# yurimjeon1892/EFGH

Hardware: AMD Instinct MI355X
Metric: frame-pairs/sec EFGHNet fwd+bwd (384x1280 RGB + 64x2048 range), whole job (higher is better)
Workload: dtype f32; 1 GPU; BASELINE.json configs[2]: EFGHNet fwd+bwd with efghloss + gradient all-reduce + fused Adam, synthetic 384x1280 RGB + 131072-point sweep, batch=8 per GPU, random-init weights; global_batch=8, points=131072, parallelism=dp1

## Files before the change

efgh_amd/csrc/backward.hip:

```cpp
#include "common.h"

namespace {
constexpr int TPB = 256;

__device__ __forceinline__ float4 sign4(const unsigned *__restrict__ bits, long long e) {
    const unsigned w = bits[e >> 5] >> ((unsigned)e & 31u);
    return make_float4((w & 1u) ? 1.f : -1.f, (w & 2u) ? 1.f : -1.f, (w & 4u) ? 1.f : -1.f, (w & 8u) ? 1.f : -1.f);
}

__device__ __forceinline__ float dact(float y, int act, float slope) {
    if (act == 1) return y > 0.f ? 1.f : 0.f;
    if (act == 2) return y > 0.f ? 1.f : slope;
    return 1.f;
}

template <bool NT>
__global__ void __launch_bounds__(TPB)
k_act_bn_bwd_reduce(const float *__restrict__ dy, long long lddy, const float *__restrict__ y, long long ldy,
                    const float *__restrict__ raw, long long ldraw, const float *__restrict__ mean,
                    const float *__restrict__ invstd, const float *__restrict__ pscale,
                    const float *__restrict__ pshift, long long M, int C, int act, float slope, int rows_per_block,
                    int CL, double *__restrict__ part, const unsigned *__restrict__ ybits) {
    __shared__ double s1s[TPB][4], s2s[TPB][4];
    const int cl = threadIdx.x % CL, rl = threadIdx.x / CL, RL = TPB / CL;
    const int c = (blockIdx.x * CL + cl) * 4;
    long long r0 = (long long)blockIdx.y * rows_per_block, r1 = r0 + rows_per_block;
    if (r1 > M) r1 = M;
    double s1[4] = {0., 0., 0., 0.}, s2[4] = {0., 0., 0., 0.};
    if (c < C) {
        float4 mu = make_float4(0.f, 0.f, 0.f, 0.f), is = mu, psc = mu, psh = mu;
        if (mean) { mu = *reinterpret_cast<const float4 *>(mean + c); is = *reinterpret_cast<const float4 *>(invstd + c); }
        const bool from_raw = !y && !ybits;
        if (from_raw) { psc = *reinterpret_cast<const float4 *>(pscale + c); psh = *reinterpret_cast<const float4 *>(pshift + c); }
        for (long long r = r0 + rl; r < r1; r += RL) {
            float4 g = ld_stream<NT>(dy + r * lddy + c);
            float4 rw = make_float4(0.f, 0.f, 0.f, 0.f);
            if (mean || from_raw) rw = ld_stream<NT>(raw + r * ldraw + c);
            float4 yy;
            if (ybits) yy = sign4(ybits, r * C + c);
            else if (y) yy = *reinterpret_cast<const float4 *>(y + r * ldy + c);
            else yy = make_float4(rw.x * psc.x + psh.x, rw.y * psc.y + psh.y, rw.z * psc.z + psh.z, rw.w * psc.w + psh.w);
            g.x *= dact(yy.x, act, slope); g.y *= dact(yy.y, act, slope);
            g.z *= dact(yy.z, act, slope); g.w *= dact(yy.w, act, slope);
            s1[0] += (double)g.x; s1[1] += (double)g.y; s1[2] += (double)g.z; s1[3] += (double)g.w;
            if (mean) {
                s2[0] += (double)g.x * (double)((rw.x - mu.x) * is.x); s2[1] += (double)g.y * (double)((rw.y - mu.y) * is.y);
                s2[2] += (double)g.z * (double)((rw.z - mu.z) * is.z); s2[3] += (double)g.w * (double)((rw.w - mu.w) * is.w);
            }
        }
    }
#pragma unroll
    for (int q = 0; q < 4; ++q) { s1s[threadIdx.x][q] = s1[q]; s2s[threadIdx.x][q] = s2[q]; }
    __syncthreads();
    if (rl != 0 || c >= C) return;
    for (int i = 1; i < RL; ++i)
#pragma unroll
        for (int q = 0; q < 4; ++q) { s1[q] += s1s[i * CL + cl][q]; s2[q] += s2s[i * CL + cl][q]; }
#pragma unroll
    for (int q = 0; q < 4; ++q) {
        part[((long long)blockIdx.y * 2) * C + c + q] = s1[q];
        part[((long long)blockIdx.y * 2 + 1) * C + c + q] = s2[q];
    }
}

__global__ void __launch_bounds__(1024)
k_bwd_finalize(const double *__restrict__ part, int G, int C, double count,
               float *__restrict__ sum_dpre, float *__restrict__ sum_dpre_xhat,
               double *__restrict__ mean_dpre, double *__restrict__ mean_dpre_xhat) {
    __shared__ double sa[32][33], sb[32][33];
    const int tx = threadIdx.x, ty = threadIdx.y;
    const int c = blockIdx.x * 32 + tx;
    double a = 0.0, b = 0.0;
    if (c < C) {
        double a1 = 0.0, b1 = 0.0, a2 = 0.0, b2 = 0.0, a3 = 0.0, b3 = 0.0;
        int g = ty;
        for (; g + 96 < G; g += 128) {
            a += part[((long long)g * 2) * C + c]; b += part[((long long)g * 2 + 1) * C + c];
            a1 += part[((long long)(g + 32) * 2) * C + c]; b1 += part[((long long)(g + 32) * 2 + 1) * C + c];
            a2 += part[((long long)(g + 64) * 2) * C + c]; b2 += part[((long long)(g + 64) * 2 + 1) * C + c];
            a3 += part[((long long)(g + 96) * 2) * C + c]; b3 += part[((long long)(g + 96) * 2 + 1) * C + c];
        }
        for (; g < G; g += 32) { a += part[((long long)g * 2) * C + c]; b += part[((long long)g * 2 + 1) * C + c]; }
        a += (a1 + a2) + a3; b += (b1 + b2) + b3;
    }
    sa[ty][tx] = a; sb[ty][tx] = b;
    __syncthreads();
    if (ty != 0 || c >= C) return;
    for (int i = 1; i < 32; ++i) { a += sa[i][tx]; b += sb[i][tx]; }
    sum_dpre[c] = (float)a; sum_dpre_xhat[c] = (float)b;
    if (mean_dpre) { mean_dpre[c] = a / count; mean_dpre_xhat[c] = b / count; }
}

template <bool NT>
__global__ void __launch_bounds__(TPB)
k_act_bn_bwd_apply(const float *__restrict__ dy, long long lddy, const float *__restrict__ y, long long ldy,
                   const float *__restrict__ raw, long long ldraw, const float *__restrict__ mean,
                   const float *__restrict__ invstd, const float *__restrict__ coef,
                   const double *__restrict__ m1, const double *__restrict__ m2, const float *__restrict__ pscale,
                   const float *__restrict__ pshift, long long M, int C, int act,
                   float slope, float *__restrict__ draw, long long lddraw, float *__restrict__ dres,
                   long long lddres, const unsigned *__restrict__ ybits) {
    const int c4n = C >> 2;
    long long total = M * c4n;
    const bool from_raw = !y && !ybits;
    for (long long i = (long long)blockIdx.x * TPB + threadIdx.x; i < total; i += (long long)gridDim.x * TPB) {
        long long r = i / c4n; int c = (int)(i - r * c4n) * 4;
        float4 g = ld_stream<NT>(dy + r * lddy + c);
        float4 rw = make_float4(0.f, 0.f, 0.f, 0.f);
        if (mean || from_raw) rw = ld_stream<NT>(raw + r * ldraw + c);
        float4 yy;
        if (ybits) yy = sign4(ybits, r * C + c);
        else if (y) yy = *reinterpret_cast<const float4 *>(y + r * ldy + c);
        else yy = make_float4(rw.x * pscale[c] + pshift[c], rw.y * pscale[c + 1] + pshift[c + 1],
                              rw.z * pscale[c + 2] + pshift[c + 2], rw.w * pscale[c + 3] + pshift[c + 3]);
        float gv[4] = {g.x * dact(yy.x, act, slope), g.y * dact(yy.y, act, slope), g.z * dact(yy.z, act, slope),
                       g.w * dact(yy.w, act, slope)};
        if (dres) st_stream<NT>(dres + r * lddres + c, make_float4(gv[0], gv[1], gv[2], gv[3]));
        float o[4];
        if (mean) {
            float rv[4] = {rw.x, rw.y, rw.z, rw.w};
#pragma unroll
            for (int q = 0; q < 4; ++q) {
                const double xh = ((double)rv[q] - (double)mean[c + q]) * (double)invstd[c + q];
                o[q] = (float)((double)coef[c + q] * ((double)gv[q] - m1[c + q] - xh * m2[c + q]));
            }
        } else {
#pragma unroll
            for (int q = 0; q < 4; ++q) o[q] = coef ? coef[c + q] * gv[q] : gv[q];
        }
        if (draw) st_stream<NT>(draw + r * lddraw + c, make_float4(o[0], o[1], o[2], o[3]));
    }
}

__device__ __forceinline__ void pool_cell_dpre(const float4 v[4], const bool ok[4], bool pooled, const float4 g, const float sc[4],
                                               const float sf[4], int act, float slope, float dpre[4][4]) {
#pragma unroll
    for (int ch = 0; ch < 4; ++ch) {
        float e[4];
#pragma unroll
        for (int q = 0; q < 4; ++q) {
            const float t = ((const float *)&v[q])[ch] * sc[ch] + sf[ch];
            e[q] = act == 1 ? (t > 0.f ? t : 0.f) : (act == 2 ? (t > 0.f ? t : t * slope) : t);
        }
        int best = 0;
#pragma unroll
        for (int q = 1; q < 4; ++q) if (e[q] > e[best]) best = q;
        const float gg = ((const float *)&g)[ch];
#pragma unroll
        for (int q = 0; q < 4; ++q) {
            const float t = ((const float *)&v[q])[ch] * sc[ch] + sf[ch];
            const float da = act == 1 ? (t > 0.f ? 1.f : 0.f) : (act == 2 ? (t > 0.f ? 1.f : slope) : 1.f);
            dpre[q][ch] = (pooled && q == best && ok[q]) ? gg * da : 0.f;
        }
    }
}

template <bool NT>
__global__ void __launch_bounds__(TPB)
k_pool_bn_bwd_reduce(const float *__restrict__ dyp, const float *__restrict__ raw, const float *__restrict__ mean,
                     const float *__restrict__ invstd, const float *__restrict__ pscale, const float *__restrict__ pshift,
                     int B, int H, int W, int C, int act, float slope, int cells_per_block, int CL, double *__restrict__ part) {
    __shared__ double s1s[TPB][4], s2s[TPB][4];
    const int Hc = (H + 1) / 2, Wc = (W + 1) / 2, Ho = H / 2, Wo = W / 2;
    const long long ncell = (long long)B * Hc * Wc;
    const int cl = threadIdx.x % CL, rl = threadIdx.x / CL, RL = TPB / CL;
    const int c = (blockIdx.x * CL + cl) * 4;
    long long r0 = (long long)blockIdx.y * cells_per_block, r1 = r0 + cells_per_block;
    if (r1 > ncell) r1 = ncell;
    double s1[4] = {0., 0., 0., 0.}, s2[4] = {0., 0., 0., 0.};
    if (c < C) {
        const float4 mu = *reinterpret_cast<const float4 *>(mean + c), is = *reinterpret_cast<const float4 *>(invstd + c);
        const float4 psc = *reinterpret_cast<const float4 *>(pscale + c), psh = *reinterpret_cast<const float4 *>(pshift + c);
        const float sc[4] = {psc.x, psc.y, psc.z, psc.w}, sf[4] = {psh.x, psh.y, psh.z, psh.w};
        const float muv[4] = {mu.x, mu.y, mu.z, mu.w}, isv[4] = {is.x, is.y, is.z, is.w};
        for (long long r = r0 + rl; r < r1; r += RL) {
            const int j = (int)(r % Wc); const long long t = r / Wc;
            const int i = (int)(t % Hc); const long long b = t / Hc;
            if (i >= Ho || j >= Wo) continue;
            const long long base = (((b * H + 2 * i) * W) + 2 * j) * (long long)C + c;
            const long long offs[4] = {0, C, (long long)W * C, (long long)W * C + C};
            float4 v[4];
            const bool ok[4] = {true, true, true, true};
#pragma unroll
            for (int q = 0; q < 4; ++q) v[q] = ld_stream<NT>(raw + base + offs[q]);
            const float4 g = *reinterpret_cast<const float4 *>(dyp + (((b * Ho + i) * Wo) + j) * (long long)C + c);
            float dpre[4][4];
            pool_cell_dpre(v, ok, true, g, sc, sf, act, slope, dpre);
#pragma unroll
            for (int q = 0; q < 4; ++q)
#pragma unroll
                for (int ch = 0; ch < 4; ++ch) {
                    const float d = dpre[q][ch];
                    s1[ch] += (double)d;
                    s2[ch] += (double)d * (double)((((const float *)&v[q])[ch] - muv[ch]) * isv[ch]);
                }
        }
    }
#pragma unroll
    for (int q = 0; q < 4; ++q) { s1s[threadIdx.x][q] = s1[q]; s2s[threadIdx.x][q] = s2[q]; }
    __syncthreads();
    if (rl != 0 || c >= C) return;
    for (int k = 1; k < RL; ++k)
#pragma unroll
        for (int q = 0; q < 4; ++q) { s1[q] += s1s[k * CL + cl][q]; s2[q] += s2s[k * CL + cl][q]; }
#pragma unroll
    for (int q = 0; q < 4; ++q) {
        part[((long long)blockIdx.y * 2) * C + c + q] = s1[q];
        part[((long long)blockIdx.y * 2 + 1) * C + c + q] = s2[q];
    }
}

template <bool NT>
__global__ void __launch_bounds__(TPB)
k_pool_bn_bwd_reduce_y(const float *__restrict__ dyp, const float *__restrict__ y, const float *__restrict__ raw,
                       const float *__restrict__ mean, const float *__restrict__ invstd, const float *__restrict__ pscale,
                       const float *__restrict__ pshift, int H, int W, int C, long long Mp, int rows_per_block, int CL,
                       double *__restrict__ part) {
    __shared__ double s1s[TPB][4], s2s[TPB][4];
    const int cl = threadIdx.x % CL, rl = threadIdx.x / CL, RL = TPB / CL;
    const int c = (blockIdx.x * CL + cl) * 4;
    const int Ho = H >> 1, Wo = W >> 1;
    long long r0 = (long long)blockIdx.y * rows_per_block, r1 = r0 + rows_per_block;
    if (r1 > Mp) r1 = Mp;
    double s1[4] = {0., 0., 0., 0.}, s2[4] = {0., 0., 0., 0.};
    if (c < C) {
        const float4 mu = *reinterpret_cast<const float4 *>(mean + c), is = *reinterpret_cast<const float4 *>(invstd + c);
        const float4 psc = *reinterpret_cast<const float4 *>(pscale + c), psh = *reinterpret_cast<const float4 *>(pshift + c);
        const float muv[4] = {mu.x, mu.y, mu.z, mu.w}, isv[4] = {is.x, is.y, is.z, is.w};
        const float scv[4] = {psc.x, psc.y, psc.z, psc.w}, shv[4] = {psh.x, psh.y, psh.z, psh.w};
        float bet[4], rg[4];
        bool flat = false;
#pragma unroll
        for (int q = 0; q < 4; ++q) {
            bet[q] = fmaf(muv[q], scv[q], shv[q]);
            rg[q] = scv[q] != 0.f ? isv[q] / scv[q] : 0.f;
            flat |= scv[q] == 0.f;
        }
        for (long long r = r0 + rl; r < r1; r += RL) {
            const float4 g4 = ld_stream<NT>(dyp + r * C + c), y4 = ld_stream<NT>(y + r * C + c);
            const float gv[4] = {g4.x, g4.y, g4.z, g4.w}, yv[4] = {y4.x, y4.y, y4.z, y4.w};
            float rw0[4] = {0.f, 0.f, 0.f, 0.f};
            if (flat) {
                const int j = (int)(r % Wo); const long long t = r / Wo;
                const int i = (int)(t % Ho); const long long b = t / Ho;
                const float4 w4 = *reinterpret_cast<const float4 *>(raw + (((b * H + 2 * i) * W) + 2 * j) * (long long)C + c);
                rw0[0] = w4.x; rw0[1] = w4.y; rw0[2] = w4.z; rw0[3] = w4.w;
            }
#pragma unroll
            for (int q = 0; q < 4; ++q) {
                const float d = yv[q] > 0.f ? gv[q] : 0.f;
                const float xh = scv[q] != 0.f ? (yv[q] - bet[q]) * rg[q] : (rw0[q] - muv[q]) * isv[q];
                s1[q] += (double)d;
                s2[q] += (double)d * (double)xh;
            }
        }
    }
#pragma unroll
    for (int q = 0; q < 4; ++q) { s1s[threadIdx.x][q] = s1[q]; s2s[threadIdx.x][q] = s2[q]; }
    __syncthreads();
    if (rl != 0 || c >= C) return;
    for (int k = 1; k < RL; ++k)
#pragma unroll
        for (int q = 0; q < 4; ++q) { s1[q] += s1s[k * CL + cl][q]; s2[q] += s2s[k * CL + cl][q]; }
#pragma unroll
    for (int q = 0; q < 4; ++q) {
        part[((long long)blockIdx.y * 2) * C + c + q] = s1[q];
        part[((long long)blockIdx.y * 2 + 1) * C + c + q] = s2[q];
    }
}

template <bool NT>
__global__ void __launch_bounds__(TPB)
k_pool_bn_bwd_apply(const float *__restrict__ dyp, const float *__restrict__ raw, const float *__restrict__ mean,
                    const float *__restrict__ invstd, const float *__restrict__ coef, const double *__restrict__ m1,
                    const double *__restrict__ m2, const float *__restrict__ pscale, const float *__restrict__ pshift, int B,
                    int H, int W, int C, int act, float slope, float *__restrict__ draw) {
    const int Hc = (H + 1) / 2, Wc = (W + 1) / 2, Ho = H / 2, Wo = W / 2, c4n = C >> 2;
    const long long total = (long long)B * Hc * Wc * c4n;
    for (long long idx = (long long)blockIdx.x * TPB + threadIdx.x; idx < total; idx += (long long)gridDim.x * TPB) {
        const int c = (int)(idx % c4n) * 4; long long r = idx / c4n;
        const int j = (int)(r % Wc); r /= Wc;
        const int i = (int)(r % Hc); const long long b = r / Hc;
        const bool pooled = i < Ho && j < Wo;
        const long long base = (((b * H + 2 * i) * W) + 2 * j) * (long long)C + c;
        const long long offs[4] = {0, C, (long long)W * C, (long long)W * C + C};
        const bool ok[4] = {true, 2 * j + 1 < W, 2 * i + 1 < H, (2 * j + 1 < W) && (2 * i + 1 < H)};
        float4 v[4];
#pragma unroll
        for (int q = 0; q < 4; ++q) v[q] = ok[q] ? ld_stream<NT>(raw + base + offs[q]) : make_float4(0.f, 0.f, 0.f, 0.f);
        float4 g = make_float4(0.f, 0.f, 0.f, 0.f);
        if (pooled) g = *reinterpret_cast<const float4 *>(dyp + (((b * Ho + i) * Wo) + j) * (long long)C + c);
        const float4 psc = *reinterpret_cast<const float4 *>(pscale + c), psh = *reinterpret_cast<const float4 *>(pshift + c);
        const float sc[4] = {psc.x, psc.y, psc.z, psc.w}, sf[4] = {psh.x, psh.y, psh.z, psh.w};
        float dpre[4][4];
        pool_cell_dpre(v, ok, pooled, g, sc, sf, act, slope, dpre);
#pragma unroll
        for (int q = 0; q < 4; ++q) {
            if (!ok[q]) continue;
            float o[4];
#pragma unroll
            for (int ch = 0; ch < 4; ++ch) {
                const double xh = ((double)((const float *)&v[q])[ch] - (double)mean[c + ch]) * (double)invstd[c + ch];
                o[ch] = (float)((double)coef[c + ch] * ((double)dpre[q][ch] - m1[c + ch] - xh * m2[c + ch]));
            }
            st_stream<NT>(draw + base + offs[q], make_float4(o[0], o[1], o[2], o[3]));
        }
    }
}

__global__ void __launch_bounds__(TPB)
k_maxpool2_bwd_affine(const float *__restrict__ x, const float *__restrict__ scale, const float *__restrict__ shift, int act,
                      float slope, const float *__restrict__ dy, float *__restrict__ dx, int B, int H, int W, int C) {
    const int Ho = H / 2, Wo = W / 2, c4 = C >> 2;
    long long total = (long long)B * Ho * Wo * c4;
    for (long long i = (long long)blockIdx.x * TPB + threadIdx.x; i < total; i += (long long)gridDim.x * TPB) {
        int c = (int)(i % c4) * 4; long long r = i / c4;
        int ow = (int)(r % Wo); r /= Wo;
        int oh = (int)(r % Ho); long long b = r / Ho;
        long long base = (((b * H + oh * 2) * W) + ow * 2) * (long long)C + c;
        const long long offs[4] = {0, C, (long long)W * C, (long long)W * C + C};
        const float4 sc = *reinterpret_cast<const float4 *>(scale + c), sf = *reinterpret_cast<const float4 *>(shift + c);
        const float scv[4] = {sc.x, sc.y, sc.z, sc.w}, sfv[4] = {sf.x, sf.y, sf.z, sf.w};
        float4 v[4];
#pragma unroll
        for (int q = 0; q < 4; ++q) v[q] = *reinterpret_cast<const float4 *>(x + base + offs[q]);
        float4 g = *reinterpret_cast<const float4 *>(dy + (((b * Ho + oh) * Wo) + ow) * (long long)C + c);
        float o[4][4];
        const float gg[4] = {g.x, g.y, g.z, g.w};
#pragma unroll
        for (int ch = 0; ch < 4; ++ch) {
            float e[4] = {((float *)&v[0])[ch], ((float *)&v[1])[ch], ((float *)&v[2])[ch], ((float *)&v[3])[ch]};
#pragma unroll
            for (int q = 0; q < 4; ++q) {
                float t = e[q] * scv[ch] + sfv[ch];
                e[q] = act == 1 ? (t > 0.f ? t : 0.f) : (act == 2 ? (t > 0.f ? t : t * slope) : t);
            }
            int best = 0;
#pragma unroll
            for (int q = 1; q < 4; ++q) if (e[q] > e[best]) best = q;
#pragma unroll
            for (int q = 0; q < 4; ++q) o[q][ch] = (q == best) ? gg[ch] : 0.f;
        }
#pragma unroll
        for (int q = 0; q < 4; ++q)
            *reinterpret_cast<float4 *>(dx + base + offs[q]) = make_float4(o[q][0], o[q][1], o[q][2], o[q][3]);
    }
}

__global__ void __launch_bounds__(TPB)
k_maxpool2_bwd(const float *__restrict__ x, const float *__restrict__ dy, float *__restrict__ dx, int B, int H,
               int W, int C) {
    const int Ho = H / 2, Wo = W / 2, c4 = C >> 2;
    long long total = (long long)B * Ho * Wo * c4;
    for (long long i = (long long)blockIdx.x * TPB + threadIdx.x; i < total; i += (long long)gridDim.x * TPB) {
        int c = (int)(i % c4) * 4; long long r = i / c4;
        int ow = (int)(r % Wo); r /= Wo;
        int oh = (int)(r % Ho); long long b = r / Ho;
        long long base = (((b * H + oh * 2) * W) + ow * 2) * (long long)C + c;
        const long long offs[4] = {0, C, (long long)W * C, (long long)W * C + C};
        float4 v[4];
#pragma unroll
        for (int q = 0; q < 4; ++q) v[q] = *reinterpret_cast<const float4 *>(x + base + offs[q]);
        float4 g = *reinterpret_cast<const float4 *>(dy + (((b * Ho + oh) * Wo) + ow) * (long long)C + c);
        float o[4][4];
        const float gg[4] = {g.x, g.y, g.z, g.w};
#pragma unroll
        for (int ch = 0; ch < 4; ++ch) {
            float e[4] = {((float *)&v[0])[ch], ((float *)&v[1])[ch], ((float *)&v[2])[ch], ((float *)&v[3])[ch]};
            int best = 0;
#pragma unroll
            for (int q = 1; q < 4; ++q) if (e[q] > e[best]) best = q;
#pragma unroll
            for (int q = 0; q < 4; ++q) o[q][ch] = (q == best) ? gg[ch] : 0.f;
        }
#pragma unroll
        for (int q = 0; q < 4; ++q)
            *reinterpret_cast<float4 *>(dx + base + offs[q]) = make_float4(o[q][0], o[q][1], o[q][2], o[q][3]);
    }
}

__global__ void k_segment_colmax_bwd(const float *__restrict__ dy, const int *__restrict__ argrow, int nseg, int C,
                                     float *__restrict__ dx, long long ld) {
    int i = blockIdx.x * blockDim.x + threadIdx.x;
    if (i >= nseg * C) return;
    int c = i % C;
    dx[(long long)argrow[i] * ld + c] = dy[i];
}

__global__ void __launch_bounds__(TPB)
k_segment_colmean_bwd(const float *__restrict__ dy, int P, int nseg, int C, float *__restrict__ dx, long long ld) {
    long long total = (long long)nseg * P * C;
    for (long long i = (long long)blockIdx.x * TPB + threadIdx.x; i < total; i += (long long)gridDim.x * TPB) {
        int c = (int)(i % C); long long r = i / C;
        int s = (int)(r / P);
        dx[r * ld + c] = dy[(long long)s * C + c] / (float)P;
    }
}

__global__ void __launch_bounds__(TPB)
k_softmax2_bwd(const float *__restrict__ y, const float *__restrict__ dy, int B, long long HW,
               float *__restrict__ dx, long long ld) {
    long long total = (long long)B * HW;
    for (long long i = (long long)blockIdx.x * TPB + threadIdx.x; i < total; i += (long long)gridDim.x * TPB) {
        long long b = i / HW, p = i - b * HW;
        float y0 = y[(b * 2) * HW + p], y1 = y[(b * 2 + 1) * HW + p];
        float g0 = dy[(b * 2) * HW + p], g1 = dy[(b * 2 + 1) * HW + p];
        float dot = g0 * y0 + g1 * y1;
        for (int c = 0; c < (int)ld; ++c) dx[i * ld + c] = 0.f;
        dx[i * ld] = y0 * (g0 - dot);
        dx[i * ld + 1] = y1 * (g1 - dot);
    }
}

__global__ void __launch_bounds__(TPB)
k_heads_bwd(const float *__restrict__ y, const float *__restrict__ dmask, const float *__restrict__ ddepth, int B, long long HW,
            float4 *__restrict__ dx) {
    long long total = (long long)B * HW;
    for (long long i = (long long)blockIdx.x * TPB + threadIdx.x; i < total; i += (long long)gridDim.x * TPB) {
        long long b = i / HW, p = i - b * HW;
        float4 o = make_float4(ddepth ? ddepth[i] : 0.f, 0.f, 0.f, 0.f);
        if (dmask) {
            float y0 = y[(b * 2) * HW + p], y1 = y[(b * 2 + 1) * HW + p];
            float g0 = dmask[(b * 2) * HW + p], g1 = dmask[(b * 2 + 1) * HW + p];
            float dot = g0 * y0 + g1 * y1;
            o.y = y0 * (g0 - dot);
            o.z = y1 * (g1 - dot);
        }
        dx[i] = o;
    }
}

__global__ void __launch_bounds__(TPB)
k_corr_bwd_cam(const float *__restrict__ rp, const float *__restrict__ dl, int h, int wc, int wp, int nj,
               float *__restrict__ dcam) {
    const int b = blockIdx.z, y = blockIdx.y;
    int i = blockIdx.x * TPB + threadIdx.x;
    if (i >= wc * 4) return;
    const float4 *r = reinterpret_cast<const float4 *>(rp + (((long long)b * h + y) * wp) * 16) + i;
    const float *g = dl + (long long)b * nj;
    float4 a = make_float4(0.f, 0.f, 0.f, 0.f);
    for (int j = 0; j < nj; ++j) {
        float w = g[j]; float4 v = r[(long long)j * 4];
        a.x += w * v.x; a.y += w * v.y; a.z += w * v.z; a.w += w * v.w;
    }
    reinterpret_cast<float4 *>(dcam + (((long long)b * h + y) * wc) * 16)[i] = a;
}

__global__ void __launch_bounds__(TPB)
k_corr_bwd_rng(const float *__restrict__ cam, const float *__restrict__ cam_mm, const float *__restrict__ dl,
               int h, int wc, int wp, int nj, float *__restrict__ drp) {
    extern __shared__ __attribute__((aligned(16))) float sm[];
    float4 *srow = reinterpret_cast<float4 *>(sm);
    float *sdl = sm + (size_t)wc * 16;
    const int b = blockIdx.z, y = blockIdx.y;
    const float d = cam_mm[b * 2 + 1] - cam_mm[b * 2];
    const float4 *cr = reinterpret_cast<const float4 *>(cam + (((long long)b * h + y) * wc) * 16);
    for (int i = threadIdx.x; i < wc * 4; i += TPB) {
        float4 v = cr[i];
        v.x /= d; v.y /= d; v.z /= d; v.w /= d;
        srow[i] = v;
    }
    for (int i = threadIdx.x; i < nj; i += TPB) sdl[i] = dl[(long long)b * nj + i];
    __syncthreads();
    for (int i = blockIdx.x * TPB + threadIdx.x; i < wp * 4; i += gridDim.x * TPB) {
        int xp = i >> 2, cq = i & 3;
        float4 a = make_float4(0.f, 0.f, 0.f, 0.f);
        int x0 = xp - (nj - 1); if (x0 < 0) x0 = 0;
        int x1 = xp < wc - 1 ? xp : wc - 1;
        for (int x = x0; x <= x1; ++x) {
            float w = sdl[xp - x]; float4 v = srow[x * 4 + cq];
            a.x += w * v.x; a.y += w * v.y; a.z += w * v.z; a.w += w * v.w;
        }
        reinterpret_cast<float4 *>(drp + (((long long)b * h + y) * wp) * 16)[i] = a;
    }
}

__global__ void __launch_bounds__(TPB)
k_corr_unpad(const float *__restrict__ drp, int B, int h, int w, int C, int off, float *__restrict__ dx) {
    const int wp = w + 2 * off, c4n = C >> 2;
    long long total = (long long)B * h * w * c4n;
    for (long long i = (long long)blockIdx.x * TPB + threadIdx.x; i < total; i += (long long)gridDim.x * TPB) {
        int cq = (int)(i % c4n); long long r = i / c4n;
        int xs = (int)(r % w); r /= w;
        const float4 *row = reinterpret_cast<const float4 *>(drp + (r * wp) * C) ;
        float4 a = row[(long long)(xs + off) * c4n + cq];
        int xm = w - 1 - xs;
        if (xm < off) { float4 v = row[(long long)xm * c4n + cq]; a.x += v.x; a.y += v.y; a.z += v.z; a.w += v.w; }
        if (xs < off) { float4 v = row[(long long)(xs + off + w) * c4n + cq]; a.x += v.x; a.y += v.y; a.z += v.z; a.w += v.w; }
        reinterpret_cast<float4 *>(dx)[i] = a;
    }
}

int grid_for(long long total) {
    long long g = (total + TPB - 1) / TPB;
    return (int)(g > 16384 ? 16384 : (g < 1 ? 1 : g));
}
}

#ifndef EFGH_BWD_ROW_GRAN
#define EFGH_BWD_ROW_GRAN 16
#endif
static long long bwd_rows_per_block(long long M) {
    const long long groups = 1024;
    long long rows = (M + groups - 1) / groups;
    rows = (rows + EFGH_BWD_ROW_GRAN - 1) / EFGH_BWD_ROW_GRAN * EFGH_BWD_ROW_GRAN;
    return rows < EFGH_BWD_ROW_GRAN ? EFGH_BWD_ROW_GRAN : rows;
}

extern "C" int32_t efgh_bwd_groups(int64_t M) {
    const long long rows = bwd_rows_per_block(M);
    return (int32_t)((M + rows - 1) / rows);
}

extern "C" int efgh_act_bn_bwd_reduce(const float *dy, int64_t lddy, const float *y, int64_t ldy, const float *raw,
                                      int64_t ldraw, const float *mean, const float *invstd, const float *pscale,
                                      const float *pshift, int64_t M, int32_t C,
                                      int32_t act, float slope, double *part, float *sum_dpre, float *sum_dpre_xhat,
                                      double *mean_dpre, double *mean_dpre_xhat, void *stream_) {
    hipStream_t st = (hipStream_t)stream_;
    EFGH_CHECK_ARG(dy && part && sum_dpre && sum_dpre_xhat && M > 0 && C > 0 && C % 4 == 0);
    EFGH_CHECK_ARG(y || (raw && pscale && pshift));
    EFGH_CHECK_ARG(!mean || (raw && invstd));
    EFGH_CHECK_ARG(lddy % 4 == 0 && ldy % 4 == 0 && (!mean || ldraw % 4 == 0));
    const unsigned *ybits = nullptr;
    if (y && ldy == 0) {
        EFGH_CHECK_ARG(C % 32 == 0);
        ybits = (const unsigned *)y; y = nullptr;
    }
    int G = efgh_bwd_groups(M);
    int CL = 1;
    while (CL < 64 && CL * 4 < C) CL <<= 1;
    if (efgh_stream_nt(M * C * 4ll))
        k_act_bn_bwd_reduce<true><<<dim3(cdiv(C / 4, CL), G), TPB, 0, st>>>(dy, lddy, y, ldy, raw, ldraw, mean, invstd, pscale, pshift, M,
                                                                           C, act, slope, (int)bwd_rows_per_block(M), CL, part, ybits);
    else
        k_act_bn_bwd_reduce<false><<<dim3(cdiv(C / 4, CL), G), TPB, 0, st>>>(dy, lddy, y, ldy, raw, ldraw, mean, invstd, pscale, pshift, M,
                                                                            C, act, slope, (int)bwd_rows_per_block(M), CL, part, ybits);
    k_bwd_finalize<<<cdiv(C, 32), dim3(32, 32), 0, st>>>(part, G, C, (double)M, sum_dpre, sum_dpre_xhat, mean_dpre,
                                                         mean_dpre_xhat);
    EFGH_CHECK_LAUNCH();
    return EFGH_OK;
}

__global__ void __launch_bounds__(1024)
k_bwd_finalize_f32(const float *__restrict__ part, int G, int C, double count, float *__restrict__ sum_dpre,
                   float *__restrict__ sum_dpre_xhat, double *__restrict__ mean_dpre, double *__restrict__ mean_dpre_xhat) {
    __shared__ double sa[32][33], sb[32][33];
    const int tx = threadIdx.x, ty = threadIdx.y;
    const int c = blockIdx.x * 32 + tx;
    double a = 0.0, b = 0.0;
    if (c < C) {
        double a1 = 0.0, b1 = 0.0, a2 = 0.0, b2 = 0.0, a3 = 0.0, b3 = 0.0;
        int g = ty;
        for (; g + 96 < G; g += 128) {
            a += (double)part[((long long)g * 2) * C + c]; b += (double)part[((long long)g * 2 + 1) * C + c];
            a1 += (double)part[((long long)(g + 32) * 2) * C + c]; b1 += (double)part[((long long)(g + 32) * 2 + 1) * C + c];
            a2 += (double)part[((long long)(g + 64) * 2) * C + c]; b2 += (double)part[((long long)(g + 64) * 2 + 1) * C + c];
            a3 += (double)part[((long long)(g + 96) * 2) * C + c]; b3 += (double)part[((long long)(g + 96) * 2 + 1) * C + c];
        }
        for (; g < G; g += 32) { a += (double)part[((long long)g * 2) * C + c]; b += (double)part[((long long)g * 2 + 1) * C + c]; }
        a += (a1 + a2) + a3; b += (b1 + b2) + b3;
    }
    sa[ty][tx] = a; sb[ty][tx] = b;
    __syncthreads();
    if (ty != 0 || c >= C) return;
    for (int i = 1; i < 32; ++i) { a += sa[i][tx]; b += sb[i][tx]; }
    sum_dpre[c] = (float)a; sum_dpre_xhat[c] = (float)b;
    mean_dpre[c] = a / count; mean_dpre_xhat[c] = b / count;
}

extern "C" int efgh_bwd_finalize_f32(const float *stats, int32_t rows, int32_t C, double count, float *sum_dpre,
                                     float *sum_dpre_xhat, double *mean_dpre, double *mean_dpre_xhat, void *stream_) {
    EFGH_CHECK_ARG(stats && rows > 0 && C > 0 && count > 0 && sum_dpre && sum_dpre_xhat && mean_dpre && mean_dpre_xhat);
    k_bwd_finalize_f32<<<cdiv(C, 32), dim3(32, 32), 0, (hipStream_t)stream_>>>(stats, rows, C, count, sum_dpre, sum_dpre_xhat,
                                                                               mean_dpre, mean_dpre_xhat);
    EFGH_CHECK_LAUNCH();
    return EFGH_OK;
}

extern "C" int efgh_act_bn_bwd_apply(const float *dy, int64_t lddy, const float *y, int64_t ldy, const float *raw,
                                     int64_t ldraw, const float *mean, const float *invstd, const float *coef,
                                     const double *m1, const double *m2, const float *pscale, const float *pshift,
                                     int64_t M, int32_t C, int32_t act, float slope,
                                     float *draw, int64_t lddraw, float *dres, int64_t lddres, void *stream_) {
    EFGH_CHECK_ARG(dy && (draw || dres) && M > 0 && C > 0 && C % 4 == 0);
    EFGH_CHECK_ARG(y || (raw && pscale && pshift && ldraw % 4 == 0));
    EFGH_CHECK_ARG(lddy % 4 == 0 && ldy % 4 == 0 && (!draw || lddraw % 4 == 0) && (!dres || lddres % 4 == 0));
    EFGH_CHECK_ARG(!mean || (raw && invstd && coef && m1 && m2 && ldraw % 4 == 0));
    const unsigned *ybits = nullptr;
    if (y && ldy == 0) {
        EFGH_CHECK_ARG(C % 32 == 0);
        ybits = (const unsigned *)y; y = nullptr;
    }
    if (efgh_stream_nt(M * C * 4ll))
        k_act_bn_bwd_apply<true><<<grid_for(M * (C / 4)), TPB, 0, (hipStream_t)stream_>>>(
            dy, lddy, y, ldy, raw, ldraw, mean, invstd, coef, m1, m2, pscale, pshift, M, C, act, slope, draw, lddraw, dres, lddres, ybits);
    else
        k_act_bn_bwd_apply<false><<<grid_for(M * (C / 4)), TPB, 0, (hipStream_t)stream_>>>(
            dy, lddy, y, ldy, raw, ldraw, mean, invstd, coef, m1, m2, pscale, pshift, M, C, act, slope, draw, lddraw, dres, lddres, ybits);
    EFGH_CHECK_LAUNCH();
    return EFGH_OK;
}

extern "C" int efgh_maxpool2_bwd(const float *x, const float *dy, float *dx, int32_t B, int32_t H, int32_t W,
                                 int32_t C, void *stream_) {
    EFGH_CHECK_ARG(x && dy && dx && B > 0 && H >= 2 && W >= 2 && C % 4 == 0);
    k_maxpool2_bwd<<<grid_for((long long)B * (H / 2) * (W / 2) * (C / 4)), TPB, 0, (hipStream_t)stream_>>>(x, dy, dx, B, H,
                                                                                                       W, C);
    EFGH_CHECK_LAUNCH();
    return EFGH_OK;
}

extern "C" int efgh_maxpool2_bwd_affine(const float *x, const float *scale, const float *shift, int32_t act, float slope,
                                        const float *dy, float *dx, int32_t B, int32_t H, int32_t W, int32_t C, void *stream_) {
    EFGH_CHECK_ARG(x && scale && shift && dy && dx && B > 0 && H >= 2 && W >= 2 && C % 4 == 0);
    k_maxpool2_bwd_affine<<<grid_for((long long)B * (H / 2) * (W / 2) * (C / 4)), TPB, 0, (hipStream_t)stream_>>>(
        x, scale, shift, act, slope, dy, dx, B, H, W, C);
    EFGH_CHECK_LAUNCH();
    return EFGH_OK;
}

extern "C" int efgh_segment_colmax_bwd(const float *dy, const int32_t *argrow, int32_t nseg, int32_t C, float *dx,
                                       int64_t ld, void *stream_) {
    EFGH_CHECK_ARG(dy && argrow && dx && nseg > 0 && C > 0);
    k_segment_colmax_bwd<<<cdiv((long long)nseg * C, 256), 256, 0, (hipStream_t)stream_>>>(dy, argrow, nseg, C, dx, ld);
    EFGH_CHECK_LAUNCH();
    return EFGH_OK;
}

extern "C" int efgh_segment_colmean_bwd(const float *dy, int32_t P, int32_t nseg, int32_t C, float *dx, int64_t ld,
                                        void *stream_) {
    EFGH_CHECK_ARG(dy && dx && P > 0 && nseg > 0 && C > 0);
    k_segment_colmean_bwd<<<grid_for((long long)nseg * P * C), TPB, 0, (hipStream_t)stream_>>>(dy, P, nseg, C, dx, ld);
    EFGH_CHECK_LAUNCH();
    return EFGH_OK;
}

extern "C" int efgh_heads_bwd(const float *y, const float *dmask, const float *ddepth, int32_t B, int64_t HW, float *dx,
                              void *stream_) {
    EFGH_CHECK_ARG(y && dx && B > 0 && HW > 0 && (((uintptr_t)dx) & 15) == 0);
    k_heads_bwd<<<grid_for((long long)B * HW), TPB, 0, (hipStream_t)stream_>>>(y, dmask, ddepth, B, HW, (float4 *)dx);
    EFGH_CHECK_LAUNCH();
    return EFGH_OK;
}

extern "C" int efgh_softmax2_bwd(const float *y, const float *dy, int32_t B, int64_t HW, float *dx, int64_t ld,
                                 void *stream_) {
    EFGH_CHECK_ARG(y && dy && dx && B > 0 && HW > 0 && ld >= 2);
    k_softmax2_bwd<<<grid_for((long long)B * HW), TPB, 0, (hipStream_t)stream_>>>(y, dy, B, HW, dx, ld);
    EFGH_CHECK_LAUNCH();
    return EFGH_OK;
}

extern "C" int efgh_corr1d_bwd(const float *rp, const float *cam, const float *cam_mm, const float *dlogit, int32_t B,
                               int32_t h, int32_t wc, int32_t wp, float *dcam_n, float *drp, void *stream_) {
    hipStream_t st = (hipStream_t)stream_;
    EFGH_CHECK_ARG(rp && cam && cam_mm && dlogit && dcam_n && drp && B > 0 && h > 0 && wc > 0 && wp >= wc);
    int nj = wp - wc + 1;
    k_corr_bwd_cam<<<dim3(cdiv(wc * 4, TPB), h, B), TPB, 0, st>>>(rp, dlogit, h, wc, wp, nj, dcam_n);
    EFGH_CHECK_ARG((size_t)wc * 64 + (size_t)nj * 4 <= 64 * 1024);
    k_corr_bwd_rng<<<dim3(cdiv(wp * 4, TPB * 4), h, B), TPB, (size_t)wc * 64 + (size_t)nj * 4, st>>>(cam, cam_mm, dlogit, h, wc, wp, nj,
                                                                                              drp);
    EFGH_CHECK_LAUNCH();
    return EFGH_OK;
}

extern "C" int efgh_corr_unpad(const float *drp, int32_t B, int32_t h, int32_t w, int32_t C, int32_t off, float *dx,
                               void *stream_) {
    EFGH_CHECK_ARG(drp && dx && B > 0 && h > 0 && w > 0 && C % 4 == 0 && off >= 0 && off <= w);
    k_corr_unpad<<<grid_for((long long)B * h * w * (C / 4)), TPB, 0, (hipStream_t)stream_>>>(drp, B, h, w, C, off, dx);
    EFGH_CHECK_LAUNCH();
    return EFGH_OK;
}

extern "C" int32_t efgh_pool_bwd_groups(int32_t B, int32_t H, int32_t W) {
    const long long ncell = (long long)B * ((H + 1) / 2) * ((W + 1) / 2);
    const long long rows = bwd_rows_per_block(ncell);
    return (int32_t)((ncell + rows - 1) / rows);
}

extern "C" int efgh_pool_bn_bwd_reduce(const float *dy_pool, const float *raw, const float *mean, const float *invstd,
                                       const float *pscale, const float *pshift, int32_t B, int32_t H, int32_t W, int32_t C,
                                       int32_t act, float slope, double *part, float *sum_dpre, float *sum_dpre_xhat,
                                       double *mean_dpre, double *mean_dpre_xhat, void *stream_) {
    hipStream_t st = (hipStream_t)stream_;
    EFGH_CHECK_ARG(dy_pool && raw && mean && invstd && pscale && pshift && part && sum_dpre && sum_dpre_xhat && mean_dpre &&
                   mean_dpre_xhat);
    EFGH_CHECK_ARG(B > 0 && H >= 2 && W >= 2 && C > 0 && C % 4 == 0);
    const long long ncell = (long long)B * ((H + 1) / 2) * ((W + 1) / 2);
    const int G = efgh_pool_bwd_groups(B, H, W);
    int CL = 1;
    while (CL < 64 && CL * 4 < C) CL <<= 1;
    if (efgh_stream_nt((long long)B * H * W * C * 4)) k_pool_bn_bwd_reduce<true><<<dim3(cdiv(C / 4, CL), G), TPB, 0, st>>>(dy_pool, raw, mean, invstd, pscale, pshift, B, H, W, C, act,
                                                                  slope, (int)bwd_rows_per_block(ncell), CL, part);
    else k_pool_bn_bwd_reduce<false><<<dim3(cdiv(C / 4, CL), G), TPB, 0, st>>>(dy_pool, raw, mean, invstd, pscale, pshift, B, H, W, C, act,
                                                                  slope, (int)bwd_rows_per_block(ncell), CL, part);
    k_bwd_finalize<<<cdiv(C, 32), dim3(32, 32), 0, st>>>(part, G, C, (double)B * H * W, sum_dpre, sum_dpre_xhat, mean_dpre,
                                                         mean_dpre_xhat);
    EFGH_CHECK_LAUNCH();
    return EFGH_OK;
}

extern "C" int efgh_pool_bn_bwd_reduce_pooled(const float *dy_pool, const float *y_pool, const float *raw, const float *mean,
                                              const float *invstd, const float *pscale, const float *pshift, int32_t B, int32_t H,
                                              int32_t W, int32_t C, double *part, float *sum_dpre, float *sum_dpre_xhat,
                                              double *mean_dpre, double *mean_dpre_xhat, void *stream_) {
    hipStream_t st = (hipStream_t)stream_;
    EFGH_CHECK_ARG(dy_pool && y_pool && raw && mean && invstd && pscale && pshift && part && sum_dpre && sum_dpre_xhat && mean_dpre &&
                   mean_dpre_xhat);
    EFGH_CHECK_ARG(B > 0 && H >= 2 && W >= 2 && C > 0 && C % 4 == 0);
    const long long Mp = (long long)B * (H / 2) * (W / 2);
    const int G = efgh_bwd_groups(Mp);
    int CL = 1;
    while (CL < 64 && CL * 4 < C) CL <<= 1;
    if (efgh_stream_nt(Mp * C * 4)) k_pool_bn_bwd_reduce_y<true><<<dim3(cdiv(C / 4, CL), G), TPB, 0, st>>>(dy_pool, y_pool, raw, mean, invstd, pscale, pshift, H, W, C, Mp,
                                                                  (int)bwd_rows_per_block(Mp), CL, part);
    else k_pool_bn_bwd_reduce_y<false><<<dim3(cdiv(C / 4, CL), G), TPB, 0, st>>>(dy_pool, y_pool, raw, mean, invstd, pscale, pshift, H, W, C, Mp,
                                                                  (int)bwd_rows_per_block(Mp), CL, part);
    k_bwd_finalize<<<cdiv(C, 32), dim3(32, 32), 0, st>>>(part, G, C, (double)B * H * W, sum_dpre, sum_dpre_xhat, mean_dpre,
                                                         mean_dpre_xhat);
    EFGH_CHECK_LAUNCH();
    return EFGH_OK;
}

extern "C" int efgh_pool_bn_bwd_apply(const float *dy_pool, const float *raw, const float *mean, const float *invstd,
                                      const float *coef, const double *m1, const double *m2, const float *pscale,
                                      const float *pshift, int32_t B, int32_t H, int32_t W, int32_t C, int32_t act,
                                      float slope, float *draw, void *stream_) {
    EFGH_CHECK_ARG(dy_pool && raw && mean && invstd && coef && m1 && m2 && pscale && pshift && draw);
    EFGH_CHECK_ARG(B > 0 && H >= 2 && W >= 2 && C > 0 && C % 4 == 0);
    const long long total = (long long)B * ((H + 1) / 2) * ((W + 1) / 2) * (C / 4);
    if (efgh_stream_nt((long long)B * H * W * C * 4)) k_pool_bn_bwd_apply<true><<<grid_for(total), TPB, 0, (hipStream_t)stream_>>>(dy_pool, raw, mean, invstd, coef, m1, m2, pscale,
                                                                          pshift, B, H, W, C, act, slope, draw);
    else k_pool_bn_bwd_apply<false><<<grid_for(total), TPB, 0, (hipStream_t)stream_>>>(dy_pool, raw, mean, invstd, coef, m1, m2, pscale,
                                                                          pshift, B, H, W, C, act, slope, draw);
    EFGH_CHECK_LAUNCH();
    return EFGH_OK;
}
```

efgh_amd/csrc/c4conv.hip:

```cpp
#include "common.h"


namespace {

typedef float f32x16 __attribute__((ext_vector_type(16)));
typedef float f32x4 __attribute__((ext_vector_type(4)));

constexpr int TP = 32;
constexpr int LWMAX = (TP - 1) * 2 + 3;
constexpr int WAVES = 4;

struct C4Args {
    const float *A; long long lda;
    int B, Hin, Win, Ho, Wo, s;
    const float *W; int N;
    const float *bias, *scale, *shift, *residual; long long ldr;
    int act; float slope;
    float *out; long long ldo;
    float *stats;
    long long units; int jblocks;
    const float *G; long long ldg; float *dW;
};

__device__ __forceinline__ void unit_coords(const C4Args &p, long long unit, long long &row, int &i, long long &b, int &j0) {
    const int jb = (int)(unit % p.jblocks);
    row = unit / p.jblocks;
    i = (int)(row % p.Ho); b = row / p.Ho;
    j0 = jb * TP;
}

__device__ __forceinline__ float4 load_px(const C4Args &p, int idx, int LW, int i, long long b, int j0) {
    const int kh = idx / LW, x = idx - kh * LW;
    const int yin = p.s * i - 1 + kh, xin = p.s * j0 - 1 + x;
    if (kh < 3 && (unsigned)yin < (unsigned)p.Hin && (unsigned)xin < (unsigned)p.Win)
        return *reinterpret_cast<const float4 *>(p.A + ((b * p.Hin + yin) * p.Win + xin) * p.lda);
    return make_float4(0.f, 0.f, 0.f, 0.f);
}

__device__ __forceinline__ void wave_lds_sync() {
    __builtin_amdgcn_fence(__ATOMIC_RELEASE, "wavefront");
    __builtin_amdgcn_wave_barrier();
    __builtin_amdgcn_fence(__ATOMIC_ACQUIRE, "wavefront");
}

template <int NT, bool RES>
__global__ void __launch_bounds__(64 * WAVES, 2) k_c4_conv(const C4Args p) {
    __shared__ float2 Pw[WAVES][3][2][LWMAX + 1];
    __shared__ float red[2][WAVES][NT * 32];
    constexpr int TPITCH = 40;
    __shared__ __attribute__((aligned(16))) float Tw[WAVES][32 * TPITCH];
    const int tid = threadIdx.x, lane = tid & 63, wave = tid >> 6, r = lane & 31, h = lane >> 5;
    const int LW = (TP - 1) * p.s + 3;
    float2 (*P)[2][LWMAX + 1] = Pw[wave];
    float *T = Tw[wave];

    float2 bw[9][NT];
    float bi[NT], sc[NT], sf[NT], s1[NT], s2[NT];
#pragma unroll
    for (int j = 0; j < NT; ++j) {
        const int n = 32 * j + r;
#pragma unroll
        for (int t = 0; t < 9; ++t) bw[t][j] = *reinterpret_cast<const float2 *>(p.W + ((long long)n * 9 + t) * 4 + 2 * h);
        bi[j] = p.bias ? p.bias[n] : 0.f;
        sc[j] = p.scale ? p.scale[n] : 1.f;
        sf[j] = p.shift ? p.shift[n] : 0.f;
        s1[j] = 0.f; s2[j] = 0.f;
    }
    const float neg = p.act == 1 ? 0.f : (p.act == 2 ? p.slope : 1.f);

#pragma unroll
    for (int j = 0; j < NT; ++j)
#pragma unroll
        for (int t = 0; t < 9; ++t) asm volatile("" ::"v"(bw[t][j].x), "v"(bw[t][j].y));

    const long long nwaves = (long long)gridDim.x * WAVES;
    long long unit = (long long)blockIdx.x * WAVES + wave;
    long long row = 0, b = 0; int i = 0, j0 = 0;
    long long crow = 0; int cj0 = 0;
    float4 pf0, pf1, pf2, pf3;
#define EFGH_FETCH(u)                                                                    \
    {                                                                                   \
        unit_coords(p, u, row, i, b, j0);                                               \
        pf0 = load_px(p, lane, LW, i, b, j0); pf1 = load_px(p, lane + 64, LW, i, b, j0); \
        pf2 = load_px(p, lane + 128, LW, i, b, j0); pf3 = load_px(p, lane + 192, LW, i, b, j0); \
    }
#define EFGH_PUT(q, v)                                                                   \
    {                                                                                   \
        const int idx = lane + 64 * q;                                                  \
        if (idx < 3 * LW) {                                                             \
            const int kh = idx / LW, x = idx - kh * LW;                                 \
            P[kh][0][x] = make_float2(v.x, v.y); P[kh][1][x] = make_float2(v.z, v.w);   \
        }                                                                               \
    }
#define EFGH_STAGE()                                                                     \
    {                                                                                   \
        crow = row; cj0 = j0;                                                           \
        EFGH_PUT(0, pf0) EFGH_PUT(1, pf1) EFGH_PUT(2, pf2) EFGH_PUT(3, pf3)             \
    }
    if (unit < p.units) {
        EFGH_FETCH(unit)
        EFGH_STAGE()
        if (unit + nwaves < p.units) EFGH_FETCH(unit + nwaves)
    }
    for (; unit < p.units; unit += nwaves) {
        const long long orow0 = crow; const int oj0 = cj0;
        wave_lds_sync();
        f32x16 acc[NT];
#pragma unroll
        for (int j = 0; j < NT; ++j)
#pragma unroll
            for (int q = 0; q < 16; ++q) acc[j][q] = 0.f;
        const int px = r * p.s;
        float2 af[9];
#pragma unroll
        for (int t = 0; t < 9; ++t) af[t] = P[t / 3][h][px + t % 3];
#pragma unroll
        for (int t = 0; t < 9; ++t) {
#pragma unroll
            for (int j = 0; j < NT; ++j) {
                acc[j] = __builtin_amdgcn_mfma_f32_32x32x2f32(af[t].x, bw[t][j].x, acc[j], 0, 0, 0);
                acc[j] = __builtin_amdgcn_mfma_f32_32x32x2f32(af[t].y, bw[t][j].y, acc[j], 0, 0, 0);
            }
        }
        wave_lds_sync();
        if (unit + nwaves < p.units) {
            EFGH_STAGE()
            if (unit + 2 * nwaves < p.units) EFGH_FETCH(unit + 2 * nwaves)
        }
        const bool full = oj0 + TP <= p.Wo;
#pragma unroll
        for (int j = 0; j < NT; ++j) {
            float4 rr[4];
            if (RES) {
#pragma unroll
                for (int pass = 0; pass < 4; ++pass) {
                    const int pl = 8 * pass + (lane >> 3), c4 = (lane & 7) * 4;
                    rr[pass] = (full || oj0 + pl < p.Wo)
                                   ? *reinterpret_cast<const float4 *>(p.residual + (orow0 * p.Wo + oj0 + pl) * p.ldr + 32 * j + c4)
                                   : make_float4(0.f, 0.f, 0.f, 0.f);
                }
            }
            wave_lds_sync();
#pragma unroll
            for (int q = 0; q < 16; ++q) {
                const int pl = (q & 3) + 8 * (q >> 2) + 4 * h;
                const bool ok = full || oj0 + pl < p.Wo;
                float v = acc[j][q] + bi[j];
                if (ok) { s1[j] += v; s2[j] = fmaf(v, v, s2[j]); }
                v = fmaf(v, sc[j], sf[j]);
                T[pl * TPITCH + r] = RES ? v : act_neg(v, neg);
            }
            wave_lds_sync();
#pragma unroll
            for (int pass = 0; pass < 4; ++pass) {
                const int pl = 8 * pass + (lane >> 3), c4 = (lane & 7) * 4;
                float4 v = *reinterpret_cast<const float4 *>(&T[pl * TPITCH + c4]);
                if (RES) {
                    v.x += rr[pass].x; v.y += rr[pass].y; v.z += rr[pass].z; v.w += rr[pass].w;
                    v.x = act_neg(v.x, neg); v.y = act_neg(v.y, neg);
                    v.z = act_neg(v.z, neg); v.w = act_neg(v.w, neg);
                }
                if (full || oj0 + pl < p.Wo)
                    *reinterpret_cast<float4 *>(p.out + (orow0 * p.Wo + oj0 + pl) * p.ldo + 32 * j + c4) = v;
            }
        }
    }
#undef EFGH_FETCH
#undef EFGH_PUT
#undef EFGH_STAGE
    if (p.stats) {
#pragma unroll
        for (int j = 0; j < NT; ++j) {
            s1[j] += __shfl_xor(s1[j], 32); s2[j] += __shfl_xor(s2[j], 32);
            if (h == 0) { red[0][wave][32 * j + r] = s1[j]; red[1][wave][32 * j + r] = s2[j]; }
        }
        __syncthreads();
        for (int n = tid; n < NT * 32; n += 64 * WAVES) {
            float a1 = 0.f, a2 = 0.f;
#pragma unroll
            for (int w = 0; w < WAVES; ++w) { a1 += red[0][w][n]; a2 += red[1][w][n]; }
            p.stats[((long long)blockIdx.x * 2 + 0) * p.N + n] = a1;
            p.stats[((long long)blockIdx.x * 2 + 1) * p.N + n] = a2;
        }
    }
}

constexpr int LW1 = TP + 2;
__device__ __forceinline__ float4 load_px4(const C4Args &p, int idx, int ip, long long b, int j0) {
    const int kh = idx / LW1, x = idx - kh * LW1;
    const int yin = 2 * ip - 1 + kh, xin = j0 - 1 + x;
    if (kh < 4 && (unsigned)yin < (unsigned)p.Hin && (unsigned)xin < (unsigned)p.Win)
        return *reinterpret_cast<const float4 *>(p.A + ((b * p.Hin + yin) * p.Win + xin) * p.lda);
    return make_float4(0.f, 0.f, 0.f, 0.f);
}

template <int NT>
__global__ void __launch_bounds__(64 * WAVES, 2) k_c4_conv_pool(const C4Args p) {
    __shared__ float2 Pw[WAVES][4][2][LW1 + 1];
    constexpr int TPITCH = 40;
    __shared__ __attribute__((aligned(16))) float Tw[WAVES][32 * TPITCH];
    const int tid = threadIdx.x, lane = tid & 63, wave = tid >> 6, r = lane & 31, h = lane >> 5;
    float2 (*P)[2][LW1 + 1] = Pw[wave];
    float *T = Tw[wave];
    const int Hp = p.Ho >> 1, Wp = p.Wo >> 1;

    float2 bw[9][NT];
    float bi[NT], sc[NT], sf[NT];
#pragma unroll
    for (int j = 0; j < NT; ++j) {
        const int n = 32 * j + r;
#pragma unroll
        for (int t = 0; t < 9; ++t) bw[t][j] = *reinterpret_cast<const float2 *>(p.W + ((long long)n * 9 + t) * 4 + 2 * h);
        bi[j] = p.bias ? p.bias[n] : 0.f;
        sc[j] = p.scale ? p.scale[n] : 1.f;
        sf[j] = p.shift ? p.shift[n] : 0.f;
    }
    const float neg = p.act == 1 ? 0.f : (p.act == 2 ? p.slope : 1.f);
#pragma unroll
    for (int j = 0; j < NT; ++j)
#pragma unroll
        for (int t = 0; t < 9; ++t) asm volatile("" ::"v"(bw[t][j].x), "v"(bw[t][j].y));

    const long long nwaves = (long long)gridDim.x * WAVES;
    long long unit = (long long)blockIdx.x * WAVES + wave;
    long long rowp = 0, b = 0; int ip = 0, j0 = 0;
    long long crow = 0; int cj0 = 0;
    float4 pf0, pf1, pf2;
#define EFGH_FETCH(u)                                                                    \
    {                                                                                   \
        const int jb = (int)((u) % p.jblocks);                                          \
        rowp = (u) / p.jblocks; ip = (int)(rowp % Hp); b = rowp / Hp; j0 = jb * TP;     \
        pf0 = load_px4(p, lane, ip, b, j0); pf1 = load_px4(p, lane + 64, ip, b, j0);    \
        pf2 = load_px4(p, lane + 128, ip, b, j0);                                       \
    }
#define EFGH_PUT(q, v)                                                                   \
    {                                                                                   \
        const int idx = lane + 64 * q;                                                  \
        if (idx < 4 * LW1) {                                                            \
            const int kh = idx / LW1, x = idx - kh * LW1;                               \
            P[kh][0][x] = make_float2(v.x, v.y); P[kh][1][x] = make_float2(v.z, v.w);   \
        }                                                                               \
    }
#define EFGH_STAGE()                                                                     \
    {                                                                                   \
        crow = rowp; cj0 = j0;                                                          \
        EFGH_PUT(0, pf0) EFGH_PUT(1, pf1) EFGH_PUT(2, pf2)                              \
    }
    if (unit < p.units) {
        EFGH_FETCH(unit)
        EFGH_STAGE()
        if (unit + nwaves < p.units) EFGH_FETCH(unit + nwaves)
    }
    for (; unit < p.units; unit += nwaves) {
        const long long orow0 = crow; const int oj0 = cj0;
        wave_lds_sync();
        f32x16 acc[2][NT];
#pragma unroll
        for (int half = 0; half < 2; ++half) {
#pragma unroll
            for (int j = 0; j < NT; ++j)
#pragma unroll
                for (int q = 0; q < 16; ++q) acc[half][j][q] = 0.f;
            float2 af[9];
#pragma unroll
            for (int t = 0; t < 9; ++t) af[t] = P[t / 3 + half][h][r + t % 3];
#pragma unroll
            for (int t = 0; t < 9; ++t) {
#pragma unroll
                for (int j = 0; j < NT; ++j) {
                    acc[half][j] = __builtin_amdgcn_mfma_f32_32x32x2f32(af[t].x, bw[t][j].x, acc[half][j], 0, 0, 0);
                    acc[half][j] = __builtin_amdgcn_mfma_f32_32x32x2f32(af[t].y, bw[t][j].y, acc[half][j], 0, 0, 0);
                }
            }
        }
        wave_lds_sync();
        if (unit + nwaves < p.units) {
            EFGH_STAGE()
            if (unit + 2 * nwaves < p.units) EFGH_FETCH(unit + 2 * nwaves)
        }
#pragma unroll
        for (int j = 0; j < NT; ++j) {
            wave_lds_sync();
#pragma unroll
            for (int q = 0; q < 16; ++q) {
                const int pl = (q & 3) + 8 * (q >> 2) + 4 * h;
                const float v0 = act_neg(fmaf(acc[0][j][q] + bi[j], sc[j], sf[j]), neg);
                const float v1 = act_neg(fmaf(acc[1][j][q] + bi[j], sc[j], sf[j]), neg);
                T[pl * TPITCH + r] = fmaxf(v0, v1);
            }
            wave_lds_sync();
#pragma unroll
            for (int pass = 0; pass < 2; ++pass) {
                const int item = 64 * pass + lane, pp = item >> 3, c4 = (item & 7) * 4;
                const float4 a = *reinterpret_cast<const float4 *>(&T[(2 * pp) * TPITCH + c4]);
                const float4 c = *reinterpret_cast<const float4 *>(&T[(2 * pp + 1) * TPITCH + c4]);
                float4 v;
                v.x = fmaxf(a.x, c.x); v.y = fmaxf(a.y, c.y); v.z = fmaxf(a.z, c.z); v.w = fmaxf(a.w, c.w);
                if ((oj0 >> 1) + pp < Wp)
                    *reinterpret_cast<float4 *>(p.out + (orow0 * Wp + (oj0 >> 1) + pp) * p.ldo + 32 * j + c4) = v;
            }
        }
    }
#undef EFGH_FETCH
#undef EFGH_PUT
#undef EFGH_STAGE
}

template <int NT16>
__global__ void __launch_bounds__(64 * WAVES) k_c4_wgrad(const C4Args p) {
    __shared__ float4 Xw[WAVES][3][LWMAX + 1];
    const int tid = threadIdx.x, lane = tid & 63, wave = tid >> 6, q16 = lane & 15, k4 = lane >> 4;
    const int LW = (TP - 1) * p.s + 3;
    float4 (*X)[LWMAX + 1] = Xw[wave];
    f32x4 acc[NT16][3];
#pragma unroll
    for (int a = 0; a < NT16; ++a)
#pragma unroll
        for (int c = 0; c < 3; ++c)
#pragma unroll
            for (int e = 0; e < 4; ++e) acc[a][c][e] = 0.f;
    int coff[3]; bool cok[3];
#pragma unroll
    for (int c = 0; c < 3; ++c) {
        const int col = 16 * c + q16, t = col >> 2, ch = col & 3;
        cok[c] = col < 36;
        coff[c] = cok[c] ? ((t / 3) * (LWMAX + 1) + t % 3) * 4 + ch : 0;
    }
    const float *Xf = reinterpret_cast<const float *>(&X[0][0]);

    const long long nwaves = (long long)gridDim.x * WAVES;
    long long unit = (long long)blockIdx.x * WAVES + wave;
    long long row = 0, b = 0; int i = 0, j0 = 0;
    float4 pf0, pf1, pf2, pf3;
    float ga[8][NT16], gn[8][NT16];
#define EFGH_FETCH(u)                                                                    \
    {                                                                                   \
        unit_coords(p, u, row, i, b, j0);                                               \
        pf0 = load_px(p, lane, LW, i, b, j0); pf1 = load_px(p, lane + 64, LW, i, b, j0); \
        pf2 = load_px(p, lane + 128, LW, i, b, j0); pf3 = load_px(p, lane + 192, LW, i, b, j0); \
        const float *grow = p.G + (row * p.Wo + j0) * p.ldg + q16;                       \
        _Pragma("unroll") for (int g = 0; g < 8; ++g) {                                 \
            const int pl = 4 * g + k4;                                                  \
            const bool ok = j0 + pl < p.Wo;                                             \
            _Pragma("unroll") for (int a = 0; a < NT16; ++a) gn[g][a] = ok ? grow[(long long)pl * p.ldg + 16 * a] : 0.f; \
        }                                                                               \
    }
#define EFGH_PUT(q, v)                                                                   \
    {                                                                                   \
        const int idx = lane + 64 * q;                                                  \
        if (idx < 3 * LW) X[idx / LW][idx % LW] = v;                                     \
    }
    if (unit < p.units) EFGH_FETCH(unit)
    for (; unit < p.units; unit += nwaves) {
        wave_lds_sync();
        EFGH_PUT(0, pf0) EFGH_PUT(1, pf1) EFGH_PUT(2, pf2) EFGH_PUT(3, pf3)
#pragma unroll
        for (int g = 0; g < 8; ++g)
#pragma unroll
            for (int a = 0; a < NT16; ++a) ga[g][a] = gn[g][a];
        wave_lds_sync();
        if (unit + nwaves < p.units) EFGH_FETCH(unit + nwaves)
#pragma unroll
        for (int g = 0; g < 8; ++g) {
            const int pl = 4 * g + k4;
            float xb[3];
#pragma unroll
            for (int c = 0; c < 3; ++c) xb[c] = cok[c] ? Xf[coff[c] + pl * p.s * 4] : 0.f;
#pragma unroll
            for (int a = 0; a < NT16; ++a)
#pragma unroll
                for (int c = 0; c < 3; ++c) acc[a][c] = __builtin_amdgcn_mfma_f32_16x16x4f32(ga[g][a], xb[c], acc[a][c], 0, 0, 0);
        }
    }
#undef EFGH_FETCH
#undef EFGH_PUT
    float *plane = p.dW + ((long long)blockIdx.x * WAVES + wave) * (16 * NT16 * 36);
#pragma unroll
    for (int a = 0; a < NT16; ++a)
#pragma unroll
        for (int c = 0; c < 3; ++c) {
            if (!cok[c]) continue;
#pragma unroll
            for (int e = 0; e < 4; ++e)
                plane[(16 * a + 4 * k4 + e) * 36 + 16 * c + q16] = acc[a][c][e];
        }
}

bool c4_geometry_ok(const efgh_gemm_desc *d) {
    if (!d || d->mode != 1 || d->C != 4 || d->T != 9 || d->M_dev || d->nbatch > 1) return false;
    if (d->sh != d->sw || (d->sh != 1 && d->sh != 2) || d->osh != 1 || d->osw != 1 || d->oh0 || d->ow0) return false;
    if (d->Hv != d->Ho || d->Wv != d->Wo || d->B <= 0 || d->M != (int64_t)d->B * d->Ho * d->Wo) return false;
    for (int t = 0; t < 9; ++t) if (d->dh[t] != t / 3 - 1 || d->dw[t] != t % 3 - 1) return false;
    if (d->residual && (d->ldr % 4 != 0 || (((uintptr_t)d->residual) & 15) != 0)) return false;
    return d->lda % 4 == 0 && (((uintptr_t)d->A) & 15) == 0;
}

void fill(C4Args &a, const efgh_gemm_desc *d) {
    a.A = d->A; a.lda = d->lda; a.B = d->B; a.Hin = d->Hin; a.Win = d->Win; a.Ho = d->Ho; a.Wo = d->Wo; a.s = d->sh;
    a.W = d->W; a.N = d->N; a.bias = d->bias; a.scale = d->scale; a.shift = d->shift; a.residual = d->residual; a.ldr = d->ldr; a.act = d->act; a.slope = d->slope;
    a.out = d->out; a.ldo = d->ldo; a.stats = d->stats;
    a.jblocks = (d->Wo + TP - 1) / TP;
    a.units = (long long)d->B * d->Ho * a.jblocks;
    a.G = nullptr; a.ldg = 0; a.dW = nullptr;
}

int grid_of(long long units) {
    const long long g = (units + WAVES - 1) / WAVES;
    return (int)(g < 768 ? g : 768);
}

}

extern "C" int efgh_c4_supported(const efgh_gemm_desc *d) {
    return (c4_geometry_ok(d) && (d->N == 32 || d->N == 64 || d->N == 128)) ? 1 : 0;
}

extern "C" int32_t efgh_c4_stats_rows(int32_t B, int32_t Ho, int32_t Wo) {
    return grid_of((long long)B * Ho * ((Wo + TP - 1) / TP));
}

extern "C" int efgh_c4_conv3x3(const efgh_gemm_desc *d, void *stream_) {
    hipStream_t st = (hipStream_t)stream_;
    EFGH_CHECK_ARG(efgh_c4_supported(d) && d->W && d->out && (((uintptr_t)d->W) & 7) == 0);
    EFGH_CHECK_ARG(d->ldo % 4 == 0 && (((uintptr_t)d->out) & 15) == 0);
    C4Args a;
    fill(a, d);
    const int grid = grid_of(a.units);
    const bool res = d->residual != nullptr;
#define EFGH_GO(NT)                                                                  \
    {                                                                               \
        if (res) k_c4_conv<NT, true><<<grid, 64 * WAVES, 0, st>>>(a);               \
        else k_c4_conv<NT, false><<<grid, 64 * WAVES, 0, st>>>(a);                  \
    }
    if (d->N == 32) EFGH_GO(1) else if (d->N == 64) EFGH_GO(2) else EFGH_GO(4)
#undef EFGH_GO
    EFGH_CHECK_LAUNCH();
    return EFGH_OK;
}

extern "C" int efgh_c4_pooled_supported(const efgh_gemm_desc *d) {
    return (efgh_c4_supported(d) && d->sh == 1 && !d->residual && !d->stats && d->Ho >= 2 && d->Wo >= 2) ? 1 : 0;
}

extern "C" int efgh_c4_conv3x3_pooled(const efgh_gemm_desc *d, void *stream_) {
    hipStream_t st = (hipStream_t)stream_;
    EFGH_CHECK_ARG(efgh_c4_pooled_supported(d) && d->W && d->out && (((uintptr_t)d->W) & 7) == 0);
    EFGH_CHECK_ARG(d->ldo % 4 == 0 && (((uintptr_t)d->out) & 15) == 0);
    C4Args a;
    fill(a, d);
    a.units = (long long)d->B * (d->Ho / 2) * a.jblocks;
    const int grid = grid_of(a.units);
    if (d->N == 32) k_c4_conv_pool<1><<<grid, 64 * WAVES, 0, st>>>(a);
    else if (d->N == 64) k_c4_conv_pool<2><<<grid, 64 * WAVES, 0, st>>>(a);
    else k_c4_conv_pool<4><<<grid, 64 * WAVES, 0, st>>>(a);
    EFGH_CHECK_LAUNCH();
    return EFGH_OK;
}

extern "C" int efgh_c4_wgrad_supported(const efgh_gemm_desc *d) {
    return (c4_geometry_ok(d) && d->N % 16 == 0 && d->N >= 32 && d->N <= 128) ? 1 : 0;
}

extern "C" int64_t efgh_c4_wgrad_workspace(const efgh_gemm_desc *d) {
    if (!efgh_c4_wgrad_supported(d)) return 0;
    C4Args a;
    fill(a, d);
    return (int64_t)grid_of(a.units) * WAVES * d->N * 36;
}

extern "C" int efgh_c4_wgrad(const efgh_gemm_desc *d, const float *G, int64_t ldg, float *dWp, float *workspace,
                             const efgh_wgrad_out_desc *out, void *stream_) {
    hipStream_t st = (hipStream_t)stream_;
    EFGH_CHECK_ARG(efgh_c4_wgrad_supported(d) && G && dWp && ldg >= d->N);
    EFGH_CHECK_ARG(workspace && (((uintptr_t)workspace) & 15) == 0 && (((uintptr_t)dWp) & 15) == 0);
    C4Args a;
    fill(a, d);
    a.G = G; a.ldg = ldg; a.dW = workspace;
    const int grid = grid_of(a.units);
    switch (d->N / 16) {
    case 2: k_c4_wgrad<2><<<grid, 256, 0, st>>>(a); break;
    case 3: k_c4_wgrad<3><<<grid, 256, 0, st>>>(a); break;
    case 4: k_c4_wgrad<4><<<grid, 256, 0, st>>>(a); break;
    case 5: k_c4_wgrad<5><<<grid, 256, 0, st>>>(a); break;
    case 6: k_c4_wgrad<6><<<grid, 256, 0, st>>>(a); break;
    case 7: k_c4_wgrad<7><<<grid, 256, 0, st>>>(a); break;
    default: k_c4_wgrad<8><<<grid, 256, 0, st>>>(a); break;
    }
    const bool wrote = efgh_launch_fold_splits(workspace, grid * WAVES, (long long)d->N * 36, dWp, st, out);
    EFGH_CHECK_LAUNCH();
    return wrote ? EFGH_WROTE_OUT : EFGH_OK;
}
```

efgh_amd/csrc/common.h:

```cpp
#pragma once
#include <hip/hip_runtime.h>
#include <stdint.h>
#include <stdlib.h>
#include <stdio.h>
#include <stdarg.h>
#include <atomic>

#include "../../include/efgh_hip.h"

void efgh_set_error(const char *fmt, ...);

#define EFGH_CHECK_ARG(cond)                                                         \
    do {                                                                             \
        if (!(cond)) {                                                               \
            efgh_set_error("%s:%d: invalid argument: %s", __FILE__, __LINE__, #cond); \
            return EFGH_E_INVALID;                                                   \
        }                                                                            \
    } while (0)

#define EFGH_CHECK_LAUNCH()                                                          \
    do {                                                                             \
        hipError_t e_ = hipGetLastError();                                           \
        if (e_ != hipSuccess) {                                                      \
            efgh_set_error("%s:%d: launch failed: %s", __FILE__, __LINE__,           \
                           hipGetErrorString(e_));                                   \
            return EFGH_E_LAUNCH;                                                    \
        }                                                                            \
    } while (0)

static inline int cdiv(int64_t a, int64_t b) { return (int)((a + b - 1) / b); }

__device__ __forceinline__ float act_neg(float v, float neg) { return v > 0.f ? v : fmaf(neg, v, 0.f); }

template <bool NT>
__device__ __forceinline__ float4 ld_stream(const float *p) {
    if (NT) {
        typedef float v4f __attribute__((ext_vector_type(4)));
        const v4f v = __builtin_nontemporal_load(reinterpret_cast<const v4f *>(p));
        return make_float4(v.x, v.y, v.z, v.w);
    }
    return *reinterpret_cast<const float4 *>(p);
}
template <bool NT>
__device__ __forceinline__ void st_stream(float *p, const float4 &v) {
    if (NT) {
        typedef float v4f __attribute__((ext_vector_type(4)));
        v4f w; w.x = v.x; w.y = v.y; w.z = v.z; w.w = v.w;
        __builtin_nontemporal_store(w, reinterpret_cast<v4f *>(p));
    } else {
        *reinterpret_cast<float4 *>(p) = v;
    }
}
static inline bool efgh_stream_nt(long long bytes) { return bytes >= (384ll << 20); }

static inline bool efgh_raise_lds_once(std::atomic<unsigned long long> &done, const void *fn, int bytes) {
    int dev = 0;
    if (hipGetDevice(&dev) != hipSuccess) return false;
    const unsigned long long bit = 1ull << (dev & 63);
    if (done.load(std::memory_order_acquire) & bit) return true;
    if (hipFuncSetAttribute(fn, hipFuncAttributeMaxDynamicSharedMemorySize, bytes) != hipSuccess) return false;
    done.fetch_or(bit, std::memory_order_release);
    return true;
}

#ifndef EFGH_MFMA_NT_OUT
#define EFGH_MFMA_NT_OUT 0
#endif
__device__ __forceinline__ void st_out(float *p, float v) {
#if EFGH_MFMA_NT_OUT
    __builtin_nontemporal_store(v, p);
#else
    *p = v;
#endif
}

__device__ __forceinline__ void dma16(const float *src, unsigned lds_byte_addr) {
    unsigned keep;
    const unsigned dst = __builtin_amdgcn_readfirstlane(lds_byte_addr);
    asm volatile("s_mov_b32 %0, m0\n\ts_mov_b32 m0, %2\n\ts_nop 0\n\tglobal_load_lds_dwordx4 %1, off\n\ts_mov_b32 m0, %0"
                 : "=&s"(keep) : "v"(src), "s"(dst) : "memory");
}
__device__ __forceinline__ unsigned lds_addr(const float *p) {
    return (unsigned)(uintptr_t)(const __attribute__((address_space(3))) float *)p;
}

template <int N> __device__ __forceinline__ void wait_vm() { asm volatile("s_waitcnt vmcnt(%0)" ::"n"(N) : "memory"); }


static inline long long efgh_round_chunks(long long M, long long blocks, int wg_per_cu, int unit, long long min_chunk,
                                          double plane_elems, long long *chunk_out) {
    const long long slots = 256LL * wg_per_cu;
    const double fold_rows = plane_elems * 1.31e-5 * 2.0 / wg_per_cu;
    long long best_zs = 1, best_chunk = (M + unit - 1) / unit * unit;
    double best = -1.0;
    auto consider = [&](long long zs) {
        if (zs < 1) return;
        long long chunk = (M + zs - 1) / zs;
        chunk = (chunk + unit - 1) / unit * unit;
        if (zs > 1 && chunk < min_chunk) return;
        const long long z = (M + chunk - 1) / chunk;
        const long long wg = z * blocks, full = wg / slots, rem = wg % slots;
        const double rounds = (double)full + (rem ? 0.5 + 0.5 * (double)rem / (double)slots : 0.0);
        const double cost = rounds * ((double)chunk + 128.0) + (z > 1 ? (double)z * fold_rows : 0.0);
        if (best < 0.0 || cost < best * 0.995) { best = cost; best_zs = z; best_chunk = chunk; }
    };
    const long long zmax = M / min_chunk > 1 ? M / min_chunk : 1;
    auto clamp = [&](long long z) { return z < 1 ? 1 : (z > zmax ? zmax : z); };
    consider(1);
    for (int r = 1; r <= 4; ++r) {
        const long long zs = r * slots / blocks;
        consider(clamp(zs)); consider(clamp(zs - 1)); consider(clamp(zs + 1));
    }
    consider(zmax); consider(clamp(zmax - 1)); consider(clamp(zmax / 2));
    if (chunk_out) *chunk_out = best_chunk;
    return best_zs;
}

static inline int efgh_wg_per_cu(const void *kernel, int threads, size_t dyn_lds) {
    int n = 0;
    if (hipOccupancyMaxActiveBlocksPerMultiprocessor(&n, kernel, threads, dyn_lds) != hipSuccess || n < 1) n = 1;
    return n;
}

bool efgh_launch_fold_splits(const float *part, int zs, long long total, float *dst, hipStream_t st, const efgh_wgrad_out_desc *out = nullptr);
static inline bool efgh_wgrad_out_fits(const efgh_wgrad_out_desc *out, int rows, int T, int Cp) {
    if (!out || !out->W || out->T != T || out->Cp != Cp || rows < out->N || rows >= out->N + 4) return false;
    for (int t = 0; t < T; ++t) if (out->taps[t] != t) return false;
    return true;
}

__device__ __forceinline__ void wino_pack_item(const float *__restrict__ Wp, float *__restrict__ U, int N, int C, long long i) {
    const double G[6][3] = {{0.25, 0., 0.}, {-1. / 6, -1. / 6, -1. / 6}, {-1. / 6, 1. / 6, -1. / 6},
                            {1. / 24, 1. / 12, 1. / 6}, {1. / 24, -1. / 12, 1. / 6}, {0., 0., 1.}};
    const int ci = (int)(i % 16); long long r = i / 16;
    const int n = (int)(r % N); const int ch = (int)(r / N);
    const int cc = ch / 3, kh = ch - cc * 3, c = cc * 16 + ci;
    const float *w = Wp + ((long long)n * 9 + kh * 3) * C + c;
    const double w0 = w[0], w1 = w[C], w2 = w[2 * (long long)C];
#pragma unroll
    for (int a = 0; a < 6; ++a)
        U[(((long long)ch * 6 + a) * N + n) * 16 + ci] = (float)fma(G[a][2], w2, fma(G[a][1], w1, G[a][0] * w0));
}

__device__ __forceinline__ void w2_pack_item(const float *__restrict__ Wp, float *__restrict__ U, int N, int C, long long i) {
    const double a = 0.75, b = 1.5, f0 = a * a * b * b, fa = 2 * a * a * (a * a - b * b), fb = 2 * b * b * (b * b - a * a);
    const double G[6][3] = {{1 / f0, 0., 0.}, {1 / fa, a / fa, a * a / fa}, {1 / fa, -a / fa, a * a / fa},
                            {1 / fb, b / fb, b * b / fb}, {1 / fb, -b / fb, b * b / fb}, {0., 0., 1.}};
    const int c = (int)(i % C); const long long n = i / C;
    double w[3][3];
#pragma unroll
    for (int t = 0; t < 9; ++t) w[t / 3][t % 3] = Wp[(n * 9 + t) * C + c];
    double gw[6][3];
#pragma unroll
    for (int p = 0; p < 6; ++p)
#pragma unroll
        for (int kw = 0; kw < 3; ++kw) gw[p][kw] = fma(G[p][2], w[2][kw], fma(G[p][1], w[1][kw], G[p][0] * w[0][kw]));
#pragma unroll
    for (int p = 0; p < 6; ++p)
#pragma unroll
        for (int q = 0; q < 6; ++q)
            U[((long long)(6 * p + q) * N + n) * C + c] = (float)fma(gw[p][2], G[q][2], fma(gw[p][1], G[q][1], gw[p][0] * G[q][0]));
}
```

efgh_amd/nets/fn.py:

```python
import torch

from .. import ops
from ..ops import ACT_NONE, ceil4


def rows_ok(t):
    if t.stride(-1) != 1:
        return False
    ld = t.stride(-2) if t.dim() >= 2 else t.shape[-1]
    exp = ld
    for d in range(t.dim() - 2, -1, -1):
        if t.shape[d] != 1 and t.stride(d) != exp:
            return False
        exp *= t.shape[d]
    return ld % 4 == 0 and t.data_ptr() % 16 == 0


def as_rows(t):
    return t if rows_ok(t) else t.contiguous()


def ld_of(t):
    return t.stride(-2) if t.dim() >= 2 else t.shape[-1]


class LayerSpec:
    dgrad = custom_forward = custom_wgrad = None
    takes_bnsrc = passthrough = pool = defer_act = bwd_fusable = False

    def __init__(self, N, C, T, mode, launches, layouts, M, out_shape, bn=None, train=False, act=ACT_NONE, slope=0.0, table=None,
                 c_real=None):
        self.N, self.C, self.T, self.mode, self.M = N, C, T, mode, M
        self.launches, self.layouts, self.out_shape = launches, layouts, out_shape
        self.bn, self.train, self.act, self.slope, self.table = bn, train, act, slope, table
        self.c_real = c_real if c_real is not None else C

    def for_tape(self, dgrad, takes_bnsrc=False, custom_forward=None, custom_wgrad=None, passthrough=False, pool=False,
                 defer_act=False, bwd_fusable=False):
        self.dgrad, self.takes_bnsrc = dgrad, takes_bnsrc
        self.custom_forward, self.custom_wgrad = custom_forward, custom_wgrad
        self.passthrough = passthrough
        self.pool = pool
        self.defer_act = defer_act
        self.bwd_fusable = bwd_fusable
        return self


def run_launches(spec, x, lda, weight, out, ldo, bias, want_stats, a_off=0, out_off=0, lazy=None, pool=False, w2v=None, **epilogue):
    Np = ceil4(spec.N)
    wps = [lay.pack(weight) for lay in spec.layouts]
    custom = spec.custom_forward
    stats, thin = None, False
    if want_stats:
        thin = custom is not None or ops.no_stats_epilogue(spec.mode, spec.C, Np, spec.T, spec.launches)
        if not thin:
            gs = [ops.stats_rows(spec.mode, spec.C, Np, g, m) for g, m in spec.launches]
            stats = torch.empty((sum(gs), 2, Np), dtype=torch.float32, device=x.device)
    if custom is not None:
        custom(x, weight, out)
    if w2v is not None:
        ops.TLS.w2v_wanted = w2v
    g0 = 0
    for li, (geom, m) in enumerate(spec.launches if custom is None else ()):
        T = ops.taps_of(spec.T, geom)
        st = None
        if stats is not None:
            st = stats[g0:g0 + gs[li]]
            g0 += gs[li]
        ops.gather_gemm(x, lda, spec.C, T, wps[li], Np, m, out, ldo, mode=spec.mode, geom=geom, table=spec.table, bias=bias, stats=st,
                        a_off=a_off, out_off=out_off, flops=2.0 * m * spec.N * T * spec.c_real, lazy=lazy, pool=pool, **epilogue)
    if w2v is not None:
        ops.TLS.w2v_wanted = False
    if thin:
        stats, _ = ops.col_stats(out, spec.M, Np, ldo, x_off=out_off)
    return stats


def bn_batch_stats(bn, stats, Np, count, save=False):
    N = bn.num_features
    ops.bn_tick(bn)
    momentum = bn.momentum if bn.momentum is not None else 0.1
    rm, rv = ops.pad_vec(bn.running_mean, Np), ops.pad_vec(bn.running_var, Np, 1.0)
    res = ops.bn_finalize(stats, stats.shape[0], Np, count, ops.pad_vec(bn.weight, Np), ops.pad_vec(bn.bias, Np), rm, rv, momentum,
                          bn.eps, save=save)
    if Np != N:
        bn.running_mean.copy_(rm[:N])
        bn.running_var.copy_(rv[:N])
    return res


def materialize(x, lazy):
    M = x.numel() // x.shape[-1]
    y = torch.empty(x.shape, dtype=torch.float32, device=x.device)
    ops.scale_shift_act(x, ld_of(x), lazy.scale, lazy.shift, y, x.shape[-1], M, x.shape[-1], lazy.act, lazy.slope)
    return y


def claim_grad(p):
    slot = getattr(p, '_efgh_flat', None) if p is not None else None
    if slot is None:
        return None, None
    flat, i = slot
    g = flat.claim(p, i)
    if g is None:
        return None, None
    return g, (lambda stream=None: flat.deliver(i, stream))


def note_use(*params):
    for p in params:
        slot = getattr(p, '_efgh_flat', None) if p is not None else None
        if slot is not None:
            slot[0].uses[slot[1]] += 1


def _bias_grad_behind_bn(ctx, p_bias, draw, M, Np, N, train_bn, delivered):
    if not ctx.needs_input_grad[2]:
        return None
    if not train_bn:
        return ops.col_sum(draw, M, Np)[:N]
    g, done = claim_grad(p_bias)
    if g is not None:
        delivered.append(done)
        return None
    return torch.zeros(N, dtype=torch.float32, device=ctx.saved_tensors[0].device)


class BnSrc:
    __slots__ = ('raw', 'y', 'psc', 'psh', 'mean', 'invstd', 'act', 'slope', 'M', 'N')

    def __init__(self, raw, y, psc, psh, mean, invstd, act, slope, M, N):
        self.raw, self.y, self.psc, self.psh, self.mean, self.invstd = raw, y, psc, psh, mean, invstd
        self.act, self.slope, self.M, self.N = act, slope, M, N

    def fits(self, M, N):
        return self.M == M and self.N == N


TRACE = None


class GemmLayerFn(torch.autograd.Function):

    @staticmethod
    def forward(ctx, x, weight, bias, gamma, beta, residual, spec, out_target=None):
        ctx.planes_split = ops.planes_split_active()
        old, ops.TLS.planes_split = ops.TLS.planes_split, ctx.planes_split
        try:
            return GemmLayerFn._forward(ctx, x, weight, bias, gamma, beta, residual, spec, out_target)
        finally:
            ops.TLS.planes_split = old

    @staticmethod
    def _forward(ctx, x, weight, bias, gamma, beta, residual, spec, out_target=None):
        ctx.set_materialize_grads(False)
        ctx.xsrc = getattr(x, '_efgh_bnsrc', None)
        lazy = getattr(x, '_efgh_lazy', None)
        x = as_rows(x)
        if lazy is not None and not (spec.custom_forward is None and len(spec.launches) == 1 and not spec.passthrough
                                     and x.shape[-1] == spec.C
                                     and ops.lazy_capable(spec.mode, spec.C, ceil4(spec.N), spec.launches[0][0])):
            x, lazy = materialize(x, lazy), None
        ctx.lazy = lazy
        dev = x.device
        N, Np = spec.N, ceil4(spec.N)
        M = spec.M
        bn = spec.bn
        b = None if bias is None else ops.pad_vec(bias.detach(), Np)
        out = torch.empty(tuple(spec.out_shape) + (Np,), dtype=torch.float32, device=dev)
        res = None if residual is None else as_rows(residual)
        mean = invstd = raw = None
        need_stats = bn is not None and spec.train
        assert spec.custom_forward is None or (bn is not None and bias is None)
        w2v = bool(ctx.needs_input_grad[1])
        if bn is None:
            run_launches(spec, x, ld_of(x), weight, out, Np, b, False, lazy=lazy, w2v=w2v, residual=res,
                         ldr=0 if res is None else ld_of(res), act=spec.act, slope=spec.slope)
        else:
            stats = run_launches(spec, x, ld_of(x), weight, out, Np, b, need_stats, lazy=lazy, w2v=w2v)
        y = out
        if bn is not None:
            raw = out
            if need_stats:
                scale, shift, mean, invstd = bn_batch_stats(bn, stats, Np, float(M), save=True)
            else:
                with torch.no_grad():
                    invstd = ops.pad_vec(torch.rsqrt(bn.running_var + bn.eps), Np)
                    mean = ops.pad_vec(bn.running_mean.clone(), Np)
                    scale = ops.pad_vec(gamma.detach(), Np) * invstd
                    shift = ops.pad_vec(beta.detach(), Np) - mean * scale
            if spec.pool:
                assert res is None
                y = ops.maxpool2_affine(raw, scale, shift, spec.act, spec.slope)
            elif (spec.defer_act and ops.LAZY_ACT and need_stats and res is None and Np == N and out_target is None
                  and spec.custom_forward is None):
                y = raw.detach()
                y._efgh_lazy = ops.LazyAct(scale, shift, spec.act, spec.slope)
            else:
                y = None
                if out_target is not None and Np == N:
                    tb, toff = out_target
                    if tuple(tb.shape[:-1]) == tuple(raw.shape[:-1]) and toff % 4 == 0 and toff + N <= tb.shape[-1]:
                        y = tb[..., toff:toff + N]
                if y is None:
                    y = torch.empty_like(raw)
                ybits = None
                if (res is not None and need_stats and ops.BN_MASK_BITS and Np % 32 == 0 and spec.act != ACT_NONE
                        and any(ctx.needs_input_grad)):
                    ybits = torch.empty(M * Np // 32, dtype=torch.int32, device=dev)
                ops.scale_shift_act(raw, Np, scale, shift, y, ld_of(y), M, Np, spec.act, spec.slope, res=res,
                                    ldr=0 if res is None else ld_of(res), bits=ybits)
                ctx.ybits = ybits
        if TRACE is not None:
            y._efgh_src = ('bn' if bn is not None else 'plain', spec.N, spec.pool, residual is not None)
        ctx.bnsrc = None
        if need_stats and not spec.pool and Np == N and any(ctx.needs_input_grad):
            ctx.bnsrc = y._efgh_bnsrc = BnSrc(raw, y.detach() if residual is not None else None, scale, shift, mean, invstd,
                                              spec.act, spec.slope, M, Np)
        ctx.spec = spec
        if not hasattr(ctx, 'ybits'):
            ctx.ybits = None
        ctx.train_step = ops.TLS.train_step
        ctx.has = (bias is not None, gamma is not None, residual is not None)
        ctx.params = (weight, bias, gamma, beta)
        if any(ctx.needs_input_grad[1:5]):
            note_use(weight, bias, gamma, beta)
        psc, psh = (scale, shift) if (bn is not None and residual is None) else (None, None)
        ctx.save_for_backward(x, weight, y, raw, mean, invstd, scale if bn is not None else None, psc, psh)
        if spec.passthrough:
            return y, x.view_as(x)
        return y

    @staticmethod
    def backward(ctx, dy, dskip=None):
        old, ops.TLS.train_step = ops.TLS.train_step, ctx.train_step
        old_split, ops.TLS.planes_split = ops.TLS.planes_split, ctx.planes_split
        try:
            return GemmLayerFn._backward(ctx, dy, dskip)
        finally:
            ops.TLS.train_step = old
            ops.TLS.planes_split = old_split

    @staticmethod
    def _backward(ctx, dy, dskip=None):
        spec = ctx.spec
        sums = getattr(dy, '_efgh_bnsums', None) if dy is not None else None
        if sums is not None and (sums[1] is not ctx.bnsrc or sums[2] != dy._version):
            sums = None
        if dy is None:
            dy = torch.zeros(tuple(spec.out_shape) + (ceil4(spec.N),), dtype=torch.float32, device=ctx.saved_tensors[0].device)
        x, weight, y, raw, mean, invstd, coef, psc, psh = ctx.saved_tensors
        ymask = None if psc is not None else y
        ybits = ctx.ybits
        has_bias, has_bn, has_res = ctx.has
        N, Np, M = spec.N, ceil4(spec.N), spec.M
        dev = x.device
        fused_pool = spec.pool and has_bn and spec.train and not has_res and Np == N
        if TRACE is not None:
            g0, m0 = spec.launches[0] if spec.launches else (None, M)
            TRACE.append(dict(M=M, N=N, C=spec.C, T=spec.T, mode=spec.mode, bn=has_bn, res=has_res, pool=spec.pool, act=spec.act,
                              nl=len(spec.launches), route=ops.gemm_route(spec.mode, spec.C, Np, ops.taps_of(spec.T, g0), g0, m0),
                              x_from=getattr(x, '_efgh_src', None), dx=bool(ctx.needs_input_grad[0]),
                              in_elems=int(x.numel()), custom=spec.custom_forward is not None))
        if spec.pool and not fused_pool:
            dy = ops.maxpool2_bwd_affine(raw, psc, psh, spec.act, spec.slope, dy.contiguous())
        dy = as_rows(dy)
        dbias = dgamma = dbeta = dres = None
        need_pre = spec.act != ACT_NONE or has_bn or has_res or has_bias
        p_w, p_bias, p_gamma, p_beta = ctx.params
        delivered = []
        gs1 = gs2 = None
        if Np == N and has_bn and ctx.needs_input_grad[3] and ctx.needs_input_grad[4]:
            gs1, d1 = claim_grad(p_beta)
            gs2, d2 = claim_grad(p_gamma) if gs1 is not None else (None, None)
            if gs2 is None:
                gs1 = None
            else:
                delivered += [d1, d2]
        elif Np == N and has_bias and not has_bn and ctx.needs_input_grad[2]:
            gs1, d1 = claim_grad(p_bias)
            if gs1 is not None:
                delivered.append(d1)
        own_wgrad = ctx.needs_input_grad[1] and spec.custom_wgrad is None
        pre_v = pre_gy = None
        fuse_bwd = (ops.W2_BWD_FUSED and spec.bwd_fusable and has_bn and spec.train and Np == N
                    and ctx.needs_input_grad[0] and own_wgrad and (ybits is not None or (psc is not None and not has_res))
                    and len(spec.out_shape) == 3 and ((fused_pool and ops.W2_BWD_FUSED_POOL) or not spec.pool))
        if fused_pool:
            draw, s1, s2 = ops.pool_bn_bwd(dy.contiguous(), raw, mean, invstd, coef, psc, psh, spec.act, spec.slope,
                                           s1=gs1, s2=gs2, transforms=fuse_bwd, y_pool=y)
            if fuse_bwd:
                (pre_v, pre_gy), draw = draw, None
            if gs1 is None:
                dbeta, dgamma = s1, s2
            if has_bias:
                dbias = _bias_grad_behind_bn(ctx, p_bias, draw, M, Np, N, True, delivered)
        elif not need_pre:
            draw = dy
        else:
            G = ops.bwd_groups(M)
            part = torch.empty((G, 2, Np), dtype=torch.float64, device=dev)
            s1 = gs1 if gs1 is not None else torch.empty(Np, dtype=torch.float32, device=dev)
            s2 = gs2 if gs2 is not None else torch.empty(Np, dtype=torch.float32, device=dev)
            train_bn = has_bn and spec.train
            m1 = torch.empty(Np, dtype=torch.float64, device=dev) if train_bn else None
            m2 = torch.empty(Np, dtype=torch.float64, device=dev) if train_bn else None
            ldy = Np if ymask is None else ld_of(ymask)
            if ybits is not None:
                ymask, ldy = ybits, 0
            if sums is not None and train_bn:
                f1, f2, m1, m2 = ops.bwd_finalize_f32(sums[0], Np, float(M))
                if gs1 is not None:
                    gs1.copy_(f1)
                    gs2.copy_(f2)
                s1, s2 = (gs1, gs2) if gs1 is not None else (f1, f2)
            else:
                ops.act_bn_bwd_reduce(dy, ld_of(dy), ymask, ldy, raw, Np, mean if has_bn else None,
                                      invstd if has_bn else None, M, Np, spec.act, spec.slope, part, s1, s2, m1, m2,
                                      pscale=psc, pshift=psh)
            if has_bn and gs1 is None:
                dbeta, dgamma = (s1, s2) if Np == N else (s1[:N].clone(), s2[:N].clone())
            if has_bias and not has_bn and gs1 is None:
                dbias = s1 if Np == N else s1[:N].clone()
            if fuse_bwd:
                Bo, Ho, Wo = spec.out_shape
                pre_v, pre_gy, dres = ops.wino2d_bwd_transforms(dy, ld_of(dy), raw, Np, ybits, None if ybits is not None else psc,
                                                                None if ybits is not None else psh, mean, invstd, coef, m1, m2, Np,
                                                                Bo, Ho, Wo, spec.act, spec.slope, has_res)
                draw = None
            else:
                draw = torch.empty(tuple(spec.out_shape) + (Np,), dtype=torch.float32, device=dev)
                if has_res:
                    dres = torch.empty(tuple(spec.out_shape) + (Np,), dtype=torch.float32, device=dev)
                ops.act_bn_bwd_apply(dy, ld_of(dy), ymask, ldy, raw, Np, mean if train_bn else None,
                                     invstd if train_bn else None, coef, m1, m2, M, Np, spec.act, spec.slope, draw, Np,
                                     dres, Np, pscale=psc, pshift=psh)
            if has_bias and has_bn:
                dbias = _bias_grad_behind_bn(ctx, p_bias, draw, M, Np, N, train_bn, delivered)
        gW = dw_done = side = None
        if own_wgrad:
            gW, dw_done = claim_grad(p_w)
            side = ops.wgrad_stream(dev) if (gW is not None and ops.WGRAD_SIDE) else None
        dx = None
        if ctx.needs_input_grad[0]:
            kw = {}
            if dskip is not None:
                kw['add'] = as_rows(dskip)
            if ctx.xsrc is not None and spec.takes_bnsrc:
                kw['bnsrc'] = ctx.xsrc
            if pre_v is not None:
                kw['pre_v'] = pre_v
            dx = spec.dgrad(spec, weight, draw, x, **kw)
        dW = None
        if ctx.needs_input_grad[1] and spec.custom_wgrad is not None:
            dW = spec.custom_wgrad(x, weight, draw)
        elif own_wgrad:
            dW = gW if gW is not None else torch.empty_like(weight)

            xw, lazy_w = x, ctx.lazy
            if lazy_w is not None and not ops.wgrad_lazy_capable(spec.mode, spec.C, Np, spec.launches[0][0]):
                xw, lazy_w = materialize(x, lazy_w), None

            def run_wgrad():
                x = xw
                for (geom, m), lay in zip(spec.launches, spec.layouts):
                    T = ops.taps_of(spec.T, geom)
                    dWp = torch.empty((Np, T, spec.C), dtype=torch.float32, device=dev)
                    ua = lay.fold_args()
                    done = ops.gather_wgrad(x, ld_of(x), spec.C, T, Np, m, draw, Np, dWp, mode=spec.mode, geom=geom,
                                            table=spec.table, unpack=None if ua is None else (dW,) + ua,
                                            lazy=lazy_w, pre_gy=pre_gy)
                    if not done:
                        lay.unpack(dWp, dW)
            if side is None:
                run_wgrad()
            else:
                side.wait_stream(torch.cuda.current_stream())
                x.record_stream(side)
                (draw if draw is not None else pre_gy).record_stream(side)
                with torch.cuda.stream(side):
                    run_wgrad()
            if gW is not None:
                dW = None
                delivered.append(dw_done if side is None else (lambda: dw_done(side)))
        if dres is not None and Np != N:
            dres = dres[..., :N]
        for done in delivered:
            done()
        return dx, dW, dbias, dgamma, dbeta, dres, None, None


class ConcatFn(torch.autograd.Function):

    @staticmethod
    def forward(ctx, buf, *parts):
        ctx.widths = [p.shape[-1] for p in parts]
        return buf.view_as(buf)

    @staticmethod
    def backward(ctx, g):
        outs, off = [], 0
        for w in ctx.widths:
            outs.append(g[..., off:off + w])
            off += w
        return (None,) + tuple(outs)


def concat(buf, parts):
    off, ok = 0, buf is not None
    for p in parts:
        ok = ok and p.shape[:-1] == buf.shape[:-1] and p.stride() == buf.stride() and \
            p.data_ptr() == buf.data_ptr() + 4 * off
        off += p.shape[-1]
    if ok and off == buf.shape[-1]:
        return ConcatFn.apply(buf, *parts)
    return torch.cat(parts, -1)


class MaxPool2Fn(torch.autograd.Function):
    @staticmethod
    def forward(ctx, x):
        x = x.contiguous()
        ctx.save_for_backward(x)
        return ops.maxpool2(x)

    @staticmethod
    def backward(ctx, dy):
        (x,) = ctx.saved_tensors
        B, H, W, C = x.shape
        dx = torch.zeros_like(x) if (H % 2 or W % 2) else torch.empty_like(x)
        ops.maxpool2_bwd(x, dy.contiguous(), dx)
        return dx


class SegmentColMaxFn(torch.autograd.Function):
    @staticmethod
    def forward(ctx, x, seg, nseg, C):
        x = as_rows(x)
        y, arg = ops.segment_colmax(x, ld_of(x), C, seg, nseg, want_arg=True)
        ctx.save_for_backward(arg)
        ctx.shape = (tuple(x.shape), C, nseg)
        return y

    @staticmethod
    def backward(ctx, dy):
        (arg,) = ctx.saved_tensors
        shape, C, nseg = ctx.shape
        dx = torch.zeros(shape, dtype=torch.float32, device=dy.device)
        ops.segment_colmax_bwd(dy.contiguous(), arg, nseg, C, dx, shape[-1])
        return dx, None, None, None


class SegmentColMeanFn(torch.autograd.Function):
    @staticmethod
    def forward(ctx, x, P, nseg, C):
        x = as_rows(x)
        ctx.meta = (tuple(x.shape), P, nseg, C)
        return ops.segment_colmean(x, ld_of(x), C, P, nseg)

    @staticmethod
    def backward(ctx, dy):
        shape, P, nseg, C = ctx.meta
        dx = torch.zeros(shape, dtype=torch.float32, device=dy.device)
        ops.segment_colmean_bwd(dy.contiguous(), P, nseg, C, dx, shape[-1])
        return dx, None, None, None


class SplatFn(torch.autograd.Function):

    @staticmethod
    def forward(ctx, feat, lv, Cf, use_emg=True, normalize=True):
        feat = as_rows(feat)
        splat, wsum = ops.splat_fwd(lv, feat, Cf, use_emg, normalize)
        ctx.save_for_backward(wsum)
        ctx.meta = (lv, Cf, feat.shape[-1], use_emg, normalize)
        return splat

    @staticmethod
    def backward(ctx, g):
        (wsum,) = ctx.saved_tensors
        lv, Cf, ldf, use_emg, normalize = ctx.meta
        gfeat = torch.zeros((lv.n_in, ldf), dtype=torch.float32, device=g.device) if ldf != Cf else \
            torch.empty((lv.n_in, Cf), dtype=torch.float32, device=g.device)
        ops.splat_bwd(lv, g.contiguous(), wsum, Cf, gfeat, use_emg, normalize)
        return gfeat, None, None, None, None


class Softmax2ToNchwFn(torch.autograd.Function):
    @staticmethod
    def forward(ctx, x):
        x = x.contiguous()
        y = ops.softmax2_to_nchw(x)
        ctx.save_for_backward(y)
        ctx.ld = x.shape[-1]
        return y

    @staticmethod
    def backward(ctx, dy):
        (y,) = ctx.saved_tensors
        B, _, H, W = y.shape
        dx = torch.empty((B, H, W, ctx.ld), dtype=torch.float32, device=dy.device)
        ops.softmax2_bwd(y, dy.contiguous(), dx)
        return dx


class HeadsToNchwFn(torch.autograd.Function):
    @staticmethod
    def forward(ctx, x):
        depth, mask = ops.heads_to_nchw(x.contiguous())
        ctx.save_for_backward(mask)
        ctx.set_materialize_grads(False)
        return depth, mask

    @staticmethod
    def backward(ctx, gd, gm):
        (mask,) = ctx.saved_tensors
        return ops.heads_bwd(mask, None if gm is None else gm.contiguous(), None if gd is None else gd.contiguous())


class NhwcToNchwFn(torch.autograd.Function):
    @staticmethod
    def forward(ctx, x, Cs):
        ctx.meta = (tuple(x.shape), Cs)
        return ops.nhwc_to_nchw(x.contiguous(), Cs)

    @staticmethod
    def backward(ctx, dy):
        shape, Cs = ctx.meta
        return ops.nchw_to_nhwc(dy.contiguous(), shape[-1]), None


class RangeImageFn(torch.autograd.Function):

    @staticmethod
    def forward(ctx, pc, e_l, H, W, fov_up, fov_down):
        img, pix = ops.range_image(pc, e_l, H, W, fov_up, fov_down)
        ctx.save_for_backward(pc, e_l, pix)
        ctx.hw = (H, W)
        return img

    @staticmethod
    def backward(ctx, g):
        pc, e_l, pix = ctx.saved_tensors
        H, W = ctx.hw
        B, _, N = pc.shape
        ge = ops.raster_pose_bwd(pix, g.contiguous(), pc, e_l.detach(), B, N, H * W, 0).view(B, 4, 4)
        return None, ge, None, None, None, None


class DepthImageFn(torch.autograd.Function):

    @staticmethod
    def forward(ctx, pc, P, H, W):
        img, pix = ops.depth_image(pc, P, H, W)
        ctx.save_for_backward(pc, pix)
        ctx.hw = (H, W)
        return img

    @staticmethod
    def backward(ctx, g):
        pc, pix = ctx.saved_tensors
        H, W = ctx.hw
        B, _, N = pc.shape
        gP = ops.raster_pose_bwd(pix, g.contiguous(), pc, None, B, N, H * W, 1).view(B, 3, 4)
        return None, gP, None, None


class CorrHeadFn(torch.autograd.Function):

    @staticmethod
    def forward(ctx, cam, rng):
        cam, rng = cam.contiguous(), rng.contiguous()
        score, logit, rp, cam_mm, rng_mm = ops.corr_head(cam, rng, want_logit=True, want_aux=True)
        ctx.save_for_backward(cam, rng, rp, cam_mm, rng_mm, score)
        return score

    @staticmethod
    def backward(ctx, ds):
        cam, rng, rp, cam_mm, rng_mm, score = ctx.saved_tensors
        B, h, wc, C = cam.shape
        wr = rng.shape[2]
        off = int(wr / 8)
        dl = (ds * score * (1 - score) / 16.0).contiguous()
        dcam_n, drp = ops.corr1d_bwd(rp, cam, cam_mm, dl, B, h, wc, wr + 2 * off)
        drng_n = ops.corr_unpad(drp, B, h, wr, C, off)

        return ops.norm_bwd(cam, dcam_n.contiguous(), cam_mm), ops.norm_bwd(rng, drng_n.contiguous(), rng_mm)


class GImageLossFn(torch.autograd.Function):

# ... 16 lines not shown
```

efgh_amd/ops.py:

```python
import ctypes
import os as _os
import threading
import weakref

import torch

from . import _C
from ._C import c_float, c_int32, c_int64, ptr

ACT_NONE, ACT_RELU, ACT_LEAKY = 0, 1, 2


def _L():
    return _C.lib()


def _st():
    return _C.stream_ptr()


def ceil4(n):
    return (n + 3) // 4 * 4


# ... 214 lines not shown
    for i in ent[1]:
        ref, key = jobs[i]
        w = ref()
        if w is None or not w.is_cuda or w.device != device or epoch_of(w) is not holder:
            continue
        c = w.__dict__.get('_efgh_cache', {}).get(key)
        if c is not None and c[0] != _ver(w):
            return True
    return False


def pack_weight(w, N, T, C, sn, sc, st, taps=None, Np=None, Cp=None, key=None):
    Np = Np or N
    Cp = Cp or C
    prm = (N, T, C, Np, Cp, sn, sc, st, None if taps is None else tuple(int(t) for t in taps))
    wd = w.detach()
    _C.require_cuda(wd)
    if key is None or not wd.is_contiguous():
        out = torch.empty((Np, T, Cp), dtype=torch.float32, device=wd.device)
        _pack_one(wd.contiguous(), out, prm)
        return out
    key = tuple(key)
    store = w.__dict__.setdefault('_efgh_cache', {})
    ent = store.get(key)
    cur = _ver(w)
    if ent is not None and ent[0] == cur:
        return ent[1]
    if ent is None or getattr(ent[1], '_efgh_pack', None) != prm:
        buf = torch.empty((Np, T, Cp), dtype=torch.float32, device=wd.device)
        buf._efgh_pack = prm
        _pack_one(wd, buf, prm)
        store[key] = (cur, buf)
        buf._efgh_holder = epoch_of(w)
        with _LOCK:
            jl = buf._efgh_holder.jobs
            if len(jl) >= 1024 and len(jl) % 256 == 0:
                jl[:] = [j for j in jl if j[0]() is not None]
            jl.append((weakref.ref(w), key))
        return buf
    if BATCH_PACK and _same_storage(ent[0], cur):
        _repack_all(wd.device, epoch_of(w))
        ent = store[key]
        if ent[0] == cur:
            return ent[1]
    _pack_one(wd, ent[1], prm)
    store[key] = (cur, ent[1])
    if getattr(ent[1], '_efgh_holder', None) is not epoch_of(w):
        ent[1]._efgh_holder = epoch_of(w)
        with _LOCK:
            ent[1]._efgh_holder.jobs.append((weakref.ref(w), key))
    return ent[1]


class WeightLayout:
    __slots__ = ('N', 'T', 'C', 'sn', 'sc', 'st', 'taps', 'Np', 'Cp', 'key')

    def __init__(self, N, T, C, sn, sc, st, taps, Np=None, Cp=None, key=None):
        self.N, self.T, self.C, self.sn, self.sc, self.st, self.taps = N, T, C, sn, sc, st, taps
        self.Np, self.Cp, self.key = Np or N, Cp or C, key

    def pack(self, w):
        return pack_weight(w, self.N, self.T, self.C, self.sn, self.sc, self.st, self.taps, Np=self.Np, Cp=self.Cp, key=self.key)

    def unpack(self, dWp, dW):
        unpack_weight(dWp, dW, self.N, self.T, self.C, self.Cp, self.sn, self.sc, self.st, self.taps)

    def fold_args(self):
        return (self.N, self.T, self.C, self.Cp, self.sn, self.sc, self.st, self.taps, False)


def pad_vec(v, Np, fill=0.0):
    if v is None or v.numel() == Np:
        return v
    v = v.detach()
    if not v.is_cuda or v.dtype != torch.float32 or not v.is_contiguous():
        out = torch.full((Np,), fill, dtype=torch.float32, device=v.device)
        out[:v.numel()] = v
        return out
    out = torch.empty((Np,), dtype=torch.float32, device=v.device)
    _C.check(_L().efgh_pad_vec(ptr(v), c_int32(v.numel()), ptr(out), c_int32(Np), c_float(fill), _st()))
    return out


def gemm_grid_m(M, N):
    return _L().efgh_gather_gemm_grid_m(c_int64(M), c_int32(N))


USE_WINO = True


def wino_eligible(mode, C, N, geom):
    if not USE_WINO or mode != 1 or geom is None or C % 16 or N % 64:
        return False
    (B, Hin, Win, Hv, Wv, sh, sw, dh, dw, Ho, Wo, osh, osw, oh0, ow0) = geom
    return (len(dh) == 9 and (sh, sw, osh, osw, oh0, ow0) == (1, 1, 1, 1, 0, 0) and Hv == Hin == Ho and Wv == Win == Wo
            and list(dh) == [t // 3 - 1 for t in range(9)] and list(dw) == [t % 3 - 1 for t in range(9)])


USE_WINO2D = True
WINO2D_MIN_C = 128
WINO2D_MIN_C_WGRAD = 128
WINO2D_MIN_C_TRAIN = 128


def _pow2(v):
    return v > 0 and (v & (v - 1)) == 0


def wino2d_eligible(mode, C, N, geom, wgrad=False):
    if not USE_WINO2D or not wino_eligible(mode, C, N, geom):
        return False
    lim = WINO2D_MIN_C_WGRAD if wgrad else (min(WINO2D_MIN_C, WINO2D_MIN_C_TRAIN) if TLS.train_step else WINO2D_MIN_C)
    if geom[1] < 8 or geom[2] < 8:
        return False
    return min(C, N) >= lim and _pow2(C // 4) and _pow2(N // 4) and C <= 512 and N <= 512


def wino2d_weight(Wp, N, C):
    def make():
        U = torch.empty((36, N, C), dtype=torch.float32, device=Wp.device)
        _C.check(_L().efgh_wino2d_pack(ptr(Wp), ptr(U), c_int32(N), c_int32(C), _st()))
        return U
    return _cached(Wp, ('wino2d',), _ver(Wp), make)


USE_C4 = True


def c4_eligible(mode, C, N, geom, wgrad=False):
    if not USE_C4 or mode != 1 or geom is None or C != 4:
        return False
    if (N % 16 or not 32 <= N <= 128) if wgrad else N not in (32, 64, 128):
        return False
    (B, Hin, Win, Hv, Wv, sh, sw, dh, dw, Ho, Wo, osh, osw, oh0, ow0) = geom
    return (len(dh) == 9 and sh == sw and sh in (1, 2) and (osh, osw, oh0, ow0) == (1, 1, 0, 0) and Hv == Ho and Wv == Wo
            and list(dh) == [t // 3 - 1 for t in range(9)] and list(dw) == [t % 3 - 1 for t in range(9)])


USE_SMALLC = True


SC_MIN_PIXELS_32 = 60000


def sc_eligible(mode, C, N, geom, wgrad=False):
    if not USE_SMALLC or mode != 1 or geom is None:
        return False
    (B, Hin, Win, Hv, Wv, sh, sw, dh, dw, Ho, Wo, osh, osw, oh0, ow0) = geom
    if not ((sh, sw, osh, osw, oh0, ow0) == (1, 1, 1, 1, 0, 0) and Hv == Hin == Ho and Wv == Win == Wo):
        return False
    if len(dh) == 1:
        return (C, N) in ((64, 32), (32, 64)) and dh[0] == 0 and dw[0] == 0
    if C == 32 and N == 32 and not wgrad and Hin * Win < SC_MIN_PIXELS_32:
        return False
    return (C in (16, 32) and N in (16, 32) and len(dh) == 9
            and list(dh) == [t // 3 - 1 for t in range(9)] and list(dw) == [t % 3 - 1 for t in range(9)])


def _sc_aligned(d, lda, ldo, residual, ldr, stats):
    ok = (lda % 4 == 0 and ldo % 4 == 0 and d.A % 16 == 0 and d.out % 16 == 0
          and (residual is None or (ldr % 4 == 0 and d.residual % 16 == 0)))
    if not ok and stats is not None:
        raise _C.EfghError('16- / 32-channel layer with BatchNorm statistics on a channel slice that is not 16-byte aligned')
    return ok


def wino_weight(Wp, N, C):
    def make():
        U = torch.empty((3 * C // 16, 6, N, 16), dtype=torch.float32, device=Wp.device)
        _C.check(_L().efgh_wino_pack(ptr(Wp), ptr(U), c_int32(N), c_int32(C), _st()))
        return U
    return _cached(Wp, ('wino',), _ver(Wp), make)


USE_THIN = True

def thin_eligible(mode, C, N, T):
    if not USE_THIN or mode != 1 or N % 4 or C % 4:
        return False
    if C == 4 and N <= 16 and T in (1, 2, 4, 9) and T * N * 16 + 4 * 64 * 36 * 4 <= 64 * 1024:
        return True
    return N == 4 and T * C * 16 <= 60 * 1024


def conv_bytes(M, N, T, C):
    return 4.0 * (float(M) * (C + N) + float(N) * T * C)


RIDGE_FLOP_PER_BYTE = 30.0


def hbm_bound(M, N, T, C):
    return 2.0 * M * N * T * C / conv_bytes(M, N, T, C) < RIDGE_FLOP_PER_BYTE


PROFILE_DED = None
TRACE_THIN = None
PROFILE_WINO = None
PROFILE = None


KSPLIT_MAX_ROWS = 16384


def gemm_route(mode, C, N, T, geom, M, stats=False, M_dev=False, batch=False, pool=False, plain=True, aligned=True):
    if mode == MODE_BLUR_R:
        return 'blur_r'
    if (KSPLIT_MAX_ROWS and mode == 2 and M <= KSPLIT_MAX_ROWS and T == 15 and N % 4 == 0 and T * C >= 1024 and plain
            and not (stats or M_dev or batch)):
        return 'ksplit'
    if not (stats or M_dev) and thin_eligible(mode, C, N, T):
        return 'thin'
    if M_dev or batch:
        return 'gemm'
    if c4_eligible(mode, C, N, geom):
        return 'c4'
    if aligned and sc_eligible(mode, C, N, geom):
        return 'sc'
    if wino2d_eligible(mode, C, N, geom):
        return 'wino2d'
    if wino_eligible(mode, C, N, geom):
        return 'wino_hpool' if pool == 'h' else 'wino'
    return 'gemm'


def wgrad_route(mode, C, N, T, geom, aligned=True):
    if mode == MODE_BLUR_R:
        return 'blur_r'
    if aligned and C == 4 and N == 4 and T == 9 and mode == 1:
        return 'c4n4'
    if thin_eligible(mode, C, N, T) and (N == 4 or (T in (1, 2, 4, 9) and _pow2(N // 4))):
        return 'thin'
    if (aligned and USE_SMALLC and C == 4 and N in (32, 64) and geom is not None and geom[5] == 1
            and sc_eligible(mode, 16, 16, geom, wgrad=True)):
        return 'sc_c4'
    if c4_eligible(mode, C, N, geom, wgrad=True):
        return 'c4'
    if aligned and sc_eligible(mode, C, N, geom, wgrad=True):
        return 'sc'
    if USE_WINO_WGRAD and wino2d_eligible(mode, C, N, geom, wgrad=True):
        return 'wino2d'
    if USE_WINO_WGRAD and C % 64 == 0 and wino_eligible(mode, C, N, geom):
        return 'wino'
    return 'gemm'


def stats_rows(mode, C, N, geom, M):
    route = gemm_route(mode, C, N, 1 if geom is None else len(geom[7]), geom, M, stats=True)
    if route == 'sc':
        return _L().efgh_sc_stats_rows(c_int32(geom[0]), c_int32(geom[1]), c_int32(geom[2]))
    if route == 'c4':
        return _L().efgh_c4_stats_rows(c_int32(geom[0]), c_int32(geom[9]), c_int32(geom[10]))
    if route == 'wino2d':
        return _L().efgh_wino2d_stats_rows(c_int32(geom[0]), c_int32(geom[1]), c_int32(geom[2]), c_int32(N))
    if route == 'wino':
        return _L().efgh_wino_grid_m(c_int32(geom[0]), c_int32(geom[1]), c_int32(geom[2]))
    return gemm_grid_m(M, N)


def taps_of(T, geom):
    return T if geom is None else len(geom[7])


def no_stats_epilogue(mode, C, N, T, launches):
    return all(gemm_route(mode, C, N, taps_of(T, g), g, m) == 'thin' for g, m in launches)


def _desc(A, lda, C, T, mode, N, M, geom=None, table=None, a_off=0, Wp=None, out=None, ldo=0, out_off=0, bias=None, scale=None,
          shift=None, residual=None, ldr=0, res_off=0, act=ACT_NONE, slope=0.0, stats=None, M_dev=None, batch=None):
    d = _C.GemmDesc()
    if A is not None:
        d.A = A.data_ptr() + 4 * a_off
    d.lda, d.C, d.T, d.mode, d.N, d.M = lda, C, T, mode, N, M
    if geom is not None:
        (d.B, d.Hin, d.Win, d.Hv, d.Wv, d.sh, d.sw, dh, dw, d.Ho, d.Wo, d.osh, d.osw, d.oh0, d.ow0) = geom
        for i, (a, b) in enumerate(zip(dh, dw)):
            d.dh[i], d.dw[i] = a, b
    for field, t in (('table', table), ('W', Wp), ('bias', bias), ('scale', scale), ('shift', shift), ('stats', stats), ('M_dev', M_dev)):
        if t is not None:
            setattr(d, field, t.data_ptr())
    if out is not None:
        d.out, d.ldo = out.data_ptr() + 4 * out_off, ldo
    if residual is not None:
        d.residual = residual.data_ptr() + 4 * res_off
    d.ldr, d.act, d.slope = ldr, act, slope
    if batch is not None:
        d.nbatch, d.batch_stride_a, d.batch_stride_w, d.batch_stride_out = batch[:4]
        if len(batch) > 4:
            d.batch_stride_table = batch[4]
    return d


_DEDICATED = ('thin', 'c4', 'c4n4', 'sc_c4')


def _prof_start(on):
    if on is None:
        return None
    ev = (torch.cuda.Event(enable_timing=True), torch.cuda.Event(enable_timing=True))
    ev[0].record()
    return ev


def _prof_end(ev, route, shape, flops, plain, wino_list=None, batched=False):
    if ev is None:
        return
    ev[1].record()
    if route in ('blur_r', 'planes'):
        plain.append(ev + (flops, shape))
        return
    nbytes = conv_bytes(*shape[1:])
    if PROFILE_DED is not None and (route in _DEDICATED or route == 'sc'):
        PROFILE_DED.append(ev + (nbytes, shape))
    wino = route in ('wino2d', 'wino', 'wino_hpool')
    if route in _DEDICATED or (not wino and not batched and hbm_bound(*shape[1:])):
        if PROFILE_THIN is not None:
            PROFILE_THIN.append(ev + (nbytes, shape))
    elif route == 'wino2d' and PROFILE_WINO2D is not None:
        PROFILE_WINO2D.append(ev + (flops, shape))
    else:
        (wino_list if (wino and wino_list is not None) else plain).append(ev + (flops, shape))


def _blur_gemm_ksplit(A, lda, C, Wp, N, M, out, ldo, table, bias, act, slope, a_off, out_off, flops, alias_mask=False):
    S, Ts = 5, 3
    dev = out.device

    def regroup():
        return Wp.view(N, S, Ts * C).permute(1, 0, 2).contiguous()
    Wg = _cached(Wp, ('ksplit', S), _ver(Wp), regroup)
    part = _scratch(S * M * N, dev)
    gather_gemm(A, lda, C, Ts, Wg, N, M, part, N, mode=2, table=table, a_off=a_off, batch=(S, 0, N * Ts * C, M * N, Ts),
                flops=flops if flops is not None else 2.0 * M * N * 15 * C, alias_mask=alias_mask)
    b = None
    if bias is not None:
        b = bias if bias.numel() == N else None
        assert b is not None
    _C.check(_L().efgh_fold_planes(ptr(part), c_int32(S), c_int64(M), c_int32(N), ptr(b), c_int32(act), c_float(slope),
                                   _C.c_void_p(out.data_ptr() + 4 * out_off), c_int64(ldo), _st()))


def gather_gemm(A, lda, C, T, Wp, N, M, out, ldo, mode=0, geom=None, table=None, bias=None, scale=None,
                shift=None, residual=None, ldr=0, act=ACT_NONE, slope=0.0, stats=None, a_off=0, out_off=0,
                res_off=0, M_dev=None, flops=None, batch=None, alias_mask=False, bn_bwd=None, pool=False, lazy=None, pre_v=None):
    key = (mode, C, N, T, geom, M, stats is not None, M_dev is not None, batch is not None, pool,
           scale is None and shift is None and residual is None and (bias is None or bias.numel() == N))
    route = gemm_route(*key)
    if (lazy is not None or pre_v is not None) and not (route == 'wino2d' and min(C, N) >= 64):
        raise _C.EfghError('gather_gemm(lazy= / pre_v=) on a launch the 2-D Winograd path does not serve (ask lazy_capable() first)')
    if route == 'blur_r':
        if (geom is not None or batch is not None or M_dev is not None or scale is not None or shift is not None or residual is not None
                or stats is not None or alias_mask or pool or bn_bwd is not None):
            raise _C.EfghError('gather_gemm(mode=MODE_BLUR_R) takes a plain blur launch: bias and activation only')
        blur_r_gemm(A, lda, C, T, Wp, N, M, out, ldo, table, bias=bias, act=act, slope=slope, a_off=a_off, out_off=out_off, flops=flops)
        return None
    if route == 'ksplit':
        return _blur_gemm_ksplit(A, lda, C, Wp, N, M, out, ldo, table, bias, act, slope, a_off, out_off, flops, alias_mask)
    d = _desc(A, lda, C, T, mode, N, M, geom, table, a_off, Wp, out, ldo, out_off, bias, scale, shift, residual, ldr, res_off, act, slope,
              stats, M_dev, batch)
    d.table_alias_mask = 1 if (alias_mask and mode == 2) else 0
    if route == 'sc' and not _sc_aligned(d, lda, ldo, residual, ldr, stats):
        route = gemm_route(*key, aligned=False)
    if pool and route not in ('c4', 'wino2d', 'wino_hpool'):
        raise _C.EfghError('gather_gemm(pool=True) on a launch no pooling epilogue serves (ask pool_fusable() first)')
    ev = _prof_start(PROFILE)
    bn_stats = None
    if route == 'thin':
        if TRACE_THIN is not None:
            TRACE_THIN.append(int(_L().efgh_thin_supported(ctypes.byref(d))))
        _C.check(_L().efgh_thin_gemm(ctypes.byref(d), _st()))
    elif route == 'c4':
        assert lda % 4 == 0
        _C.check((_L().efgh_c4_conv3x3_pooled if pool else _L().efgh_c4_conv3x3)(ctypes.byref(d), _st()))
    elif route == 'sc':
        _C.check(_L().efgh_sc_conv3x3(ctypes.byref(d), _st()))
    elif route == 'wino2d':
        if (bn_bwd is not None and stats is None and BN_BWD_FUSED_2D and out_off == 0 and not pool and bn_bwd.fits(M, N)
                and bn_bwd.y is None and bn_bwd.raw.stride(-2) % 4 == 0):
            rows = _L().efgh_wino2d_stats_rows(c_int32(geom[0]), c_int32(geom[1]), c_int32(geom[2]), c_int32(N))
            bn_stats = _bn_bwd_sums(d, bn_bwd, rows, N, out.device)
        _wino2d_forward(d, A, a_off, lda, C, N, geom, Wp, pool=pool, lazy=lazy, pre_v=pre_v)
    elif route == 'wino_hpool':
        _C.check(_L().efgh_wino_conv3x3_hpool(ctypes.byref(d), ptr(wino_weight(Wp, N, C)), _st()))
    elif route == 'wino':
        if bn_bwd is not None and stats is None and BN_BWD_FUSED and out_off == 0 and bn_bwd.fits(M, N):
            rows = _L().efgh_wino_grid_m(c_int32(geom[0]), c_int32(geom[1]), c_int32(geom[2]))
            bn_stats = _bn_bwd_sums(d, bn_bwd, rows, N, out.device)
        _C.check(_L().efgh_wino_conv3x3(ctypes.byref(d), ptr(wino_weight(Wp, N, C)), _st()))
    else:
        _C.check(_L().efgh_gather_gemm(ctypes.byref(d), _st()))
    if ev is not None:
        _prof_end(ev, route, (mode, M, N, T, C), float(flops) if flops is not None else 2.0 * M * N * T * C, PROFILE, PROFILE_WINO,
                  batched=batch is not None)
    return bn_stats


def _bn_bwd_sums(d, src, rows, N, device):
    part = torch.empty((rows, 2, N), dtype=torch.float32, device=device)
    d.stats, d.stats_mode = part.data_ptr(), 1
    d.bn_raw, d.bn_ldraw = src.raw.data_ptr(), src.raw.stride(-2)
    if src.y is not None:
        d.bn_y, d.bn_ldy = src.y.data_ptr(), src.y.stride(-2)
    else:
        d.bn_pscale, d.bn_pshift = src.psc.data_ptr(), src.psh.data_ptr()
    d.bn_mean, d.bn_invstd = src.mean.data_ptr(), src.invstd.data_ptr()
    d.bn_act, d.bn_slope = src.act, src.slope
    return part


GEMM_DMA = True


def apply_switches():
    _L().efgh_gather_gemm_set_dma(c_int32(1 if GEMM_DMA else 0))


PLANE_DMA = True
PLANE_DMA_NBUF = 0
PROFILE_WINO2D = None
PROFILE_WINO2D_GEMM = None
PLANES_SPLIT = None
PLANE_SPLIT_HITS = [0, 0]


def planes_split_active():
    if PLANES_SPLIT is not None:
        return bool(PLANES_SPLIT)
    return torch.backends.cuda.matmul.fp32_precision == 'tf32'


def _planes_split_now():
    m = TLS.planes_split
    return planes_split_active() if m is None else m


def _batched_plain_gemm(A3, W3, out3, rows, C, N):
    g = _desc(A3, 36 * C, C, 1, 0, N, rows, Wp=W3, out=out3, ldo=36 * N, batch=(36, C, N * C, N))
    ev = _prof_start(PROFILE_WINO2D_GEMM)
    if PLANE_DMA and _L().efgh_plane_gemm_supported(ctypes.byref(g)):
        if _planes_split_now():
            PLANE_SPLIT_HITS[0] += 1
            _C.check(_L().efgh_plane_gemm_x6(ctypes.byref(g), c_int32(PLANE_DMA_NBUF), _st()))
        else:
            _C.check(_L().efgh_plane_gemm(ctypes.byref(g), c_int32(PLANE_DMA_NBUF), _st()))
    else:
        _C.check(_L().efgh_gather_gemm(ctypes.byref(g), _st()))
    _prof_end(ev, 'planes', (0, rows, N, 36, C), 2.0 * 36 * rows * C * N, PROFILE_WINO2D_GEMM)


W2V_CACHE = {}
W2V_KEEP = True


def w2v_clear():
    me = threading.get_ident()
    with _LOCK:
        for k in [k for k, v in W2V_CACHE.items() if v[2] == me]:
            del W2V_CACHE[k]


POOL_FUSED = True
POOL_HALF = True


def pool_fusable(mode, C, N, geom, residual=None, stats=None):
    if not (POOL_FUSED and residual is None and stats is None and geom is not None and geom[1] >= 2 and geom[2] >= 2):
        return False
    route = gemm_route(mode, C, N, len(geom[7]), geom, geom[0] * geom[3] * geom[4], pool='h')
    if route == 'c4':
        return geom[5] == 1 and geom[6] == 1
    if route == 'wino2d':
        return True
    return 'h' if (route == 'wino_hpool' and POOL_HALF) else False


class LazyAct:
    __slots__ = ('scale', 'shift', 'act', 'slope')

    def __init__(self, scale, shift, act, slope):
        self.scale, self.shift, self.act, self.slope = scale, shift, act, slope


LAZY_ACT = True
W2_BWD_FUSED = True
W2_BWD_FUSED_POOL = True
LAZY_HITS = [0, 0]


def lazy_capable(mode, C, N, geom):
    return geom is not None and min(C, N) >= 64 and gemm_route(mode, C, N, len(geom[7]), geom, 0) == 'wino2d'


def wino2d_input(A, a_off, lda, C, B, H, W, V, lazy=None):
    if lazy is None:
        _C.check(_L().efgh_wino2d_input(_C.c_void_p(A.data_ptr() + 4 * a_off), c_int64(lda), c_int32(C), c_int32(B), c_int32(H),
                                        c_int32(W), ptr(V), _st()))
    else:
        LAZY_HITS[0] += 1
        _C.check(_L().efgh_wino2d_input_act(_C.c_void_p(A.data_ptr() + 4 * a_off), c_int64(lda), c_int32(C), c_int32(B), c_int32(H),
                                            c_int32(W), ptr(lazy.scale), ptr(lazy.shift), c_int32(lazy.act), c_float(lazy.slope),
                                            ptr(V), _st()))


def wino2d_bwd_transforms(dy, lddy, raw, ldraw, ybits, psc, psh, mean, invstd, coef, m1, m2, N, B, H, W, act, slope, want_dres):
    T2 = _L().efgh_wino2d_tiles(c_int32(B), c_int32(H), c_int32(W))
    dev = raw.device
    Vd = torch.empty((T2, 36, N), dtype=torch.float32, device=dev)
    Gy = torch.empty((T2, 36, N), dtype=torch.float32, device=dev)
    dres = torch.empty((B, H, W, N), dtype=torch.float32, device=dev) if want_dres else None
    LAZY_HITS[1] += 1
    _C.check(_L().efgh_wino2d_bwd_transforms(ptr(dy), c_int64(lddy), ptr(raw), c_int64(ldraw), ptr(ybits), ptr(psc), ptr(psh), ptr(mean),
                                             ptr(invstd), ptr(coef), ptr(m1), ptr(m2), c_int32(N), c_int32(B), c_int32(H), c_int32(W),
                                             c_int32(act), c_float(slope), ptr(Vd), ptr(Gy), ptr(dres), c_int64(N), _st()))
    return Vd, Gy, dres


def _wino2d_forward(d, A, a_off, lda, C, N, geom, Wp, pool=False, lazy=None, pre_v=None):
    B, H, W = geom[0], geom[1], geom[2]
    T = _L().efgh_wino2d_tiles(c_int32(B), c_int32(H), c_int32(W))
    dev = A.device if A is not None else pre_v.device
    Mb = torch.empty((T, 36, N), dtype=torch.float32, device=dev)
    if pre_v is not None:
        assert tuple(pre_v.shape) == (T, 36, C)
        V = pre_v
    else:
        V = torch.empty((T, 36, C), dtype=torch.float32, device=dev)
        wino2d_input(A, a_off, lda, C, B, H, W, V, lazy)
    if pre_v is None and W2V_KEEP and TLS.w2v_wanted and a_off == 0:
        with _LOCK:
            if len(W2V_CACHE) > 512:
                W2V_CACHE.clear()
            W2V_CACHE[(A.data_ptr(), lda, C, B, H, W)] = (V, A._version, threading.get_ident())
    _batched_plain_gemm(V, wino2d_weight(Wp, N, C), Mb, T, C, N)
    if pool:
        _C.check(_L().efgh_wino2d_output_pooled(ptr(Mb), ctypes.byref(d), _st()))
    else:
        _C.check(_L().efgh_wino2d_output(ptr(Mb), ctypes.byref(d), _st()))


def bn_finalize(stats, G, C, count, gamma, beta, rmean, rvar, momentum, eps, save=False):
    dev = stats.device
    scale = torch.empty(C, dtype=torch.float32, device=dev)
    shift = torch.empty(C, dtype=torch.float32, device=dev)
    sm = torch.empty(C, dtype=torch.float32, device=dev) if save else None
    si = torch.empty(C, dtype=torch.float32, device=dev) if save else None
    _C.check(_L().efgh_bn_finalize(ptr(stats), c_int32(G), c_int32(C), ctypes.c_double(count), ptr(gamma), ptr(beta),
                                   ptr(rmean), ptr(rvar), c_float(momentum), c_float(eps), ptr(scale), ptr(shift),
                                   ptr(sm), ptr(si), _st()))
    return scale, shift, sm, si


def col_stats(x, M, C, ld, x_off=0):
    G = _L().efgh_col_stats_groups(c_int64(M))
    stats = torch.empty((G, 2, C), dtype=torch.float32, device=x.device)
    _C.check(_L().efgh_col_stats(_C.c_void_p(x.data_ptr() + 4 * x_off), c_int64(M), c_int32(C), c_int64(ld),
                                 ptr(stats), _st()))
    return stats, G


def scale_shift_act(x, ldx, scale, shift, y, ldy, M, C, act=ACT_NONE, slope=0.0, res=None, ldr=0, x_off=0,
                    y_off=0, res_off=0, bits=None):
    if bits is not None:
        _C.check(_L().efgh_scale_shift_act_bits(
            _C.c_void_p(x.data_ptr() + 4 * x_off), c_int64(ldx), ptr(scale), ptr(shift),
            _C.c_void_p(0 if res is None else res.data_ptr() + 4 * res_off), c_int64(ldr),
            _C.c_void_p(y.data_ptr() + 4 * y_off), c_int64(ldy), ptr(bits), c_int64(M), c_int32(C), c_int32(act), c_float(slope),
            _st()))
        return
    _C.check(_L().efgh_scale_shift_act(
        _C.c_void_p(x.data_ptr() + 4 * x_off), c_int64(ldx), ptr(scale), ptr(shift),
        _C.c_void_p(0 if res is None else res.data_ptr() + 4 * res_off), c_int64(ldr),
        _C.c_void_p(y.data_ptr() + 4 * y_off), c_int64(ldy), c_int64(M), c_int32(C), c_int32(act), c_float(slope),
        _st()))


def maxpool2(x):
    B, H, W, C = x.shape
    y = torch.empty((B, H // 2, W // 2, C), dtype=torch.float32, device=x.device)
    _C.check(_L().efgh_maxpool2(ptr(x), ptr(y), c_int32(B), c_int32(H), c_int32(W), c_int32(C), _st()))
    return y


def maxpool_v2(x):
    B, H, W, C = x.shape
    y = torch.empty((B, H // 2, W, C), dtype=torch.float32, device=x.device)
    _C.check(_L().efgh_maxpool_v2(ptr(x), ptr(y), c_int32(B), c_int32(H), c_int32(W), c_int32(C), _st()))
    return y


def maxpool2_affine(raw, scale, shift, act, slope=0.0):
    B, H, W, C = raw.shape
    y = torch.empty((B, H // 2, W // 2, C), dtype=torch.float32, device=raw.device)
    _C.check(_L().efgh_maxpool2_affine(ptr(raw), ptr(scale), ptr(shift), c_int32(act), c_float(slope), ptr(y), c_int32(B),
                                       c_int32(H), c_int32(W), c_int32(C), _st()))
    return y


def maxpool2_bwd_affine(raw, scale, shift, act, slope, dy):
    B, H, W, C = raw.shape
    dx = torch.zeros_like(raw) if (H % 2 or W % 2) else torch.empty_like(raw)
    _C.check(_L().efgh_maxpool2_bwd_affine(ptr(raw), ptr(scale), ptr(shift), c_int32(act), c_float(slope), ptr(dy), ptr(dx),
                                           c_int32(B), c_int32(H), c_int32(W), c_int32(C), _st()))
    return dx


def nchw_to_nhwc(x, Cd=None):
    _C.require_cuda(x)
    x = x.contiguous()
    B, Cs = x.shape[0], x.shape[1]
    sp = tuple(x.shape[2:])
    HW = 1
    for s in sp:
        HW *= s
    Cd = Cd or Cs
# ... 199 lines not shown
    def fold_args(self):
        return None


def blur_r_dgrad(lv, draw, C0, w, C):
    from .lattice import filter_offsets
    H = lv.H
    Wd = blur_r_pack(w, filter_offsets(lv.radius)[1])
    dx = torch.empty((H, C), dtype=torch.float32, device=draw.device)
    blur_r_gemm(draw, draw.stride(0), C0, lv.F, Wd, C, H, dx, C, lv.nbr, flops=2.0 * H * lv.F * C * C0, hit=1)
    return dx


def range_image(pc, e_l, H, W, fov_up, fov_down):
    _C.require_cuda(pc, e_l)
    pc, e_l = pc.contiguous(), e_l.detach().contiguous()
    B, _, N = pc.shape
    dev = pc.device
    pix = torch.empty((B, N), dtype=torch.int32, device=dev)
    vals = torch.empty((B, N, 4), dtype=torch.float32, device=dev)
    win = torch.empty((B, H * W), dtype=torch.int32, device=dev)
    img = torch.empty((B, H, W, 4), dtype=torch.float32, device=dev)
    _C.check(_L().efgh_range_image(ptr(pc), ptr(e_l), c_int32(B), c_int32(N), c_int32(H), c_int32(W),
                                   ctypes.c_double(fov_up), ctypes.c_double(fov_down), ptr(pix), ptr(vals),
                                   ptr(win), ptr(img), _st()))
    return img, pix


def depth_image(pc, cam_T_velo, H, W):
    _C.require_cuda(pc, cam_T_velo)
    pc, P = pc.contiguous(), cam_T_velo.detach().contiguous()
    B, _, N = pc.shape
    dev = pc.device
    pix = torch.empty((B, N), dtype=torch.int32, device=dev)
    vals = torch.empty((B, N, 4), dtype=torch.float32, device=dev)
    win = torch.empty((B, H * W), dtype=torch.int32, device=dev)
    img = torch.empty((B, H, W, 4), dtype=torch.float32, device=dev)
    _C.check(_L().efgh_depth_image(ptr(pc), ptr(P), c_int32(B), c_int32(N), c_int32(H), c_int32(W), ptr(pix),
                                   ptr(vals), ptr(win), ptr(img), _st()))
    return img, pix


def rotate_nearest_u8(img, rot_deg, want_nchw=True, want_nhwc4=True):
    _C.require_cuda(img, rot_deg)
    img = img.detach().contiguous()
    B, _, H, W = img.shape
    o1 = torch.empty((B, 3, H, W), dtype=torch.float32, device=img.device) if want_nchw else None
    o2 = torch.empty((B, H, W, 4), dtype=torch.float32, device=img.device) if want_nhwc4 else None
    _C.check(_L().efgh_rotate_nearest_u8(ptr(img), ptr(rot_deg.detach().contiguous().float()), c_int32(B), c_int32(H),
                                         c_int32(W), ptr(o1), ptr(o2), _st()))
    return o1, o2


def minmax(x):
    B = x.shape[0]
    n = x.numel() // B
    G = _L().efgh_minmax_groups(c_int64(n))
    part = torch.empty((B, G, 2), dtype=torch.float32, device=x.device)
    mm = torch.empty((B, 2), dtype=torch.float32, device=x.device)
    _C.check(_L().efgh_minmax(ptr(x), c_int32(B), c_int64(n), ptr(part), ptr(mm), _st()))
    return mm


USE_MFMA_CORR = True


def corr_head(cam, rng, want_logit=False, want_aux=False):
    B, h, wc, C = cam.shape
    wr = rng.shape[2]
    assert C == 16 and rng.shape[1] == h
    off = int(wr / 8)
    wp = wr + 2 * off
    nj = wp - wc + 1
    dev = cam.device
    cam_mm, rng_mm = minmax(cam), minmax(rng)
    score = torch.empty((B, nj), dtype=torch.float32, device=dev)
    logit = torch.empty((B, nj), dtype=torch.float32, device=dev) if want_logit else None
    segw = (wc + 31) // 32
    nseg = ceil4((wc + segw - 1) // segw)
    mfma = USE_MFMA_CORR and (not want_aux or h * 16 >= 128) and h * segw * 16 < 65536 and nseg <= 32
    wpitch = wp + segw if mfma else wp
    rp = torch.empty((B, h, wpitch, C), dtype=torch.float32, device=dev)
    _C.check(_L().efgh_corr_pad(ptr(rng), ptr(rng_mm), c_int32(B), c_int32(h), c_int32(wr), c_int32(C),
                                c_int32(off), c_int32(wpitch), ptr(rp), _st()))
    if mfma:
        nsplit = max(d for d in range(1, 17) if h % d == 0)
        T = h // nsplit
        nseg_real = (wc + segw - 1) // segw
        Wc = torch.empty((B, nsplit, nseg, T, segw * 16), dtype=torch.float32, device=dev)
        _C.check(_L().efgh_corr_pack_cam(ptr(cam), ptr(cam_mm), c_int32(B), c_int32(h), c_int32(wc), c_int32(segw),
                                         c_int32(nseg), c_int32(nsplit), ptr(Wc), _st()))
        P = torch.empty((B, nsplit, wp, nseg), dtype=torch.float32, device=dev)
        geom = (1, T, wpitch, 1, wp, 1, 1, [], [], 1, wp, 1, 1, 0, 0)
        gather_gemm(rp, 16, segw * 16, T, Wc, nseg, wp, P, nseg, mode=3, geom=geom, flops=2.0 * B * nj * h * wc * 16,
                    batch=(B * nsplit, T * wpitch * 16, nseg * T * segw * 16, wp * nseg))
        _C.check(_L().efgh_corr_fold(ptr(P), c_int32(B), c_int32(nsplit), c_int64(wp), c_int32(nseg),
                                     c_int32(nseg_real), c_int32(segw), c_int32(nj), ptr(logit), ptr(score), _st()))
        if want_aux:
            return score, logit, rp, cam_mm, rng_mm
        return score, logit
    part = torch.empty((B, h, nj), dtype=torch.float32, device=dev)
    _C.check(_L().efgh_corr1d(ptr(rp), ptr(cam), ptr(cam_mm), c_int32(B), c_int32(h), c_int32(wc), c_int32(wp),
                              ptr(part), ptr(logit), ptr(score), _st()))
    if want_aux:
        return score, logit, rp, cam_mm, rng_mm
    return score, logit


PROFILE_WGRAD = None
PROFILE_WINO_WGRAD = None
PROFILE_THIN = None
USE_WINO_WGRAD = True


_SCRATCH = {}
WGRAD_SIDE = _os.environ.get('EFGH_WGRAD_STREAM', '1') != '0'


def wgrad_stream(device):
    from .nets import efghbackbone as bb
    return bb._side_stream(device, 2)


def reserve_comm_queue():
    global WGRAD_SIDE
    if _os.environ.get('EFGH_WGRAD_STREAM') is None:
        WGRAD_SIDE = False


def side_streams():
    from .nets import efghbackbone as bb
    return list(bb._SIDE.values())
DETERMINISTIC = False


def _scratch(nfloats, device):
    nfloats = int(nfloats)
    if nfloats <= 0:
        return None
    key = (device.index, _C.stream_ptr().value, threading.get_ident())
    t = _SCRATCH.get(key)
    if t is None or t.numel() < nfloats:
        t = _SCRATCH[key] = torch.empty(max(nfloats, 1 << 22), dtype=torch.float32, device=device)
    return t


FOLD_UNPACK = True
FOLD_UNPACK_HITS = [0]


def wgrad_lazy_capable(mode, C, N, geom):
    return geom is not None and min(C, N) >= 64 and wgrad_route(mode, C, N, len(geom[7]), geom) == 'wino2d'


_WGRAD_ENTRY = {'c4n4': ('efgh_c4n4_wgrad', 'efgh_c4n4_wgrad_workspace'), 'thin': ('efgh_thin_wgrad', 'efgh_thin_wgrad_workspace'),
                'sc_c4': ('efgh_sc_wgrad', 'efgh_sc_wgrad_workspace'), 'c4': ('efgh_c4_wgrad', 'efgh_c4_wgrad_workspace'),
                'sc': ('efgh_sc_wgrad', 'efgh_sc_wgrad_workspace'), 'gemm': ('efgh_gather_wgrad', 'efgh_gather_wgrad_workspace')}


def _wgrad_aligned(route, d, lda, ldg, G, dWp):
    if route == 'c4n4':
        return lda % 4 == 0 and ldg % 4 == 0 and dWp.data_ptr() % 16 == 0 and _L().efgh_c4n4_supported(ctypes.byref(d))
    return lda % 4 == 0 and ldg % 4 == 0 and d.A % 16 == 0 and G.data_ptr() % 16 == 0


def gather_wgrad(A, lda, C, T, N, M, G, ldg, dWp, mode=0, geom=None, table=None, unpack=None, lazy=None, pre_gy=None):
    route = wgrad_route(mode, C, N, T, geom)
    if (lazy is not None or pre_gy is not None) and not (route == 'wino2d' and min(C, N) >= 64):
        raise _C.EfghError('gather_wgrad(lazy= / pre_gy=) on a launch the 2-D Winograd weight gradient does not serve')
    if route == 'blur_r':
        blur_r_wgrad(A, lda, C, T, N, M, G, ldg, dWp, table)
        return False
    od = None
    if unpack is not None and FOLD_UNPACK and unpack[4] % 4 == 0 and unpack[2] <= 16:
        dW_, n_, t_, c_, cp_, sn_, sc_, st_, taps_, acc_ = unpack
        od = _C.WgradOutDesc()
        od.W, od.N, od.T, od.C, od.Cp, od.sn, od.sc, od.st = dW_.data_ptr(), n_, t_, c_, cp_, sn_, sc_, st_
        for i_, t__ in enumerate(taps_):
            od.taps[i_] = int(t__)
        od.accumulate = 1 if acc_ else 0
    odp = None if od is None else ctypes.byref(od)
    ev = _prof_start(PROFILE_WGRAD)
    d = _desc(A, lda, C, T, mode, N, M, geom, table)
    if route in ('c4n4', 'sc_c4', 'sc') and not _wgrad_aligned(route, d, lda, ldg, G, dWp):
        route = wgrad_route(mode, C, N, T, geom, aligned=False)
    if route == 'wino2d':
        B, H, W = geom[0], geom[1], geom[2]
        T2 = _L().efgh_wino2d_tiles(c_int32(B), c_int32(H), c_int32(W))
        dev = dWp.device
        with _LOCK:
            kept = W2V_CACHE.pop((A.data_ptr(), lda, C, B, H, W), None)
        if kept is not None:
            kept[0].record_stream(torch.cuda.current_stream())
        S = torch.empty((36, N, C), dtype=torch.float32, device=dev)
        if kept is not None and kept[1] == A._version and kept[0].shape == (T2, 36, C):
            V = kept[0]
        else:
            V = torch.empty((T2, 36, C), dtype=torch.float32, device=dev)
            wino2d_input(A, 0, lda, C, B, H, W, V, lazy)
        if pre_gy is not None:
            assert tuple(pre_gy.shape) == (T2, 36, N)
            Gy = pre_gy
        else:
            Gy = torch.empty((T2, 36, N), dtype=torch.float32, device=dev)
            _C.check(_L().efgh_wino2d_dy(ptr(G), c_int64(ldg), c_int32(N), c_int32(B), c_int32(H), c_int32(W), ptr(Gy), _st()))
        g = _desc(V, 36 * C, C, 1, 0, N, T2, batch=(36, C, 0, 0))
        pv = _prof_start(PROFILE_WINO2D_GEMM)
        if PLANE_DMA and _L().efgh_plane_wgrad_supported(ctypes.byref(g), c_int64(36 * N)):
            split = _planes_split_now()
            if split:
                PLANE_SPLIT_HITS[1] += 1
            fn = _L().efgh_plane_wgrad_x6_batched if split else _L().efgh_plane_wgrad_batched
            _C.check(fn(ctypes.byref(g), ptr(Gy), c_int64(36 * N), c_int64(N), ptr(S), c_int64(N * C),
                        ptr(_scratch(_L().efgh_plane_wgrad_workspace(ctypes.byref(g)), dev)), c_int32(PLANE_DMA_NBUF), _st()))
        else:
            _C.check(_L().efgh_gather_wgrad_batched(ctypes.byref(g), ptr(Gy), c_int64(36 * N), c_int64(N), ptr(S), c_int64(N * C),
                                                    ptr(_scratch(_L().efgh_gather_wgrad_workspace(ctypes.byref(g)), dev)), _st()))
        _prof_end(pv, 'planes', (0, T2, N, 36, C), 2.0 * 36 * T2 * C * N, PROFILE_WINO2D_GEMM)
        done = _C.check_wrote(_L().efgh_wino2d_wfinish(ptr(S), ptr(dWp), c_int32(N), c_int32(C), odp, _st()))
    elif route == 'wino':
        S = _scratch(_L().efgh_wino_wgrad_workspace(ctypes.byref(d)), dWp.device)
        done = _C.check_wrote(_L().efgh_wino_wgrad(ctypes.byref(d), ptr(G), c_int64(ldg), ptr(S), ptr(dWp), odp, _st()))
    else:
        entry, workspace = _WGRAD_ENTRY[route]
        S = _scratch(getattr(_L(), workspace)(ctypes.byref(d)), dWp.device)
        done = _C.check_wrote(getattr(_L(), entry)(ctypes.byref(d), ptr(G), c_int64(ldg), ptr(dWp), ptr(S), odp, _st()))
    if done:
        FOLD_UNPACK_HITS[0] += 1
    if ev is not None:
        _prof_end(ev, route, (mode, M, N, T, C), 2.0 * M * N * T * C, PROFILE_WGRAD, PROFILE_WINO_WGRAD)
    return done


def unpack_weight(Wp, W, N, T, C, Cp, sn, sc, st, taps, accumulate=False):
    tp = (ctypes.c_int32 * 16)(*([int(t) for t in taps] + [0] * (16 - len(taps))))
    _C.check(_L().efgh_unpack_weight(ptr(Wp), ptr(W), c_int32(N), c_int32(T), c_int32(C), c_int32(Cp), c_int64(sn),
                                     c_int64(sc), c_int64(st), tp, c_int32(1 if accumulate else 0), _st()))


def table_scatter_add(src, table, M, T, C, dst):
    _C.check(_L().efgh_table_scatter_add(ptr(src), ptr(table), c_int64(M), c_int32(T), c_int32(C), ptr(dst), _st()))


def bwd_groups(M):
    return _L().efgh_bwd_groups(c_int64(M))


def act_bn_bwd_reduce(dy, lddy, y, ldy, raw, ldraw, mean, invstd, M, C, act, slope, part, s1, s2, m1, m2,
                      pscale=None, pshift=None):
    _C.check(_L().efgh_act_bn_bwd_reduce(ptr(dy), c_int64(lddy), ptr(y), c_int64(ldy), ptr(raw), c_int64(ldraw),
                                         ptr(mean), ptr(invstd), ptr(pscale), ptr(pshift), c_int64(M), c_int32(C),
                                         c_int32(act),
                                         c_float(slope), ptr(part), ptr(s1), ptr(s2), ptr(m1), ptr(m2), _st()))


POOL_REDUCE_FROM_Y = True


def pool_bn_bwd(dy_pool, raw, mean, invstd, coef, pscale, pshift, act, slope, s1=None, s2=None, transforms=False, y_pool=None):
    B, H, W, C = raw.shape
    dev = raw.device
    s1 = s1 if s1 is not None else torch.empty(C, dtype=torch.float32, device=dev)
    s2 = s2 if s2 is not None else torch.empty(C, dtype=torch.float32, device=dev)
    m1 = torch.empty(C, dtype=torch.float64, device=dev)
    m2 = torch.empty(C, dtype=torch.float64, device=dev)
    if (POOL_REDUCE_FROM_Y and y_pool is not None and act == ACT_RELU and y_pool.is_contiguous()
            and tuple(y_pool.shape) == (B, H // 2, W // 2, C)):
        G = _L().efgh_bwd_groups(c_int64(B * (H // 2) * (W // 2)))
        part = torch.empty((G, 2, C), dtype=torch.float64, device=dev)
        _C.check(_L().efgh_pool_bn_bwd_reduce_pooled(ptr(dy_pool), ptr(y_pool), ptr(raw), ptr(mean), ptr(invstd), ptr(pscale), ptr(pshift),
                                                     c_int32(B), c_int32(H), c_int32(W), c_int32(C), ptr(part), ptr(s1), ptr(s2), ptr(m1),
                                                     ptr(m2), _st()))
    else:
        G = _L().efgh_pool_bwd_groups(c_int32(B), c_int32(H), c_int32(W))
        part = torch.empty((G, 2, C), dtype=torch.float64, device=dev)
        _C.check(_L().efgh_pool_bn_bwd_reduce(ptr(dy_pool), ptr(raw), ptr(mean), ptr(invstd), ptr(pscale), ptr(pshift), c_int32(B),
                                              c_int32(H), c_int32(W), c_int32(C), c_int32(act), c_float(slope), ptr(part), ptr(s1),
                                              ptr(s2), ptr(m1), ptr(m2), _st()))
    if transforms:
        T2 = _L().efgh_wino2d_tiles(c_int32(B), c_int32(H), c_int32(W))
        Vd = torch.empty((T2, 36, C), dtype=torch.float32, device=dev)
        Gy = torch.empty((T2, 36, C), dtype=torch.float32, device=dev)
        LAZY_HITS[1] += 1
        _C.check(_L().efgh_wino2d_bwd_transforms_pooled(ptr(dy_pool), c_int64(C), ptr(raw), c_int64(C), ptr(pscale), ptr(pshift), ptr(mean),
                                                        ptr(invstd), ptr(coef), ptr(m1), ptr(m2), c_int32(C), c_int32(B), c_int32(H),
                                                        c_int32(W), c_int32(act), c_float(slope), ptr(Vd), ptr(Gy), _st()))
        return (Vd, Gy), s1, s2
    draw = torch.empty_like(raw)
    _C.check(_L().efgh_pool_bn_bwd_apply(ptr(dy_pool), ptr(raw), ptr(mean), ptr(invstd), ptr(coef), ptr(m1), ptr(m2), ptr(pscale),
                                         ptr(pshift), c_int32(B), c_int32(H), c_int32(W), c_int32(C), c_int32(act),
                                         c_float(slope), ptr(draw), _st()))
    return draw, s1, s2


def act_bn_bwd_apply(dy, lddy, y, ldy, raw, ldraw, mean, invstd, coef, m1, m2, M, C, act, slope, draw, lddraw,
                     dres, lddres, pscale=None, pshift=None):
    _C.check(_L().efgh_act_bn_bwd_apply(ptr(dy), c_int64(lddy), ptr(y), c_int64(ldy), ptr(raw), c_int64(ldraw),
                                        ptr(mean), ptr(invstd), ptr(coef), ptr(m1), ptr(m2), ptr(pscale), ptr(pshift),
                                        c_int64(M), c_int32(C),
                                        c_int32(act), c_float(slope), ptr(draw), c_int64(lddraw), ptr(dres),
                                        c_int64(lddres), _st()))


def col_sum(x, M, C):
    stats, G = col_stats(x, M, C, x.shape[-1])
    return stats[:, 0, :].sum(0)


def maxpool2_bwd(x, dy, dx):
    B, H, W, C = x.shape
    _C.check(_L().efgh_maxpool2_bwd(ptr(x), ptr(dy), ptr(dx), c_int32(B), c_int32(H), c_int32(W), c_int32(C), _st()))


def segment_colmax_bwd(dy, arg, nseg, C, dx, ld):
    _C.check(_L().efgh_segment_colmax_bwd(ptr(dy), ptr(arg), c_int32(nseg), c_int32(C), ptr(dx), c_int64(ld), _st()))


def segment_colmean_bwd(dy, P, nseg, C, dx, ld):
    _C.check(_L().efgh_segment_colmean_bwd(ptr(dy), c_int32(P), c_int32(nseg), c_int32(C), ptr(dx), c_int64(ld),
                                           _st()))


def softmax2_bwd(y, dy, dx):
    B, _, H, W = y.shape
    _C.check(_L().efgh_softmax2_bwd(ptr(y), ptr(dy), c_int32(B), c_int64(H * W), ptr(dx), c_int64(dx.shape[-1]),
                                    _st()))


def raster_bwd(pix, gimg, B, N, HW):
    gv = torch.empty((B, N, 4), dtype=torch.float32, device=gimg.device)
    _C.check(_L().efgh_raster_bwd(ptr(pix), ptr(gimg), c_int32(B), c_int32(N), c_int64(HW), ptr(gv), _st()))
    return gv


def raster_pose_bwd(pix, gimg, pc, e_l, B, N, HW, mode):
    _C.require_cuda(pix, gimg, pc)
    pc = pc.contiguous()
    part = torch.empty((B, 64, 16), dtype=torch.float64, device=gimg.device)
    out = torch.empty((B, 16 if mode == 0 else 12), dtype=torch.float32, device=gimg.device)
    _C.check(_L().efgh_raster_pose_bwd(ptr(pix), ptr(gimg), ptr(pc), ptr(None if e_l is None else e_l.contiguous()), c_int32(B),
                                       c_int32(N), c_int64(HW), c_int32(mode), ptr(part), ptr(out), _st()))
    return out


def corr1d_bwd_mfma(rp, cam, cam_mm, dl, B, h, wc, wp, rp_pitch=None):
    dev = cam.device
    nj = wp - wc + 1
    rp_pitch = rp_pitch or wp
    wpP, wcP = ceil4(wp), ceil4(wc)
    f = lambda *shape: torch.empty(shape, dtype=torch.float32, device=dev)
    rpT, camT = f(B, h * 16, wpP), f(B, h * 16, wcP)
    _C.check(_L().efgh_corr_planes(ptr(rp), None, c_int32(B), c_int32(h), c_int32(wp), c_int32(rp_pitch), c_int32(wpP),
                                   ptr(rpT), _st()))
    _C.check(_L().efgh_corr_planes(ptr(cam), ptr(cam_mm), c_int32(B), c_int32(h), c_int32(wc), c_int32(wc), c_int32(wcP),
                                   ptr(camT), _st()))
    T, TT = f(B, wc, wpP), f(B, wp, wcP)
    _C.check(_L().efgh_corr_toeplitz(ptr(dl), c_int32(B), c_int32(nj), c_int32(wc), c_int32(wp), c_int32(wpP), c_int32(0),
                                     ptr(T), _st()))
    _C.check(_L().efgh_corr_toeplitz(ptr(dl), c_int32(B), c_int32(nj), c_int32(wp), c_int32(wc), c_int32(wcP), c_int32(1),
                                     ptr(TT), _st()))
    dcamT, drpT = f(B, h * 16, wc), f(B, h * 16, wp)
    M = h * 16
    gather_gemm(rpT, wpP, wpP, 1, T, wc, M, dcamT, wc, mode=0, flops=2.0 * B * h * wc * 16 * nj,
                batch=(B, M * wpP, wc * wpP, M * wc))
    gather_gemm(camT, wcP, wcP, 1, TT, wp, M, drpT, wp, mode=0, flops=2.0 * B * h * wc * 16 * nj,
                batch=(B, M * wcP, wp * wcP, M * wp))
    dcam, drp = f(B, h, wc, 16), f(B, h, wp, 16)
    _C.check(_L().efgh_corr_unplanes(ptr(dcamT), c_int32(B), c_int32(h), c_int32(wc), c_int32(wc), ptr(dcam), _st()))
    _C.check(_L().efgh_corr_unplanes(ptr(drpT), c_int32(B), c_int32(h), c_int32(wp), c_int32(wp), ptr(drp), _st()))
    return dcam, drp


def corr1d_bwd(rp, cam, cam_mm, dl, B, h, wc, wp):
    pitch = rp.shape[2]
    if (USE_MFMA_CORR and h * 16 >= 128) or pitch != wp:
        return corr1d_bwd_mfma(rp, cam, cam_mm, dl, B, h, wc, wp, rp_pitch=pitch)
    dcam = torch.empty_like(cam)
    drp = torch.empty_like(rp)
    _C.check(_L().efgh_corr1d_bwd(ptr(rp), ptr(cam), ptr(cam_mm), ptr(dl), c_int32(B), c_int32(h), c_int32(wc),
                                  c_int32(wp), ptr(dcam), ptr(drp), _st()))
    return dcam, drp


def norm_bwd(x, dxn, mm):
    B = x.shape[0]
    n = x.numel() // B
    G = _L().efgh_minmax_groups(c_int64(n))
    part = torch.empty((B, G, 3), dtype=torch.float32, device=x.device)
    dx = torch.empty_like(x)
    _C.check(_L().efgh_norm_bwd(ptr(x), ptr(dxn), ptr(mm), c_int32(B), c_int64(n), ptr(part), ptr(dx), _st()))
    return dx


def corr_unpad(drp, B, h, w, C, off):
    dx = torch.empty((B, h, w, C), dtype=torch.float32, device=drp.device)
    _C.check(_L().efgh_corr_unpad(ptr(drp), c_int32(B), c_int32(h), c_int32(w), c_int32(C), c_int32(off), ptr(dx),
                                  _st()))
    return dx


def convt_col2im(Y, B, Hin, Win, Ho, Wo, O, pad, scale, shift, act, slope, out):
    _C.check(_L().efgh_convt_col2im(ptr(Y), c_int64(Y.shape[-1]), c_int32(B), c_int32(Hin), c_int32(Win), c_int32(Ho),
                                    c_int32(Wo), c_int32(O), c_int32(pad), ptr(scale), ptr(shift), c_int32(act),
                                    c_float(slope), ptr(out), c_int64(out.shape[-1]), _st()))


def convt_im2col(G, B, Hin, Win, Ho, Wo, O, pad, Ycol):
    _C.check(_L().efgh_convt_im2col(ptr(G), c_int64(G.shape[-1]), c_int32(B), c_int32(Hin), c_int32(Win), c_int32(Ho),
                                    c_int32(Wo), c_int32(O), c_int32(pad), ptr(Ycol), c_int64(Ycol.shape[-1]), _st()))


def gimg_loss_fwd(pred_depth, pred_mask, gdep4, img_mask):
    B, _, H, W = pred_depth.shape
    dev = pred_depth.device
    gt_depth = torch.empty((B, 1, H, W), dtype=torch.float32, device=dev)
    gt_mask = torch.empty((B, 1, H, W), dtype=torch.float32, device=dev)
    G = _L().efgh_gimg_loss_groups(c_int64(B * H * W))
    part = torch.empty((G, 3), dtype=torch.float64, device=dev)
    out3 = torch.empty(3, dtype=torch.float32, device=dev)
    _C.check(_L().efgh_gimg_loss_fwd(ptr(pred_depth), ptr(pred_mask), c_int64(pred_mask.stride(0)), ptr(gdep4), ptr(img_mask),
                                     c_int32(B), c_int64(H * W), ptr(gt_depth), ptr(gt_mask), ptr(part), ptr(out3), _st()))
    return out3, gt_depth, gt_mask


def gimg_loss_bwd(pred_depth, pred_mask, gt_depth, img_mask, out3, g_depth, g_mask):
    B, _, H, W = pred_depth.shape
    d_depth = torch.empty_like(pred_depth)
    d_mask = torch.zeros_like(pred_mask)
    _C.check(_L().efgh_gimg_loss_bwd(ptr(pred_depth), ptr(pred_mask), c_int64(pred_mask.stride(0)), ptr(gt_depth), ptr(img_mask),
                                     c_int32(B), c_int64(H * W), ptr(out3), ptr(g_depth), ptr(g_mask), ptr(d_depth), ptr(d_mask),
                                     c_int64(d_mask.stride(0)), _st()))
    return d_depth, d_mask
```

include/efgh_hip.h:

```cpp
#ifndef EFGH_HIP_H
#define EFGH_HIP_H
#include <stdint.h>

#ifdef __cplusplus
extern "C" {
#endif

#define EFGH_OK 0
#define EFGH_E_INVALID (-1)
#define EFGH_E_LAUNCH (-2)
#define EFGH_WROTE_OUT 1

const char *efgh_last_error(void);

#define EFGH_ABI_VERSION 4
int efgh_version(void);

#define EFGH_LATTICE_INFO_H 0
#define EFGH_LATTICE_INFO_ERR 1
#define EFGH_LATTICE_INFO_ALIAS 2
#define EFGH_LATTICE_INFO_CURSOR 3
#define EFGH_LATTICE_INFO_SEG 4
#define EFGH_LATTICE_MAX_SAMPLES 1024

int64_t efgh_lattice_hash_capacity(int32_t n_cap);
int64_t efgh_lattice_workspace_bytes(int32_t n_cap, int32_t h_cap, int32_t nsamples);

int efgh_lattice_level_build(const float *pts, int64_t pts_cstride, const int32_t *n_dev, int32_t n_cap,
                             const int32_t *sid, int32_t pts_per_sample, int32_t nsamples, float scale32,
                             float div32, float *bary, float *emg, int32_t *off, int32_t *list, int32_t h_cap,
                             int32_t *vseg, float *pts_next, int32_t *vsid, int32_t *info, void *workspace,
                             int64_t hash_slots, void *stream);

int efgh_lattice_level_neighbors(const void *workspace, int32_t n_cap, int32_t h_cap_build, int32_t nsamples,
                                 int32_t *info, const int32_t *vsid, int32_t h_cap, int32_t *nbr, int32_t *alist,
                                 int32_t alias_cap, int64_t hash_slots, void *stream);

int32_t efgh_lattice_part_max_entries(int32_t n_cap);
int64_t efgh_lattice_part_list_len(int32_t n_cap, int32_t nbuckets);
int32_t efgh_lattice_part_buckets(int32_t n_cap);
int64_t efgh_lattice_part_workspace_bytes(int32_t n_cap, int32_t h_cap, int32_t nsamples, int32_t nbuckets, int32_t slots);
int64_t efgh_lattice_part_zeroed_bytes(int32_t n_cap);
int efgh_lattice_part_build(const float *pts, int64_t pts_cstride, const int32_t *n_dev, int32_t n_cap,
                            const int32_t *sid, int32_t pts_per_sample, int32_t nsamples, float scale32,
                            float *bary, float *emg, int32_t *list, int32_t h_cap, int32_t *info, void *workspace,
                            void *zeroed, int32_t nbuckets, int32_t slots, int32_t want_off, int32_t big_buckets, void *stream);
int efgh_lattice_part_neighbors(const void *workspace, const float *pts, int64_t pts_cstride, const int32_t *n_dev,
                                int32_t n_cap, const int32_t *sid, int32_t pts_per_sample, int32_t nsamples,
                                float scale32, float div32, int32_t h_cap_build, int32_t *info, int32_t h_cap,
                                int32_t *nbr, int32_t *alist, int32_t alias_cap, int32_t *off, int32_t *vseg,
                                float *pts_next, int32_t *vsid, int32_t nbuckets, int32_t slots, void *stream);

int efgh_splat_gather(const float *emg, const float *feat, int64_t ldf, int32_t Cf, const float *bary,
                      const int32_t *list, const int32_t *vseg, int32_t H, int32_t avg_len, int32_t lanes_per_vertex,
                      int32_t normalize, float *splat, float *wsum, void *stream);
int efgh_splat_bwd(const float *gsplat, int32_t C, int32_t coff, const float *wsum, int32_t Cf, const float *bary,
                   const int32_t *off, int32_t n, float *gfeat, int64_t ldg, int32_t normalize, void *stream);
int efgh_table_gather_transposed(const float *src, const int32_t *nbr, int32_t H, int32_t C, const int32_t *alist,
                                 const int32_t *n_alias, int32_t alias_cap, float *dst, void *stream);
int efgh_blur_dgrad_alias(const float *dy, int64_t ldy, int32_t N, const float *w, int32_t C, const int32_t *alist,
                          const int32_t *n_alias, int32_t alias_cap, float *dx, int64_t ldx, void *stream);

typedef struct {
    const float *A;
    int64_t lda;
    int32_t C;
    int32_t T;
    int32_t mode;
    int32_t B, Hin, Win, Hv, Wv, sh, sw;
    int8_t dh[16], dw[16];
    int32_t Ho, Wo, osh, osw, oh0, ow0;
    const int32_t *table;
    const float *W;
    int32_t N;
    int64_t M;
    const int32_t *M_dev;
    const float *bias, *scale, *shift;
    const float *residual; int64_t ldr;
    int32_t act;
    float slope;
    float *out; int64_t ldo;
    float *stats;
    int32_t nbatch;
    int64_t batch_stride_a, batch_stride_w, batch_stride_out;
    int32_t batch_stride_table;
    int32_t table_alias_mask;
    int32_t stats_mode;
    const float *bn_raw; int64_t bn_ldraw;
    const float *bn_y; int64_t bn_ldy;
    const float *bn_pscale, *bn_pshift, *bn_mean, *bn_invstd;
    int32_t bn_act; float bn_slope;
} efgh_gemm_desc;

int efgh_gather_gemm(const efgh_gemm_desc *d, void *stream);
int efgh_bwd_finalize_f32(const float *stats, int32_t rows, int32_t C, double count, float *sum_dpre, float *sum_dpre_xhat,
                          double *mean_dpre, double *mean_dpre_xhat, void *stream);
int32_t efgh_gather_gemm_grid_m(int64_t M, int32_t N);

int efgh_pack_weight(const float *W, float *Wp, int32_t N, int32_t T, int32_t C, int64_t sn,
                     int64_t sc, int64_t st, const int32_t *tapidx_host, void *stream);
int efgh_pack_weight_padded(const float *W, float *Wp, int32_t N, int32_t T, int32_t C, int32_t Np, int32_t Cp, int64_t sn,
                            int64_t sc, int64_t st, const int32_t *tapidx_host, void *stream);
typedef struct {
    const float *W; float *Wp;
    int32_t N, T, C, Np, Cp, pad_;
    int64_t sn, sc, st;
    int32_t taps[16];
} efgh_pack_job;
int efgh_pack_weight_batched(const efgh_pack_job *jobs_dev, const int64_t *prefix_dev, int32_t njobs, int64_t total, void *stream);
int efgh_pack_weight_batched_tiled(const efgh_pack_job *jobs_dev, const int64_t *tile_prefix_dev, int32_t njobs, int64_t ntiles,
                                   void *stream);
int efgh_fold_planes(const float *part, int32_t S, int64_t M, int32_t N, const float *bias, int32_t act, float slope, float *out,
                     int64_t ldo, void *stream);
int efgh_pad_vec(const float *v, int32_t n, float *out, int32_t np, float fill, void *stream);


int efgh_bn_finalize(const float *stats, int32_t G, int32_t C, double count, const float *gamma,
                     const float *beta, float *rmean, float *rvar, float momentum, float eps,
                     float *scale, float *shift, float *save_mean, float *save_invstd, void *stream);
int32_t efgh_col_stats_groups(int64_t M);
int efgh_col_stats(const float *x, int64_t M, int32_t C, int64_t ld, float *stats, void *stream);
int efgh_scale_shift_act(const float *x, int64_t ldx, const float *scale, const float *shift,
                         const float *res, int64_t ldr, float *y, int64_t ldy, int64_t M, int32_t C,
                         int32_t act, float slope, void *stream);
int efgh_scale_shift_act_bits(const float *x, int64_t ldx, const float *scale, const float *shift,
                              const float *res, int64_t ldr, float *y, int64_t ldy, uint32_t *bits, int64_t M, int32_t C,
                              int32_t act, float slope, void *stream);
int efgh_maxpool2(const float *x, float *y, int32_t B, int32_t H, int32_t W, int32_t C, void *stream);
int efgh_maxpool_v2(const float *x, float *y, int32_t B, int32_t H, int32_t W, int32_t C, void *stream);
int efgh_nchw_to_nhwc(const float *x, float *y, int32_t B, int32_t Cs, int64_t HW, int32_t Cd, void *stream);
int efgh_nhwc_to_nchw(const float *x, int64_t ld, float *y, int32_t B, int32_t Cs, int64_t HW, void *stream);
int efgh_segment_colmax(const float *x, int64_t ld, int32_t C, const int32_t *seg, int32_t nseg,
                        float *y, int32_t *argrow, void *stream);
int efgh_segment_colmean(const float *x, int64_t ld, int32_t C, int32_t rows_per_seg, int32_t nseg,
                         float *y, void *stream);
int64_t efgh_segment_workspace(int32_t C, int32_t nseg);
int efgh_segment_colmax_ws(const float *x, int64_t ld, int32_t C, const int32_t *seg, int32_t nseg, int64_t rows_hint, float *y,
                           int32_t *argrow, void *workspace, void *stream);
int efgh_segment_colmean_ws(const float *x, int64_t ld, int32_t C, int32_t rows_per_seg, int32_t nseg, float *y, void *workspace,
                            void *stream);
int efgh_softmax2_to_nchw(const float *x, int64_t ld, float *y, int32_t B, int64_t HW, void *stream);
int efgh_heads_to_nchw(const float *x, float *depth, float *mask, int32_t B, int64_t HW, void *stream);

int efgh_range_image(const float *pc, const float *e_l, int32_t B, int32_t N, int32_t H, int32_t W,
                     double fov_up, double fov_down, int32_t *pix, float *vals, int32_t *winner,
                     float *img, void *stream);
int efgh_depth_image(const float *pc, const float *cam_T_velo, int32_t B, int32_t N, int32_t H,
                     int32_t W, int32_t *pix, float *vals, int32_t *winner, float *img, void *stream);
int efgh_raster_bwd(const int32_t *pix, const float *gimg, int32_t B, int32_t N, int64_t HW,
                    float *gvals, void *stream);
int efgh_raster_pose_bwd(const int32_t *pix, const float *gimg, const float *pc, const float *e_l, int32_t B, int32_t N,
                         int64_t HW, int32_t mode, double *partials, float *g_pose, void *stream);
int efgh_rotate_nearest_u8(const float *img, const float *rot_deg, int32_t B, int32_t H, int32_t W,
                           float *out_nchw, float *out_nhwc4, void *stream);

int32_t efgh_minmax_groups(int64_t n);
int efgh_minmax(const float *x, int32_t B, int64_t n, float *part, float *mm, void *stream);
int efgh_corr_pad(const float *rng, const float *rng_mm, int32_t B, int32_t h, int32_t w, int32_t C,
                  int32_t off, int32_t wpitch, float *rp, void *stream);
int efgh_corr1d(const float *rp, const float *cam, const float *cam_mm, int32_t B, int32_t h,
                int32_t wc, int32_t wp, float *part, float *logit, float *score, void *stream);


typedef struct efgh_wgrad_out_desc {
    float *W;
    int32_t N, T, C, Cp;
    int64_t sn, sc, st;
    int32_t taps[16];
    int32_t accumulate;
} efgh_wgrad_out_desc;
int64_t efgh_gather_wgrad_workspace(const efgh_gemm_desc *d);
int efgh_gather_wgrad(const efgh_gemm_desc *d, const float *G, int64_t ldg, float *dWp, float *workspace,
                      const efgh_wgrad_out_desc *out, void *stream);
int efgh_gather_wgrad_batched(const efgh_gemm_desc *d, const float *G, int64_t ldg, int64_t batch_stride_g, float *dWp,
                              int64_t batch_stride_dw, float *workspace, void *stream);

int64_t efgh_lattice_neighbors_r_workspace(int32_t h_cap, int32_t nsamples);
int efgh_lattice_neighbors_r(const float *pts, int64_t pts_cstride, const int32_t *sid, int32_t pts_per_sample, int32_t nsamples,
                             float scale32, const int32_t *list, const int32_t *vseg, const int32_t *vsid, const int32_t *info,
                             int32_t h_cap, const int32_t *offsets, int32_t F, int32_t ld, int32_t *nbr, void *workspace,
                             void *stream);
int efgh_blur_r_gemm(const efgh_gemm_desc *d, int32_t ld, void *stream);
int efgh_blur_r_wgrad(const efgh_gemm_desc *d, int32_t ld, const float *G, int64_t ldg, float *dWp, float *workspace,
                      void *stream);

int efgh_wino2d_supported(const efgh_gemm_desc *d);
int64_t efgh_wino2d_tiles(int32_t B, int32_t H, int32_t W);
int32_t efgh_wino2d_stats_rows(int32_t B, int32_t H, int32_t W, int32_t N);
int efgh_wino2d_pack(const float *Wp, float *U, int32_t N, int32_t C, void *stream);
typedef struct efgh_wino_pack_job {
    const float *Wp;
    float *U;
    int32_t N, C, kind, pad_;
    int64_t first_block;
} efgh_wino_pack_job;
int efgh_wino_pack_batched(const efgh_wino_pack_job *jobs_dev, int32_t njobs, int64_t nblocks, void *stream);
int efgh_wino2d_input(const float *A, int64_t lda, int32_t C, int32_t B, int32_t H, int32_t W, float *V, void *stream);
int efgh_wino2d_input_act(const float *A, int64_t lda, int32_t C, int32_t B, int32_t H, int32_t W, const float *scale,
                          const float *shift, int32_t act, float slope, float *V, void *stream);
int efgh_wino2d_bwd_transforms(const float *dy, int64_t lddy, const float *raw, int64_t ldraw, const uint32_t *ybits,
                               const float *pscale, const float *pshift, const float *mean, const float *invstd, const float *coef,
                               const double *m1, const double *m2, int32_t N, int32_t B, int32_t H, int32_t W, int32_t act,
                               float slope, float *Vd, float *Gy, float *dres, int64_t lddres, void *stream);
int efgh_wino2d_bwd_transforms_pooled(const float *dy_pool, int64_t lddy, const float *raw, int64_t ldraw, const float *pscale,
                                      const float *pshift, const float *mean, const float *invstd, const float *coef,
                                      const double *m1, const double *m2, int32_t N, int32_t B, int32_t H, int32_t W, int32_t act,
                                      float slope, float *Vd, float *Gy, void *stream);
int efgh_wino2d_output(const float *M, const efgh_gemm_desc *d, void *stream);
int efgh_wino2d_output_pooled(const float *M, const efgh_gemm_desc *d, void *stream);
int efgh_wino2d_dy(const float *G, int64_t ldg, int32_t N, int32_t B, int32_t H, int32_t W, float *Gy, void *stream);
int efgh_wino2d_wfinish(const float *S, float *dWp, int32_t N, int32_t C, const efgh_wgrad_out_desc *out, void *stream);

int efgh_unpack_weight(const float *Wp, float *W, int32_t N, int32_t T, int32_t C, int32_t Cp, int64_t sn,
                       int64_t sc, int64_t st, const int32_t *tapidx_host, int32_t accumulate, void *stream);
int efgh_table_scatter_add(const float *src, const int32_t *table, int64_t M, int32_t T, int32_t C,
                           float *dst, void *stream);
int32_t efgh_bwd_groups(int64_t M);
int efgh_act_bn_bwd_reduce(const float *dy, int64_t lddy, const float *y, int64_t ldy, const float *raw,
                           int64_t ldraw, const float *mean, const float *invstd, const float *pscale,
                           const float *pshift, int64_t M, int32_t C,
                           int32_t act, float slope, double *part, float *sum_dpre, float *sum_dpre_xhat,
                           double *mean_dpre, double *mean_dpre_xhat, void *stream);
int efgh_act_bn_bwd_apply(const float *dy, int64_t lddy, const float *y, int64_t ldy, const float *raw,
                          int64_t ldraw, const float *mean, const float *invstd, const float *coef,
                          const double *m1, const double *m2, const float *pscale, const float *pshift,
                          int64_t M, int32_t C, int32_t act, float slope,
                          float *draw, int64_t lddraw, float *dres, int64_t lddres, void *stream);
int efgh_maxpool2_bwd(const float *x, const float *dy, float *dx, int32_t B, int32_t H, int32_t W, int32_t C,
                      void *stream);
int efgh_maxpool2_affine(const float *x, const float *scale, const float *shift, int32_t act, float slope, float *y,
                         int32_t B, int32_t H, int32_t W, int32_t C, void *stream);
int efgh_maxpool2_bwd_affine(const float *x, const float *scale, const float *shift, int32_t act, float slope,
                             const float *dy, float *dx, int32_t B, int32_t H, int32_t W, int32_t C, void *stream);
int32_t efgh_pool_bwd_groups(int32_t B, int32_t H, int32_t W);
int efgh_pool_bn_bwd_reduce(const float *dy_pool, const float *raw, const float *mean, const float *invstd, const float *pscale,
                            const float *pshift, int32_t B, int32_t H, int32_t W, int32_t C, int32_t act, float slope,
                            double *part, float *sum_dpre, float *sum_dpre_xhat, double *mean_dpre, double *mean_dpre_xhat,
                            void *stream);
int efgh_pool_bn_bwd_reduce_pooled(const float *dy_pool, const float *y_pool, const float *raw, const float *mean,
                                   const float *invstd, const float *pscale, const float *pshift, int32_t B, int32_t H, int32_t W,
                                   int32_t C, double *part, float *sum_dpre, float *sum_dpre_xhat, double *mean_dpre,
                                   double *mean_dpre_xhat, void *stream);
int efgh_pool_bn_bwd_apply(const float *dy_pool, const float *raw, const float *mean, const float *invstd, const float *coef,
                           const double *m1, const double *m2, const float *pscale, const float *pshift, int32_t B, int32_t H,
                           int32_t W, int32_t C, int32_t act, float slope, float *draw, void *stream);
int efgh_segment_colmax_bwd(const float *dy, const int32_t *argrow, int32_t nseg, int32_t C, float *dx,
                            int64_t ld, void *stream);
int efgh_segment_colmean_bwd(const float *dy, int32_t P, int32_t nseg, int32_t C, float *dx, int64_t ld,
                             void *stream);
int efgh_softmax2_bwd(const float *y, const float *dy, int32_t B, int64_t HW, float *dx, int64_t ld, void *stream);
int efgh_heads_bwd(const float *y, const float *dmask, const float *ddepth, int32_t B, int64_t HW, float *dx, void *stream);
int efgh_corr1d_bwd(const float *rp, const float *cam, const float *cam_mm, const float *dlogit, int32_t B,
                    int32_t h, int32_t wc, int32_t wp, float *dcam_n, float *drp, void *stream);
int efgh_corr_unpad(const float *drp, int32_t B, int32_t h, int32_t w, int32_t C, int32_t off, float *dx,
                    void *stream);

int efgh_adam_step(float *w, const float *g, float *m, float *v, int64_t n, float lr, float beta1,
                   float beta2, float eps, float weight_decay, int32_t step, float grad_scale, void *stream);

int efgh_thin_supported(const efgh_gemm_desc *d);
int efgh_thin_gemm(const efgh_gemm_desc *d, void *stream);
int64_t efgh_thin_wgrad_workspace(const efgh_gemm_desc *d);
int efgh_thin_wgrad(const efgh_gemm_desc *d, const float *G, int64_t ldg, float *dWp, float *workspace,
                    const efgh_wgrad_out_desc *out, void *stream);
int efgh_c4n4_supported(const efgh_gemm_desc *d);
int64_t efgh_c4n4_wgrad_workspace(const efgh_gemm_desc *d);
int efgh_c4n4_wgrad(const efgh_gemm_desc *d, const float *G, int64_t ldg, float *dWp, float *workspace,
                    const efgh_wgrad_out_desc *out, void *stream);

int efgh_sc_supported(const efgh_gemm_desc *d);
int32_t efgh_sc_stats_rows(int32_t B, int32_t H, int32_t W);
int efgh_sc_conv3x3(const efgh_gemm_desc *d, void *stream);
int efgh_sc_wgrad_supported(const efgh_gemm_desc *d);
int64_t efgh_sc_wgrad_workspace(const efgh_gemm_desc *d);
int efgh_sc_wgrad(const efgh_gemm_desc *d, const float *G, int64_t ldg, float *dWp, float *workspace,
                  const efgh_wgrad_out_desc *out, void *stream);
int efgh_c4_supported(const efgh_gemm_desc *d);
int32_t efgh_c4_stats_rows(int32_t B, int32_t Ho, int32_t Wo);
int efgh_c4_conv3x3(const efgh_gemm_desc *d, void *stream);
int efgh_c4_pooled_supported(const efgh_gemm_desc *d);
int efgh_c4_conv3x3_pooled(const efgh_gemm_desc *d, void *stream);
int efgh_c4_wgrad_supported(const efgh_gemm_desc *d);
int64_t efgh_c4_wgrad_workspace(const efgh_gemm_desc *d);
int efgh_c4_wgrad(const efgh_gemm_desc *d, const float *G, int64_t ldg, float *dWp, float *workspace,
                  const efgh_wgrad_out_desc *out, void *stream);

int efgh_debug_occupancy(char *out, int32_t cap);

int efgh_gather_gemm_set_dma(int32_t on);

int efgh_plane_gemm_supported(const efgh_gemm_desc *d);
int efgh_plane_gemm(const efgh_gemm_desc *d, int32_t nbuf, void *stream);
int efgh_plane_wgrad_supported(const efgh_gemm_desc *d, int64_t ldg);
int64_t efgh_plane_wgrad_workspace(const efgh_gemm_desc *d);
int efgh_plane_wgrad_batched(const efgh_gemm_desc *d, const float *G, int64_t ldg, int64_t batch_stride_g, float *dWp,
                             int64_t batch_stride_dw, float *workspace, int32_t nbuf, void *stream);

int efgh_plane_gemm_x6(const efgh_gemm_desc *d, int32_t nbuf, void *stream);
int efgh_plane_wgrad_x6_batched(const efgh_gemm_desc *d, const float *G, int64_t ldg, int64_t batch_stride_g, float *dWp,
                                int64_t batch_stride_dw, float *workspace, int32_t nbuf, void *stream);

int efgh_convt_col2im(const float *Y, int64_t ldy, int32_t B, int32_t Hin, int32_t Win, int32_t Ho, int32_t Wo,
                      int32_t O, int32_t pad, const float *scale, const float *shift, int32_t act, float slope,
                      float *out, int64_t ldo, void *stream);
int efgh_convt_im2col(const float *G, int64_t ldg, int32_t B, int32_t Hin, int32_t Win, int32_t Ho, int32_t Wo,
                      int32_t O, int32_t pad, float *Ycol, int64_t ldy, void *stream);

int efgh_corr_pack_cam(const float *cam, const float *cam_mm, int32_t B, int32_t h, int32_t wc, int32_t segw,
                       int32_t nseg, int32_t nsplit, float *Wc, void *stream);
int efgh_corr_fold(const float *P, int32_t B, int32_t nsplit, int64_t Mv, int32_t ldp, int32_t nseg, int32_t segw,
                   int32_t nj, float *logit, float *score, void *stream);
int efgh_norm_bwd(const float *x, const float *dxn, const float *mm, int32_t B, int64_t n, float *part, float *dx, void *stream);
int efgh_corr_planes(const float *x, const float *mm, int32_t B, int32_t h, int32_t w, int32_t w_in_pitch, int32_t wP,
                     float *out, void *stream);
int efgh_corr_unplanes(const float *in, int32_t B, int32_t h, int32_t w, int32_t wP, float *out, void *stream);
int efgh_corr_toeplitz(const float *dl, int32_t B, int32_t nj, int32_t rows, int32_t cols, int32_t colsP, int32_t transpose,
                       float *T, void *stream);

int efgh_wino_supported(const efgh_gemm_desc *d);
int32_t efgh_wino_grid_m(int32_t B, int32_t H, int32_t W);
int efgh_wino_pack(const float *Wp, float *U, int32_t N, int32_t C, void *stream);
int efgh_wino_conv3x3_hpool(const efgh_gemm_desc *d, const float *U, void *stream);
int efgh_wino_conv3x3(const efgh_gemm_desc *d, const float *U, void *stream);
int efgh_wino_wgrad_supported(const efgh_gemm_desc *d);
int64_t efgh_wino_wgrad_workspace(const efgh_gemm_desc *d);
int efgh_wino_wgrad(const efgh_gemm_desc *d, const float *G, int64_t ldg, float *S, float *dWp, const efgh_wgrad_out_desc *out,
                    void *stream);

int efgh_prep_affine_nearest_u8(const uint8_t *in, int32_t h, int32_t w, const int64_t *coef6_host, uint8_t *out,
                                int32_t nh, int32_t nw, void *stream);
int efgh_prep_crop_pad_u8(const uint8_t *in, int32_t h, int32_t w, int32_t oy, int32_t ox, uint8_t *out, int32_t th,
                          int32_t tw, void *stream);
int efgh_prep_resample_u8(const uint8_t *in, int32_t h, int32_t w, int32_t axis, int32_t out_size, const int32_t *bounds,
                          const int32_t *coeffs, int32_t ksize, uint8_t *out, void *stream);
int efgh_prep_hwc_to_chw_u8(const uint8_t *in, int32_t h, int32_t w, uint8_t *chw, uint8_t *mask, void *stream);
int efgh_prep_u8_to_f32_chw_pad(const uint8_t *in, int32_t h, int32_t w, int32_t oy, int32_t ox, float *out, int32_t th,
                                int32_t tw, void *stream);
int32_t efgh_prep_filter_blocks(int32_t n);
int efgh_prep_radius_filter(const float *pcd, const int32_t *pre_idx, int32_t n, int32_t flip_xy, float radius,
                            int32_t *block_scratch, int32_t *keep_idx, int32_t *count, void *stream);
int efgh_prep_gather_transform(const float *pcd, const int32_t *keep_idx, const int32_t *sel, int32_t n_sel,
                               int32_t flip_xy, const double *T34, int32_t num_points, float *out32, double *out64,
                               void *stream);

int efgh_pose_errors(const float *gt, const float *pred, int32_t B, int32_t mode, float *rot_err, float *trs_err,
                     void *stream);

int32_t efgh_gimg_loss_groups(int64_t n);
int efgh_gimg_loss_fwd(const float *pred_depth, const float *pred_mask, int64_t mask_bstride, const float *gdep4,
                       const uint8_t *img_mask, int32_t B, int64_t HW, float *gt_depth, float *gt_mask, double *part,
                       float *out3, void *stream);
int efgh_gimg_loss_bwd(const float *pred_depth, const float *pred_mask, int64_t mask_bstride, const float *gt_depth,
                       const uint8_t *img_mask, int32_t B, int64_t HW, const float *sums3, const float *g_depth,
                       const float *g_mask, float *d_pred_depth, float *d_pred_mask, int64_t dmask_bstride, void *stream);

int efgh_sum_depth_last(const float *pc, int64_t pc_cstride, int32_t N, const double *T34, int32_t H, int32_t W, int32_t *idx_ws,
                        uint8_t *out, void *stream);
int efgh_sum_range_last(const float *pc, int64_t pc_cstride, int32_t N, const double *T34, int32_t H, int32_t W, double fov_up,
                        double fov_down, int32_t *idx_ws, double *out, void *stream);
int efgh_sum_paint(const void *jobs_dev, int32_t njobs, void *stream);
int efgh_sum_colorize(const double *minmax, int64_t n, const uint8_t *lut, uint8_t *rgb, uint8_t *mask, void *stream);

int efgh_pose_head_normal(const float *abs_logits, int64_t lda, const float *sgn_logits, int64_t lds, int32_t B, int32_t nd,
                          float dx, float dy, float dz, float *abs_out, float *normal, float *R44, void *stream);
int efgh_pose_head_yaw(const float *score, int64_t lds, int32_t B, int32_t n, float *R44, void *stream);
int efgh_pose_cam_T_velo(const float *c_T, int64_t ldc, const float *l_T, const float *calib, const float *A, int32_t B,
                         float *out34, void *stream);

int efgh_pose_head_normal_bwd(const float *abs_logits, int64_t lda, const float *sgn_logits, int64_t lds, int32_t B, int32_t nd,
                              float dx, float dy, float dz, const float *g_abs, const float *g_normal, const float *g_R44,
                              float *g_abs_logits, void *stream);
int efgh_pose_mat44_mul(const float *a, const float *b, int32_t B, int32_t transpose_a, int32_t transpose_b, float *out, void *stream);
int efgh_pose_rotation_between(const float *src3, int32_t B, float dx, float dy, float dz, float *R44, void *stream);
int efgh_pose_cam_T_velo_bwd(const float *c_T, int64_t ldc, const float *l_T, const float *calib, const float *A,
                             const float *g_out34, int32_t B, float *g_cT33, float *g_lT44, void *stream);

typedef struct {
    const float *e_gn_abs, *e_gn_sgn, *h_hrzn_abs, *h_hrzn_sgn, *f_score, *g_trs, *e_l, *f_l;
    int64_t ld_e_gn_sgn, ld_h_hrzn_sgn, ld_f_score;
    const float *rand_init_l, *rand_init_c, *sensor2_T_sensor1;
    int32_t rand_init_l_dim, rand_init_c_dim;
    int32_t B, W, fov_pos_num;
    float fov_neg_ratio;
    float lambda_e_gn, lambda_h_hrzn, lambda_fov, lambda_g_trs, lambda_g_depth, lambda_g_mask;
} efgh_pose_loss_desc;
int efgh_pose_loss_fwd(const efgh_pose_loss_desc *d, const float *l_depth, const float *l_mask, float *gt72, int64_t *gt_cls2,
                       float *gt_f_score, float *selected, float *partials, float *L11, float *n_selected, void *stream);
int efgh_pose_loss_bwd(const efgh_pose_loss_desc *d, const float *g_L11, const float *selected, const float *n_selected,
                       float *g_e_gn_abs, float *g_e_gn_sgn, float *g_h_hrzn_abs, float *g_h_hrzn_sgn, float *g_f_score,
                       float *g_g_trs, float *g_e_l, float *g_ldepth_lmask, void *stream);

#ifdef __cplusplus
}
#endif
#endif
```

Baseline: 31.26 frame-pairs/s.

## Recompute first 4-channel conv instead of storing full-resolution pre-pool activations

For large first-layer 3x3 convs with 4 input channels followed by BN+ReLU+pool, the forward now runs a stats-only conv pass and then a fused conv+BN+pool pass, so the full-resolution raw output is never written. In backward, the conv is recomputed inside a new fused kernel that applies the pool/activation/BN backward and writes the input gradient directly. The goal is to cut the large full-resolution memory traffic and footprint in exchange for running the cheap conv two extra times. Flat-scale channels fall back to recomputing the dot product in the reduce kernel.

New measurement: 31.46 frame-pairs/s, median of 6. About the same (+0.6%).

```diff
diff --git a/efgh_amd/csrc/backward.hip b/efgh_amd/csrc/backward.hip
--- a/efgh_amd/csrc/backward.hip
+++ b/efgh_amd/csrc/backward.hip
@@ -132,29 +132,6 @@
     }
 }
 
-__device__ __forceinline__ void pool_cell_dpre(const float4 v[4], const bool ok[4], bool pooled, const float4 g, const float sc[4],
-                                               const float sf[4], int act, float slope, float dpre[4][4]) {
-#pragma unroll
-    for (int ch = 0; ch < 4; ++ch) {
-        float e[4];
-#pragma unroll
-        for (int q = 0; q < 4; ++q) {
-            const float t = ((const float *)&v[q])[ch] * sc[ch] + sf[ch];
-            e[q] = act == 1 ? (t > 0.f ? t : 0.f) : (act == 2 ? (t > 0.f ? t : t * slope) : t);
-        }
-        int best = 0;
-#pragma unroll
-        for (int q = 1; q < 4; ++q) if (e[q] > e[best]) best = q;
-        const float gg = ((const float *)&g)[ch];
-#pragma unroll
-        for (int q = 0; q < 4; ++q) {
-            const float t = ((const float *)&v[q])[ch] * sc[ch] + sf[ch];
-            const float da = act == 1 ? (t > 0.f ? 1.f : 0.f) : (act == 2 ? (t > 0.f ? 1.f : slope) : 1.f);
-            dpre[q][ch] = (pooled && q == best && ok[q]) ? gg * da : 0.f;
-        }
-    }
-}
-
 template <bool NT>
 __global__ void __launch_bounds__(TPB)
 k_pool_bn_bwd_reduce(const float *__restrict__ dyp, const float *__restrict__ raw, const float *__restrict__ mean,
@@ -215,7 +192,8 @@
 k_pool_bn_bwd_reduce_y(const float *__restrict__ dyp, const float *__restrict__ y, const float *__restrict__ raw,
                        const float *__restrict__ mean, const float *__restrict__ invstd, const float *__restrict__ pscale,
                        const float *__restrict__ pshift, int H, int W, int C, long long Mp, int rows_per_block, int CL,
-                       double *__restrict__ part) {
+                       double *__restrict__ part, const float *__restrict__ x4 = nullptr, long long ldx = 0,
+                       const float *__restrict__ Wt = nullptr, const float *__restrict__ bias = nullptr) {
     __shared__ double s1s[TPB][4], s2s[TPB][4];
     const int cl = threadIdx.x % CL, rl = threadIdx.x / CL, RL = TPB / CL;
     const int c = (blockIdx.x * CL + cl) * 4;
@@ -243,8 +221,24 @@
             if (flat) {
                 const int j = (int)(r % Wo); const long long t = r / Wo;
                 const int i = (int)(t % Ho); const long long b = t / Ho;
-                const float4 w4 = *reinterpret_cast<const float4 *>(raw + (((b * H + 2 * i) * W) + 2 * j) * (long long)C + c);
-                rw0[0] = w4.x; rw0[1] = w4.y; rw0[2] = w4.z; rw0[3] = w4.w;
+                if (raw) {
+                    const float4 w4 = *reinterpret_cast<const float4 *>(raw + (((b * H + 2 * i) * W) + 2 * j) * (long long)C + c);
+                    rw0[0] = w4.x; rw0[1] = w4.y; rw0[2] = w4.z; rw0[3] = w4.w;
+                } else {
+#pragma unroll
+                    for (int q = 0; q < 4; ++q) {
+                        if (scv[q] != 0.f) continue;
+                        float a = 0.f;
+                        for (int t = 0; t < 9; ++t) {
+                            const int yin = 2 * i - 1 + t / 3, xin = 2 * j - 1 + t % 3;
+                            if ((unsigned)yin >= (unsigned)H || (unsigned)xin >= (unsigned)W) continue;
+                            const float4 px = *reinterpret_cast<const float4 *>(x4 + ((b * H + yin) * W + xin) * ldx);
+                            const float4 wv = *reinterpret_cast<const float4 *>(Wt + ((long long)(c + q) * 9 + t) * 4);
+                            a = fmaf(px.x, wv.x, a); a = fmaf(px.y, wv.y, a); a = fmaf(px.z, wv.z, a); a = fmaf(px.w, wv.w, a);
+                        }
+                        rw0[q] = a + (bias ? bias[c + q] : 0.f);
+                    }
+                }
             }
 #pragma unroll
             for (int q = 0; q < 4; ++q) {
@@ -300,8 +294,7 @@
             float o[4];
 #pragma unroll
             for (int ch = 0; ch < 4; ++ch) {
-                const double xh = ((double)((const float *)&v[q])[ch] - (double)mean[c + ch]) * (double)invstd[c + ch];
-                o[ch] = (float)((double)coef[c + ch] * ((double)dpre[q][ch] - m1[c + ch] - xh * m2[c + ch]));
+                o[ch] = bn_bwd_draw(((const float *)&v[q])[ch], mean[c + ch], invstd[c + ch], coef[c + ch], dpre[q][ch], m1[c + ch], m2[c + ch]);
             }
             st_stream<NT>(draw + base + offs[q], make_float4(o[0], o[1], o[2], o[3]));
         }
@@ -723,6 +716,30 @@
     return EFGH_OK;
 }
 
+extern "C" int efgh_pool_bn_bwd_reduce_pooled_x4(const float *dy_pool, const float *y_pool, const float *x4, int64_t ldx,
+                                                 const float *Wt, const float *bias, const float *mean, const float *invstd,
+                                                 const float *pscale, const float *pshift, int32_t B, int32_t H, int32_t W,
+                                                 int32_t C, double *part, float *sum_dpre, float *sum_dpre_xhat, double *mean_dpre,
+                                                 double *mean_dpre_xhat, void *stream_) {
+    hipStream_t st = (hipStream_t)stream_;
+    EFGH_CHECK_ARG(dy_pool && y_pool && x4 && Wt && mean && invstd && pscale && pshift && part && sum_dpre && sum_dpre_xhat &&
+                   mean_dpre && mean_dpre_xhat);
+    EFGH_CHECK_ARG(B > 0 && H >= 2 && W >= 2 && C > 0 && C % 4 == 0 && ldx >= 4 && ldx % 4 == 0);
+    EFGH_CHECK_ARG((((uintptr_t)x4) & 15) == 0 && (((uintptr_t)Wt) & 15) == 0);
+    const long long Mp = (long long)B * (H / 2) * (W / 2);
+    const int G = efgh_bwd_groups(Mp);
+    int CL = 1;
+    while (CL < 64 && CL * 4 < C) CL <<= 1;
+    if (efgh_stream_nt(Mp * C * 4)) k_pool_bn_bwd_reduce_y<true><<<dim3(cdiv(C / 4, CL), G), TPB, 0, st>>>(dy_pool, y_pool, nullptr, mean, invstd, pscale, pshift, H, W, C, Mp,
+                                                                  (int)bwd_rows_per_block(Mp), CL, part, x4, ldx, Wt, bias);
+    else k_pool_bn_bwd_reduce_y<false><<<dim3(cdiv(C / 4, CL), G), TPB, 0, st>>>(dy_pool, y_pool, nullptr, mean, invstd, pscale, pshift, H, W, C, Mp,
+                                                                  (int)bwd_rows_per_block(Mp), CL, part, x4, ldx, Wt, bias);
+    k_bwd_finalize<<<cdiv(C, 32), dim3(32, 32), 0, st>>>(part, G, C, (double)B * H * W, sum_dpre, sum_dpre_xhat, mean_dpre,
+                                                         mean_dpre_xhat);
+    EFGH_CHECK_LAUNCH();
+    return EFGH_OK;
+}
+
 extern "C" int efgh_pool_bn_bwd_apply(const float *dy_pool, const float *raw, const float *mean, const float *invstd,
                                       const float *coef, const double *m1, const double *m2, const float *pscale,
                                       const float *pshift, int32_t B, int32_t H, int32_t W, int32_t C, int32_t act,
diff --git a/efgh_amd/csrc/c4conv.hip b/efgh_amd/csrc/c4conv.hip
--- a/efgh_amd/csrc/c4conv.hip
+++ b/efgh_amd/csrc/c4conv.hip
@@ -20,6 +20,7 @@
     float *stats;
     long long units; int jblocks;
     const float *G; long long ldg; float *dW;
+    const float *mean, *invstd, *coef; const double *m1, *m2;
 };
 
 __device__ __forceinline__ void unit_coords(const C4Args &p, long long unit, long long &row, int &i, long long &b, int &j0) {
@@ -43,7 +44,7 @@
     __builtin_amdgcn_fence(__ATOMIC_ACQUIRE, "wavefront");
 }
 
-template <int NT, bool RES>
+template <int NT, bool RES, bool STORE = true>
 __global__ void __launch_bounds__(64 * WAVES, 2) k_c4_conv(const C4Args p) {
     __shared__ float2 Pw[WAVES][3][2][LWMAX + 1];
     __shared__ float red[2][WAVES][NT * 32];
@@ -140,7 +141,7 @@
                                    : make_float4(0.f, 0.f, 0.f, 0.f);
                 }
             }
-            wave_lds_sync();
+            if (STORE) wave_lds_sync();
 #pragma unroll
             for (int q = 0; q < 16; ++q) {
                 const int pl = (q & 3) + 8 * (q >> 2) + 4 * h;
@@ -148,8 +149,9 @@
                 float v = acc[j][q] + bi[j];
                 if (ok) { s1[j] += v; s2[j] = fmaf(v, v, s2[j]); }
                 v = fmaf(v, sc[j], sf[j]);
-                T[pl * TPITCH + r] = RES ? v : act_neg(v, neg);
-            }
+                if (STORE) T[pl * TPITCH + r] = RES ? v : act_neg(v, neg);
+            }
+            if (!STORE) continue;
             wave_lds_sync();
 #pragma unroll
             for (int pass = 0; pass < 4; ++pass) {
@@ -194,18 +196,20 @@
     return make_float4(0.f, 0.f, 0.f, 0.f);
 }
 
-template <int NT>
-__global__ void __launch_bounds__(64 * WAVES, 2) k_c4_conv_pool(const C4Args p) {
+template <int NT, bool BWD, bool NTS>
+__device__ __forceinline__ void c4_rowpair(const C4Args &p) {
     __shared__ float2 Pw[WAVES][4][2][LW1 + 1];
     constexpr int TPITCH = 40;
     __shared__ __attribute__((aligned(16))) float Tw[WAVES][32 * TPITCH];
     const int tid = threadIdx.x, lane = tid & 63, wave = tid >> 6, r = lane & 31, h = lane >> 5;
     float2 (*P)[2][LW1 + 1] = Pw[wave];
     float *T = Tw[wave];
-    const int Hp = p.Ho >> 1, Wp = p.Wo >> 1;
+    const int Hp = BWD ? (p.Ho + 1) >> 1 : p.Ho >> 1, Wp = p.Wo >> 1;
 
     float2 bw[9][NT];
     float bi[NT], sc[NT], sf[NT];
+    float mu[NT], is[NT], cf[NT];
+    double dm1[NT], dm2[NT];
 #pragma unroll
     for (int j = 0; j < NT; ++j) {
         const int n = 32 * j + r;
@@ -214,6 +218,7 @@
         bi[j] = p.bias ? p.bias[n] : 0.f;
         sc[j] = p.scale ? p.scale[n] : 1.f;
         sf[j] = p.shift ? p.shift[n] : 0.f;
+        if (BWD) { mu[j] = p.mean[n]; is[j] = p.invstd[n]; cf[j] = p.coef[n]; dm1[j] = p.m1[n]; dm2[j] = p.m2[n]; }
     }
     const float neg = p.act == 1 ? 0.f : (p.act == 2 ? p.slope : 1.f);
 #pragma unroll
@@ -254,6 +259,19 @@
     for (; unit < p.units; unit += nwaves) {
         const long long orow0 = crow; const int oj0 = cj0;
         wave_lds_sync();
+        const int oip = (int)(orow0 % Hp); const long long ob = orow0 / Hp;
+        const bool row1 = 2 * oip + 1 < p.Ho;
+        float gw[NT][8];
+        if (BWD) {
+            const float *grow = p.G + ((ob * (p.Ho >> 1) + oip) * Wp + (oj0 >> 1) + 2 * h) * p.ldg + r;
+#pragma unroll
+            for (int j = 0; j < NT; ++j)
+#pragma unroll
+                for (int w = 0; w < 8; ++w) {
+                    const int pl0 = ((2 * w) & 3) + 8 * ((2 * w) >> 2);
+                    gw[j][w] = (row1 && oj0 + pl0 + 4 * h + 1 < p.Wo) ? grow[(long long)(pl0 >> 1) * p.ldg + 32 * j] : 0.f;
+                }
+        }
         f32x16 acc[2][NT];
 #pragma unroll
         for (int half = 0; half < 2; ++half) {
@@ -277,6 +295,51 @@
         if (unit + nwaves < p.units) {
             EFGH_STAGE()
             if (unit + 2 * nwaves < p.units) EFGH_FETCH(unit + 2 * nwaves)
+        }
+        if (BWD) {
+            const int c4l = (lane & 7) * 4;
+            float *olane = p.out + ((ob * p.Ho + 2 * oip) * p.Wo + oj0 + (lane >> 3)) * p.ldo + c4l;
+#pragma unroll
+            for (int j = 0; j < NT; ++j) {
+                const float scv[4] = {sc[j], sc[j], sc[j], sc[j]}, sfv[4] = {sf[j], sf[j], sf[j], sf[j]};
+                const bool ok[4] = {true, true, true, true};
+#pragma unroll
+                for (int w4 = 0; w4 < 2; ++w4) {
+                    float4 v[4];
+#pragma unroll
+                    for (int pos = 0; pos < 4; ++pos) {
+                        const int hf = pos >> 1, dq = pos & 1;
+                        v[pos] = make_float4(acc[hf][j][8 * w4 + dq] + bi[j], acc[hf][j][8 * w4 + 2 + dq] + bi[j],
+                                             acc[hf][j][8 * w4 + 4 + dq] + bi[j], acc[hf][j][8 * w4 + 6 + dq] + bi[j]);
+                    }
+                    const float4 g = make_float4(gw[j][4 * w4], gw[j][4 * w4 + 1], gw[j][4 * w4 + 2], gw[j][4 * w4 + 3]);
+                    float dpre[4][4];
+                    pool_cell_dpre(v, ok, true, g, scv, sfv, 1, 0.f, dpre);
+                    float o[2][8];
+#pragma unroll
+                    for (int pos = 0; pos < 4; ++pos)
+#pragma unroll
+                        for (int k = 0; k < 4; ++k)
+                            o[pos >> 1][2 * k + (pos & 1)] =
+                                bn_bwd_draw(((const float *)&v[pos])[k], mu[j], is[j], cf[j], dpre[pos][k], dm1[j], dm2[j]);
+#pragma unroll
+                    for (int half = 0; half < 2; ++half) {
+                        if (half == 1 && !row1) break;
+                        wave_lds_sync();
+#pragma unroll
+                        for (int q = 0; q < 8; ++q) T[(16 * w4 + (q & 3) + 8 * (q >> 2) + 4 * h) * TPITCH + r] = o[half][q];
+                        wave_lds_sync();
+                        float *orow = olane + ((long long)half * p.Wo + 16 * w4) * p.ldo + 32 * j;
+#pragma unroll
+                        for (int pass = 0; pass < 2; ++pass) {
+                            const int pl = 16 * w4 + 8 * pass + (lane >> 3);
+                            if (oj0 + pl < p.Wo)
+                                st_stream<NTS>(orow + (long long)(8 * pass) * p.ldo, *reinterpret_cast<const float4 *>(&T[pl * TPITCH + c4l]));
+                        }
+                    }
+                }
+            }
+            continue;
         }
 #pragma unroll
         for (int j = 0; j < NT; ++j) {
@@ -305,6 +368,12 @@
 #undef EFGH_PUT
 #undef EFGH_STAGE
 }
+
+template <int NT>
+__global__ void __launch_bounds__(64 * WAVES, 2) k_c4_conv_pool(const C4Args p) { c4_rowpair<NT, false, false>(p); }
+
+template <int NT, bool NTS>
+__global__ void __launch_bounds__(64 * WAVES, 2) k_c4_conv_bwd_draw(const C4Args p) { c4_rowpair<NT, true, NTS>(p); }
 
 template <int NT16>
 __global__ void __launch_bounds__(64 * WAVES) k_c4_wgrad(const C4Args p) {
@@ -402,11 +471,12 @@
     a.jblocks = (d->Wo + TP - 1) / TP;
     a.units = (long long)d->B * d->Ho * a.jblocks;
     a.G = nullptr; a.ldg = 0; a.dW = nullptr;
-}
-
-int grid_of(long long units) {
+    a.mean = a.invstd = a.coef = nullptr; a.m1 = a.m2 = nullptr;
+}
+
+int grid_of(long long units, int cap = 768) {
     const long long g = (units + WAVES - 1) / WAVES;
-    return (int)(g < 768 ? g : 768);
+    return (int)(g < cap ? g : cap);
 }
 
 }
@@ -438,6 +508,20 @@
     return EFGH_OK;
 }
 
+extern "C" int efgh_c4_conv3x3_stats(const efgh_gemm_desc *d, void *stream_) {
+    hipStream_t st = (hipStream_t)stream_;
+    EFGH_CHECK_ARG(efgh_c4_supported(d) && d->W && d->stats && !d->residual && (((uintptr_t)d->W) & 7) == 0);
+    C4Args a;
+    fill(a, d);
+    a.out = nullptr;
+    const int grid = grid_of(a.units);
+    if (d->N == 32) k_c4_conv<1, false, false><<<grid, 64 * WAVES, 0, st>>>(a);
+    else if (d->N == 64) k_c4_conv<2, false, false><<<grid, 64 * WAVES, 0, st>>>(a);
+    else k_c4_conv<4, false, false><<<grid, 64 * WAVES, 0, st>>>(a);
+    EFGH_CHECK_LAUNCH();
+    return EFGH_OK;
+}
+
 extern "C" int efgh_c4_pooled_supported(const efgh_gemm_desc *d) {
     return (efgh_c4_supported(d) && d->sh == 1 && !d->residual && !d->stats && d->Ho >= 2 && d->Wo >= 2) ? 1 : 0;
 }
@@ -453,6 +537,34 @@
     if (d->N == 32) k_c4_conv_pool<1><<<grid, 64 * WAVES, 0, st>>>(a);
     else if (d->N == 64) k_c4_conv_pool<2><<<grid, 64 * WAVES, 0, st>>>(a);
     else k_c4_conv_pool<4><<<grid, 64 * WAVES, 0, st>>>(a);
+    EFGH_CHECK_LAUNCH();
+    return EFGH_OK;
+}
+
+extern "C" int efgh_c4_conv_bwd_draw(const efgh_gemm_desc *d, const float *dy_pool, const float *mean, const float *invstd,
+                                     const float *coef, const double *m1, const double *m2, float *draw, int64_t lddraw,
+                                     void *stream_) {
+    hipStream_t st = (hipStream_t)stream_;
+    EFGH_CHECK_ARG(c4_geometry_ok(d) && (d->N == 32 || d->N == 64) && d->sh == 1 && !d->residual && d->Ho >= 2 && d->Wo >= 2);
+    EFGH_CHECK_ARG(d->Hin == d->Ho && d->Win == d->Wo && d->W && (((uintptr_t)d->W) & 7) == 0 && d->scale && d->shift);
+    EFGH_CHECK_ARG(dy_pool && mean && invstd && coef && m1 && m2 && draw && d->act == 1);
+    EFGH_CHECK_ARG(lddraw >= d->N && lddraw % 4 == 0 && (((uintptr_t)draw) & 15) == 0);
+    C4Args a;
+    fill(a, d);
+    a.stats = nullptr;
+    a.out = draw; a.ldo = lddraw;
+    a.G = dy_pool; a.ldg = d->N;
+    a.mean = mean; a.invstd = invstd; a.coef = coef; a.m1 = m1; a.m2 = m2;
+    a.units = (long long)d->B * ((d->Ho + 1) / 2) * a.jblocks;
+    const int grid = grid_of(a.units, 512);
+    const bool nt = efgh_stream_nt((long long)d->B * d->Ho * d->Wo * d->N * 4);
+#define EFGH_GO(NT)                                                                  \
+    {                                                                               \
+        if (nt) k_c4_conv_bwd_draw<NT, true><<<grid, 64 * WAVES, 0, st>>>(a);       \
+        else k_c4_conv_bwd_draw<NT, false><<<grid, 64 * WAVES, 0, st>>>(a);         \
+    }
+    if (d->N == 32) EFGH_GO(1) else EFGH_GO(2)
+#undef EFGH_GO
     EFGH_CHECK_LAUNCH();
     return EFGH_OK;
 }
diff --git a/efgh_amd/csrc/common.h b/efgh_amd/csrc/common.h
--- a/efgh_amd/csrc/common.h
+++ b/efgh_amd/csrc/common.h
@@ -52,6 +52,34 @@
     }
 }
 static inline bool efgh_stream_nt(long long bytes) { return bytes >= (384ll << 20); }
+
+__device__ __forceinline__ void pool_cell_dpre(const float4 v[4], const bool ok[4], bool pooled, const float4 g, const float sc[4],
+                                               const float sf[4], int act, float slope, float dpre[4][4]) {
+#pragma unroll
+    for (int ch = 0; ch < 4; ++ch) {
+        float e[4];
+#pragma unroll
+        for (int q = 0; q < 4; ++q) {
+            const float t = ((const float *)&v[q])[ch] * sc[ch] + sf[ch];
+            e[q] = act == 1 ? (t > 0.f ? t : 0.f) : (act == 2 ? (t > 0.f ? t : t * slope) : t);
+        }
+        int best = 0;
+#pragma unroll
+        for (int q = 1; q < 4; ++q) if (e[q] > e[best]) best = q;
+        const float gg = ((const float *)&g)[ch];
+#pragma unroll
+        for (int q = 0; q < 4; ++q) {
+            const float t = ((const float *)&v[q])[ch] * sc[ch] + sf[ch];
+            const float da = act == 1 ? (t > 0.f ? 1.f : 0.f) : (act == 2 ? (t > 0.f ? 1.f : slope) : 1.f);
+            dpre[q][ch] = (pooled && q == best && ok[q]) ? gg * da : 0.f;
+        }
+    }
+}
+
+__device__ __forceinline__ float bn_bwd_draw(float raw, float mean, float invstd, float coef, float dpre, double m1, double m2) {
+    const double xh = ((double)raw - (double)mean) * (double)invstd;
+    return (float)((double)coef * ((double)dpre - m1 - xh * m2));
+}
 
 static inline bool efgh_raise_lds_once(std::atomic<unsigned long long> &done, const void *fn, int bytes) {
     int dev = 0;
diff --git a/efgh_amd/nets/fn.py b/efgh_amd/nets/fn.py
--- a/efgh_amd/nets/fn.py
+++ b/efgh_amd/nets/fn.py
@@ -167,19 +167,30 @@
         M = spec.M
         bn = spec.bn
         b = None if bias is None else ops.pad_vec(bias.detach(), Np)
-        out = torch.empty(tuple(spec.out_shape) + (Np,), dtype=torch.float32, device=dev)
         res = None if residual is None else as_rows(residual)
         mean = invstd = raw = None
         need_stats = bn is not None and spec.train
         assert spec.custom_forward is None or (bn is not None and bias is None)
+        recompute = (spec.pool and need_stats and spec.act == ops.ACT_RELU and res is None and lazy is None and Np == N
+                     and spec.custom_forward is None and len(spec.launches) == 1 and out_target is None and not spec.passthrough
+                     and ops.c4_pool_recompute_ok(spec.mode, spec.C, Np, spec.launches[0][0], spec.launches[0][1], x, ld_of(x)))
+        ctx.c4_recompute = (b,) if recompute else None
+        out = None if recompute else torch.empty(tuple(spec.out_shape) + (Np,), dtype=torch.float32, device=dev)
         w2v = bool(ctx.needs_input_grad[1])
-        if bn is None:
+        if recompute:
+            g0, m0 = spec.launches[0]
+            wp = spec.layouts[0].pack(weight)
+            stats = ops.c4_conv_stats(x, ld_of(x), wp, Np, m0, g0, b)
+            scale, shift, mean, invstd = bn_batch_stats(bn, stats, Np, float(M), save=True)
+            out = ops.c4_conv_pooled(x, ld_of(x), wp, Np, m0, g0, b, scale, shift, spec.act, spec.slope)
+            ops.C4_POOL_HITS[0] += 1
+        elif bn is None:
             run_launches(spec, x, ld_of(x), weight, out, Np, b, False, lazy=lazy, w2v=w2v, residual=res,
                          ldr=0 if res is None else ld_of(res), act=spec.act, slope=spec.slope)
         else:
             stats = run_launches(spec, x, ld_of(x), weight, out, Np, b, need_stats, lazy=lazy, w2v=w2v)
         y = out
-        if bn is not None:
+        if bn is not None and not recompute:
             raw = out
             if need_stats:
                 scale, shift, mean, invstd = bn_batch_stats(bn, stats, Np, float(M), save=True)
@@ -285,8 +296,17 @@
         pre_v = pre_gy = None
         fuse_bwd = (ops.W2_BWD_FUSED and spec.bwd_fusable and has_bn and spec.train and Np == N
                     and ctx.needs_input_grad[0] and own_wgrad and (ybits is not None or (psc is not None and not has_res))
-                    and len(spec.out_shape) == 3 and ((fused_pool and ops.W2_BWD_FUSED_POOL) or not spec.pool))
-        if fused_pool:
+                    and len(spec.out_shape) == 3 and ((fused_pool and ops.W2_BWD_FUSED_POOL) or not spec.pool)
+                    and ctx.c4_recompute is None)
+        if fused_pool and ctx.c4_recompute is not None:
+            g0, m0 = spec.launches[0]
+            draw, s1, s2 = ops.c4_pool_bn_bwd(dy.contiguous(), y, x, ld_of(x), spec.layouts[0].pack(weight), Np, m0, g0,
+                                              ctx.c4_recompute[0], mean, invstd, coef, psc, psh, spec.act, spec.slope, s1=gs1, s2=gs2)
+            if gs1 is None:
+                dbeta, dgamma = s1, s2
+            if has_bias:
+                dbias = _bias_grad_behind_bn(ctx, p_bias, draw, M, Np, N, True, delivered)
+        elif fused_pool:
             draw, s1, s2 = ops.pool_bn_bwd(dy.contiguous(), raw, mean, invstd, coef, psc, psh, spec.act, spec.slope,
                                            s1=gs1, s2=gs2, transforms=fuse_bwd, y_pool=y)
             if fuse_bwd:
diff --git a/efgh_amd/ops.py b/efgh_amd/ops.py
--- a/efgh_amd/ops.py
+++ b/efgh_amd/ops.py
@@ -540,14 +540,15 @@
     return ev
 
 
-def _prof_end(ev, route, shape, flops, plain, wino_list=None, batched=False):
+def _prof_end(ev, route, shape, flops, plain, wino_list=None, batched=False, nbytes=None):
     if ev is None:
         return
     ev[1].record()
     if route in ('blur_r', 'planes'):
         plain.append(ev + (flops, shape))
         return
-    nbytes = conv_bytes(*shape[1:])
+    if nbytes is None:
+        nbytes = conv_bytes(*shape[1:])
     if PROFILE_DED is not None and (route in _DEDICATED or route == 'sc'):
         PROFILE_DED.append(ev + (nbytes, shape))
     wino = route in ('wino2d', 'wino', 'wino_hpool')
@@ -1353,6 +1354,61 @@
                                         c_int64(lddres), _st()))
 
 
+C4_POOL_RECOMPUTE = True
+C4_POOL_RECOMPUTE_MIN_BYTES = 384 << 20
+C4_POOL_HITS = [0, 0]
+
+
+def c4_pool_recompute_ok(mode, C, N, geom, M, A, lda):
+    if not C4_POOL_RECOMPUTE or geom is None or N not in (32, 64) or 4 * M * N < C4_POOL_RECOMPUTE_MIN_BYTES:
+        return False
+    if gemm_route(mode, C, N, len(geom[7]), geom, M, stats=True) != 'c4' or geom[5] != 1 or geom[6] != 1:
+        return False
+    if (geom[1], geom[2]) != (geom[9], geom[10]) or lda % 4 != 0:
+        return False
+    return bool(_L().efgh_c4_pooled_supported(ctypes.byref(_desc(A, lda, C, 9, mode, N, M, geom))))
+
+
+def c4_conv_stats(A, lda, Wp, N, M, geom, bias):
+    stats = torch.empty((_L().efgh_c4_stats_rows(c_int32(geom[0]), c_int32(geom[9]), c_int32(geom[10])), 2, N), dtype=torch.float32,
+                        device=A.device)
+    d = _desc(A, lda, 4, 9, 1, N, M, geom, Wp=Wp, bias=bias, stats=stats)
+    ev = _prof_start(PROFILE)
+    _C.check(_L().efgh_c4_conv3x3_stats(ctypes.byref(d), _st()))
+    _prof_end(ev, 'c4', (1, M, N, 9, 4), 2.0 * M * N * 36, PROFILE, nbytes=4.0 * (M * 4.0 + N * 36.0))
+    return stats
+
+
+def c4_conv_pooled(A, lda, Wp, N, M, geom, bias, scale, shift, act, slope):
+    y = torch.empty((geom[0], geom[9] // 2, geom[10] // 2, N), dtype=torch.float32, device=A.device)
+    d = _desc(A, lda, 4, 9, 1, N, M, geom, Wp=Wp, out=y, ldo=N, bias=bias, scale=scale, shift=shift, act=act, slope=slope)
+    ev = _prof_start(PROFILE)
+    _C.check(_L().efgh_c4_conv3x3_pooled(ctypes.byref(d), _st()))
+    _prof_end(ev, 'c4', (1, M, N, 9, 4), 2.0 * M * N * 36, PROFILE, nbytes=4.0 * (M * 4.0 + float(y.numel()) + N * 36.0))
+    return y
+
+
+def c4_pool_bn_bwd(dy_pool, y_pool, A, lda, Wp, N, M, geom, bias, mean, invstd, coef, pscale, pshift, act, slope, s1=None, s2=None):
+    B, H, W = geom[0], geom[9], geom[10]
+    dev = A.device
+    assert act == ACT_RELU and dy_pool.is_contiguous() and y_pool.is_contiguous() and tuple(y_pool.shape) == (B, H // 2, W // 2, N)
+    s1 = s1 if s1 is not None else torch.empty(N, dtype=torch.float32, device=dev)
+    s2 = s2 if s2 is not None else torch.empty(N, dtype=torch.float32, device=dev)
+    m1 = torch.empty(N, dtype=torch.float64, device=dev)
+    m2 = torch.empty(N, dtype=torch.float64, device=dev)
+    G = _L().efgh_bwd_groups(c_int64(B * (H // 2) * (W // 2)))
+    part = torch.empty((G, 2, N), dtype=torch.float64, device=dev)
+    _C.check(_L().efgh_pool_bn_bwd_reduce_pooled_x4(ptr(dy_pool), ptr(y_pool), ptr(A), c_int64(lda), ptr(Wp), ptr(bias), ptr(mean),
+                                                    ptr(invstd), ptr(pscale), ptr(pshift), c_int32(B), c_int32(H), c_int32(W), c_int32(N),
+                                                    ptr(part), ptr(s1), ptr(s2), ptr(m1), ptr(m2), _st()))
+    draw = torch.empty((B, H, W, N), dtype=torch.float32, device=dev)
+    d = _desc(A, lda, 4, 9, 1, N, M, geom, Wp=Wp, bias=bias, scale=pscale, shift=pshift, act=act, slope=slope)
+    _C.check(_L().efgh_c4_conv_bwd_draw(ctypes.byref(d), ptr(dy_pool), ptr(mean), ptr(invstd), ptr(coef), ptr(m1), ptr(m2), ptr(draw),
+                                        c_int64(N), _st()))
+    C4_POOL_HITS[1] += 1
+    return draw, s1, s2
+
+
 def col_sum(x, M, C):
     stats, G = col_stats(x, M, C, x.shape[-1])
     return stats[:, 0, :].sum(0)
diff --git a/include/efgh_hip.h b/include/efgh_hip.h
--- a/include/efgh_hip.h
+++ b/include/efgh_hip.h
@@ -241,6 +241,10 @@
                                    const float *invstd, const float *pscale, const float *pshift, int32_t B, int32_t H, int32_t W,
                                    int32_t C, double *part, float *sum_dpre, float *sum_dpre_xhat, double *mean_dpre,
                                    double *mean_dpre_xhat, void *stream);
+int efgh_pool_bn_bwd_reduce_pooled_x4(const float *dy_pool, const float *y_pool, const float *x4, int64_t ldx, const float *Wt,
+                                      const float *bias, const float *mean, const float *invstd, const float *pscale,
+                                      const float *pshift, int32_t B, int32_t H, int32_t W, int32_t C, double *part, float *sum_dpre,
+                                      float *sum_dpre_xhat, double *mean_dpre, double *mean_dpre_xhat, void *stream);
 int efgh_pool_bn_bwd_apply(const float *dy_pool, const float *raw, const float *mean, const float *invstd, const float *coef,
                            const double *m1, const double *m2, const float *pscale, const float *pshift, int32_t B, int32_t H,
                            int32_t W, int32_t C, int32_t act, float slope, float *draw, void *stream);
@@ -280,6 +284,9 @@
 int efgh_c4_conv3x3(const efgh_gemm_desc *d, void *stream);
 int efgh_c4_pooled_supported(const efgh_gemm_desc *d);
 int efgh_c4_conv3x3_pooled(const efgh_gemm_desc *d, void *stream);
+int efgh_c4_conv3x3_stats(const efgh_gemm_desc *d, void *stream);
+int efgh_c4_conv_bwd_draw(const efgh_gemm_desc *d, const float *dy_pool, const float *mean, const float *invstd, const float *coef,
+                          const double *m1, const double *m2, float *draw, int64_t lddraw, void *stream);
 int efgh_c4_wgrad_supported(const efgh_gemm_desc *d);
 int64_t efgh_c4_wgrad_workspace(const efgh_gemm_desc *d);
 int efgh_c4_wgrad(const efgh_gemm_desc *d, const float *G, int64_t ldg, float *dWp, float *workspace,
```
